# Chemical118/TREW

Hardware: NVIDIA B200
Metric: Gbases/s for trew short 5 32 at 1/2/4/8 B200; % of HBM roofline (higher is better)
Workload: dtype u64

## Files before the change

trew_b200/csrc/device_ctx.cu:

```cuda
#include <algorithm>
#include <chrono>
#include <cstdarg>
#include <cstdio>
#include <cstdlib>
#include <cstring>
#include <string>
#include <thread>
#include <vector>

#include <cuda_runtime.h>

#include "host_internal.h"
#include "scan_kernels.cuh"

using namespace trew;

namespace {

struct SlotRes {
    void* h_buf = nullptr;
    void* d_buf = nullptr;
    unsigned char* h_inv = nullptr;
    unsigned char* d_inv = nullptr;
    size_t inv_cap = 0;
    unsigned int* h_keys = nullptr;
    unsigned int* d_survivors = nullptr;
    unsigned int* d_counters = nullptr;
    unsigned char* d_scratch = nullptr;
    size_t scratch_bytes = 0;
    size_t survivors_cap = 0;
    cudaStream_t stream = nullptr;
    cudaEvent_t ev_start = nullptr, ev_done = nullptr;
    bool in_flight = false;
};

struct RangeInfo { uint32_t r0, r1; uint64_t bases; uint32_t max_len; };

}

struct trew_resident {
    void* d_buf = nullptr;
    DevBatch batch{};
    uint32_t n_reads = 0, n_units = 0, max_read_len = 0;
    uint64_t bases = 0;
    unsigned int* d_survivors = nullptr;
    unsigned int* d_counters = nullptr;
    unsigned char* d_scratch = nullptr;
    size_t scratch_bytes = 0;
    cudaEvent_t ev[4] = {nullptr, nullptr, nullptr, nullptr};
    bool ev_pending = false;
};

struct trew_ctx {
    trew_config cfg{};
    int sm_count = 0;
    LaunchPlan plan{};
    cudaStream_t aux_stream = nullptr;
    cudaEvent_t ev_join = nullptr;
    int resident_streams = 1;
    uint64_t resident_seq = 0;
    DevCfg dcfg{};
    size_t n_slots = 0;
    unsigned int* d_error = nullptr;
    unsigned short* d_thr = nullptr;
    unsigned long long* d_total_surv = nullptr;
    std::vector<SlotRes> slots;
    size_t next_slot = 0;
    size_t staging_bytes = 0;
    cudaStream_t main_stream = nullptr;
    cudaEvent_t ev_a = nullptr, ev_b = nullptr;
    trew_entry* d_entries = nullptr; size_t d_entries_cap = 0;
    trew_entry* d_sorted = nullptr; size_t d_sorted_cap = 0;
    trew_entry* d_concat = nullptr; size_t d_concat_cap = 0;
    bool sorted_valid = false;
    void* d_sort_tmp = nullptr; size_t sort_tmp_bytes = 0;
    unsigned int* d_n = nullptr;
    uint64_t n_export = 0;
    bool export_valid = false;
    trew_stats stats{};
    Pool* pool = nullptr;
    bool own_pool = true;
    std::string err;
    std::vector<RangeInfo> ranges_tmp;
    unsigned int keys_seen = 0;
    bool sparse_val = true;
    unsigned int exact_flags = 0;
    std::vector<InvList> inv_tmp;
    IngestScratch ingest;
    cudaEvent_t ev_t0 = nullptr, ev_t1 = nullptr;
    double screen_ms = 0, decide_ms = 0, exact_ms = 0; uint64_t n_prof_scans = 0;
    std::vector<trew_resident*> pending_prof;
    void* h_export = nullptr; size_t h_export_bytes = 0;
    unsigned int report_min = 0;
    trew_entry* d_filtered = nullptr; size_t d_filtered_cap = 0;
};

namespace {

int fail(trew_ctx* c, int status, const char* fmt, ...) {
    char buf[512];
    va_list ap; va_start(ap, fmt); vsnprintf(buf, sizeof(buf), fmt, ap); va_end(ap);
    if (c) c->err = buf;
    return status;
}

#define CK(call)                                                                                         \
    do {                                                                                                 \
        cudaError_t e_ = (call);                                                                         \
        if (e_ != cudaSuccess) return fail(ctx, TREW_ERR_CUDA, "%s: %s", #call, cudaGetErrorString(e_)); \
    } while (0)

void build_thr(double B, std::vector<unsigned short>& thr) {
    thr.assign(kThrTableSize, 0xFFFF);
    for (int T = 1; T < kThrTableSize; T++) {
        int lo = 0, hi = T;
        while (lo < hi) {
            int mid = (lo + hi) / 2;
            if ((double)mid / (double)T >= B) hi = mid; else lo = mid + 1;
        }
        thr[T] = (unsigned short)lo;
    }
}

int run_cap_for(const trew_config& cfg, uint32_t max_read_len) {
    uint32_t w = max_read_len;
    if (cfg.mode == TREW_MODE_LONG) w = std::min<uint32_t>(max_read_len, 2u * (uint32_t)cfg.slice_length);
    w = std::min<uint32_t>(w, (uint32_t)kMaxWindow);
    return (int)std::max<uint32_t>((w + 2 + 7) & ~7u, 32u);
}

constexpr unsigned int kLongThreadCap = 32768;

size_t scratch_need(const trew_ctx* ctx, uint32_t max_read_len, uint32_t n_units, unsigned int* stride, size_t* long_off,
                    unsigned int* s_cap, unsigned int* max_slices) {
    unsigned int st = 16;
    if (ctx->cfg.mode == TREW_MODE_LONG) st = 2u * (max_read_len / (uint32_t)ctx->cfg.slice_length + 2u);
    st = (st + 15u) & ~15u;
    *stride = st;
    size_t bytes = ((size_t)st * (size_t)exact_warps_total(ctx->sm_count) + 255) & ~(size_t)255;
    *long_off = bytes;
    *s_cap = 0; *max_slices = 0;
    if (long_thread_path_applies(ctx->dcfg) && (ctx->exact_flags & 16u)) {
        *s_cap = std::min<unsigned int>(std::max<unsigned int>(n_units, 1u), kLongThreadCap);
        *max_slices = max_read_len / (uint32_t)ctx->cfg.slice_length + 1u;
        bytes += long_thread_scratch_bytes(*s_cap, *max_slices);
    }
    return bytes;
}

constexpr int kScanCounters = 8;

static int env_blocks_thread() {
    static const int v = [] { const char* e = getenv("TREW_GRID_THREAD"); int x = e && *e ? atoi(e) : 0; return x > 0 ? x : 0; }();
    return v;
}

int launch_scan(trew_ctx* ctx, const DevBatch& b, uint32_t n_units, uint32_t max_read_len, unsigned int* d_survivors,
                unsigned int* d_counters, unsigned char** d_scratch, size_t* scratch_bytes, cudaStream_t st,
                cudaEvent_t* ev = nullptr) {
    unsigned int stride, s_cap, max_slices;
    size_t long_off;
    size_t need = scratch_need(ctx, max_read_len, n_units, &stride, &long_off, &s_cap, &max_slices);
    if (need > *scratch_bytes) {
        if (*d_scratch) { CK(cudaStreamSynchronize(st)); CK(cudaFree(*d_scratch)); *d_scratch = nullptr; }
        CK(cudaMalloc((void**)d_scratch, need));
        *scratch_bytes = need;
    }
    ctx->export_valid = false;
    CK(cudaMemsetAsync(d_counters, 0, kScanCounters * sizeof(unsigned int), st));
    if (ev) CK(cudaEventRecord(ev[0], st));
    const bool thread_path = thread_path_applies(ctx->dcfg, max_read_len) && !(ctx->exact_flags & 4u) && n_units < (1u << 28);
    launch_filter(ctx->dcfg, b, n_units, max_read_len, d_survivors + n_units, d_counters + 2, d_survivors, d_counters, ctx->plan, st,
                  ev ? ev[1] : nullptr, thread_path ? d_survivors + n_units - 1 : nullptr, thread_path ? d_counters + 4 : nullptr,
                  d_counters + 7);
    if (ev) CK(cudaEventRecord(ev[2], st));
    ExactArgs a{};
    a.survivors = d_survivors; a.n_survivors = d_counters; a.work_counter = d_counters + 1;
    a.slice_scratch = *d_scratch; a.slice_scratch_stride = stride; a.run_cap = run_cap_for(ctx->cfg, max_read_len);
    a.total_survivors = ctx->d_total_surv;
    a.packed_probes = n_units < (1u << 28) ? 1 : 0;
    a.exp_flags = ctx->exact_flags;
    if (thread_path) {
        unsigned int* hard = d_survivors + n_units;
        launch_exact_thread(ctx->dcfg, b, d_survivors, d_counters, a.packed_probes, hard, d_counters + 3, ctx->d_total_surv,
                            ctx->sm_count, env_blocks_thread(), d_counters + 6, st);
        ExactArgs ab = a;
        ab.survivors = d_survivors + n_units - 1; ab.reverse = 1; ab.n_survivors = d_counters + 4;
        launch_exact(ctx->dcfg, b, ab, ctx->plan, st);
        a.survivors = hard; a.n_survivors = d_counters + 3; a.work_counter = d_counters + 5; a.total_survivors = nullptr;
        ctx->stats.kernel_launches += 2;
    } else if (s_cap > 0 && n_units < (1u << 28)) {
        unsigned int* hard = d_survivors + n_units;
        launch_long_thread(ctx->dcfg, b, d_survivors, d_counters, a.packed_probes, s_cap, max_slices, *d_scratch + long_off, hard,
                           d_counters + 3, ctx->d_total_surv, ctx->sm_count, st);
        a.survivors = hard; a.n_survivors = d_counters + 3; a.total_survivors = nullptr;
        ctx->stats.kernel_launches += 3;
    }
    launch_exact(ctx->dcfg, b, a, ctx->plan, st);
    if (ev) CK(cudaEventRecord(ev[3], st));
    CK(cudaGetLastError());
    ctx->stats.kernel_launches += 3;
    return TREW_OK;
}

int retire_slot(trew_ctx* ctx, SlotRes& s) {
    if (!s.in_flight) return TREW_OK;
    CK(cudaEventSynchronize(s.ev_done));
    float ms = 0.f;
    CK(cudaEventElapsedTime(&ms, s.ev_start, s.ev_done));
    ctx->stats.device_ms += ms;
    s.in_flight = false;
    ctx->keys_seen = std::max(ctx->keys_seen, *s.h_keys);
    return TREW_OK;
}

int export_sorted(trew_ctx* ctx, uint64_t* n_out);
int check_device_error(trew_ctx* ctx);

int grow_table_to(trew_ctx* ctx, size_t min_slots) {
    size_t new_slots = ctx->n_slots;
    while (new_slots < ((size_t)1 << 28) && new_slots < min_slots) new_slots <<= 1;
    if (new_slots == ctx->n_slots) return TREW_OK;
    uint64_t n = 0;
    int rc = export_sorted(ctx, &n);
    if (rc) return rc;
    Slot* d_new = nullptr;
    CK(cudaMalloc((void**)&d_new, new_slots * sizeof(Slot)));
    CK(cudaMemsetAsync(d_new, 0, new_slots * sizeof(Slot), ctx->main_stream));
    CK(cudaMemsetAsync(ctx->d_error + 1, 0, sizeof(unsigned int), ctx->main_stream));
    Slot* d_old = ctx->dcfg.slots;
    ctx->dcfg.slots = d_new; ctx->dcfg.slot_mask = (unsigned int)(new_slots - 1); ctx->n_slots = new_slots;
    launch_merge_entries(ctx->dcfg, ctx->d_entries, (unsigned int)n, ctx->main_stream);
    CK(cudaGetLastError());
    CK(cudaStreamSynchronize(ctx->main_stream));
    CK(cudaFree(d_old));
    ctx->stats.kernel_launches += 1;
    ctx->keys_seen = (unsigned int)n;
    for (auto& sl : ctx->slots) *sl.h_keys = (unsigned int)n;
    return check_device_error(ctx);
}

int maybe_grow_table(trew_ctx* ctx) {
    if ((size_t)ctx->keys_seen * 16 <= ctx->n_slots) return TREW_OK;
    unsigned int keys = 0;
    CK(cudaMemcpy(&keys, ctx->d_error + 1, sizeof(keys), cudaMemcpyDeviceToHost));
    ctx->keys_seen = std::max(ctx->keys_seen, keys);
    if ((size_t)keys * 4 <= ctx->n_slots) return TREW_OK;
    return grow_table_to(ctx, (size_t)keys * 8);
}

int submit_ranges(trew_ctx* ctx, const ChunkView& cv, const RangeInfo* rg, int n_ranges) {
    uint64_t total_bases = 0; uint32_t max_len = 0;
    for (int i = 0; i < n_ranges; i++) { total_bases += rg[i].bases; max_len = std::max(max_len, rg[i].max_len); }
    const uint32_t n = n_ranges ? rg[n_ranges - 1].r1 - rg[0].r0 : 0u;
    if (n == 0) return TREW_OK;
    SlotRes& s = ctx->slots[ctx->next_slot];
    ctx->next_slot = (ctx->next_slot + 1) % ctx->slots.size();
    static const bool trace = getenv("TREW_SUBMIT_TRACE") != nullptr;
    auto now = [] { return std::chrono::duration<double, std::milli>(std::chrono::steady_clock::now().time_since_epoch()).count(); };
    const double t0 = trace ? now() : 0;
    int rc = retire_slot(ctx, s);
    if (rc) return rc;
    const double t1 = trace ? now() : 0;
    if ((rc = maybe_grow_table(ctx)) != TREW_OK) return rc;
    const double t2 = now();
    BatchView v;
    batch_layout(s.h_buf, n, total_bases, &v);
    std::vector<uint64_t> bit0((size_t)n_ranges);
    uint64_t acc = 0;
    for (int i = 0; i < n_ranges; i++) { bit0[i] = acc; acc += rg[i].bases; }
    v.bit_off[n] = (uint32_t)total_bases;
    const uint32_t first = rg[0].r0;
    std::vector<uint64_t> side_flat((size_t)3 * n_ranges);
    uint64_t (*side)[3] = (uint64_t (*)[3])side_flat.data();
    if (ctx->inv_tmp.size() < (size_t)n_ranges) ctx->inv_tmp.resize((size_t)n_ranges);
    auto pack = [&](bool list) {
        pack_prepare(bit0.data(), n_ranges, total_bases, v);
        ctx->pool->run(n_ranges, [&](int i) {
            pack_chunk_range(cv, rg[i].r0, rg[i].r1, rg[i].r0 - first, bit0[i], v, side[i], list ? &ctx->inv_tmp[(size_t)i] : nullptr, list,
                             rg[i].bases);
        });
        pack_fixup(bit0.data(), side, n_ranges, v);
    };
    size_t n_inv = 0;
    bool sparse = ctx->sparse_val;
    pack(sparse);
    const bool tail_pad = (total_bases & 31) != 0;
    if (sparse) {
        n_inv = tail_pad ? 1 : 0;
        for (int i = 0; i < n_ranges; i++) n_inv += ctx->inv_tmp[(size_t)i].size();
        if (n_inv > s.inv_cap) { sparse = false; pack(false); }
    }

    const double t3 = now();
    ctx->stats.host_pack_bytes += total_bases; ctx->stats.host_pack_ms += t3 - t2;
    CK(cudaEventRecord(s.ev_start, s.stream));
    const size_t head_bytes = (size_t)((char*)v.val - (char*)s.h_buf);
    unsigned int* d_val = (unsigned int*)((char*)s.d_buf + head_bytes);
    size_t sent = v.bytes;
    if (sparse) {
        std::vector<size_t> at((size_t)n_ranges + 1, 0);
        for (int i = 0; i < n_ranges; i++) at[(size_t)i + 1] = at[(size_t)i] + ctx->inv_tmp[(size_t)i].bytes();
        ctx->pool->run(n_ranges, [&](int i) {
            const InvList& l = ctx->inv_tmp[(size_t)i];
            if (l.bytes()) memcpy(s.h_inv + at[(size_t)i], l.buf.get(), l.bytes());
        });
        if (tail_pad) inv_record(s.h_inv + at[(size_t)n_ranges], (uint32_t)total_bases, (1ULL << (32 - (total_bases & 31))) - 1ULL);
        const size_t ones_words = (size_t)((total_bases + 31) / 32);
        CK(cudaMemsetAsync(d_val, 0xFF, ones_words * 4, s.stream));
        CK(cudaMemsetAsync(d_val + ones_words, 0, (v.plane_words - ones_words) * 4, s.stream));
        CK(cudaMemcpyAsync(s.d_buf, s.h_buf, head_bytes, cudaMemcpyHostToDevice, s.stream));
        if (n_inv) {
            CK(cudaMemcpyAsync(s.d_inv, s.h_inv, n_inv * kInvRecBytes, cudaMemcpyHostToDevice, s.stream));
            launch_clear_invalid(d_val, (const unsigned int*)s.d_inv, (unsigned int)n_inv, s.stream);
            ctx->stats.kernel_launches += 1;
        }
        sent = head_bytes + n_inv * kInvRecBytes;
    } else {
        CK(cudaMemcpyAsync(s.d_buf, s.h_buf, v.bytes, cudaMemcpyHostToDevice, s.stream));
    }
    DevBatch b{};
    b.n_reads = n;
    b.bit_off = (const unsigned int*)s.d_buf;
    b.hi = (const unsigned int*)((char*)s.d_buf + ((char*)v.hi - (char*)s.h_buf));
    b.lo = b.hi + v.plane_words; b.val = d_val;
    uint32_t n_units = ctx->cfg.mode == TREW_MODE_PAIR ? n / 2 : n;
    rc = launch_scan(ctx, b, n_units, max_len, s.d_survivors, s.d_counters, &s.d_scratch, &s.scratch_bytes, s.stream);
    if (rc) return rc;
    CK(cudaMemcpyAsync(s.h_keys, ctx->d_error + 1, sizeof(unsigned int), cudaMemcpyDeviceToHost, s.stream));
    CK(cudaEventRecord(s.ev_done, s.stream));
    s.in_flight = true;
    ctx->stats.reads += n; ctx->stats.bases += total_bases; ctx->stats.units += n_units; ctx->stats.h2d_bytes += sent;
    if (trace)
        fprintf(stderr, "[submit] %u reads: wait slot %.3f ms, table check %.3f ms, pack %.3f ms, enqueue %.3f ms\n", n, t1 - t0, t2 - t1,
                t3 - t2, now() - t3);
    return TREW_OK;
}

int submit_chunk_view(trew_ctx* ctx, const ChunkView& cv, uint32_t n) {
    if (n == 0) return TREW_OK;
    const uint32_t unit = cv.unit;
    const uint32_t n_units = n / unit;
    uint64_t span = 0;
    for (int sd = 0; sd < (int)unit; sd++) {
        const int32_t* l = cv.locs[sd];
        span += (uint64_t)std::max<int64_t>(0, (int64_t)l[2 * (size_t)(n_units - 1) + 1] - l[0] + 1);
    }
    uint64_t by_size = span / std::max<uint64_t>(1, ctx->staging_bytes / 16) + 1;
    uint32_t n_ranges = (uint32_t)std::min<uint64_t>(n_units, std::max<uint64_t>(by_size, (uint64_t)ctx->pool->size() * 4));
    auto& rg = ctx->ranges_tmp;
    rg.resize(n_ranges);
    for (uint32_t i = 0; i < n_ranges; i++) {
        rg[i].r0 = (uint32_t)((uint64_t)n_units * i / n_ranges) * unit;
        rg[i].r1 = (uint32_t)((uint64_t)n_units * (i + 1) / n_ranges) * unit;
    }
    ctx->pool->run((int)n_ranges, [&](int i) { chunk_stats(cv, rg[i].r0, rg[i].r1, &rg[i].bases, &rg[i].max_len); });
    uint32_t mx = 0;
    for (auto& r : rg) mx = std::max(mx, r.max_len);
    if (ctx->cfg.mode == TREW_MODE_SHORT && mx > 1000)
        return fail(ctx, TREW_ERR_TOO_LONG, "%s", trew_status_string(TREW_ERR_TOO_LONG));
    if (ctx->cfg.mode == TREW_MODE_PAIR && mx > (uint32_t)kMaxWindow) return fail(ctx, TREW_ERR_TOO_LONG, "paired read longer than %d", kMaxWindow);
    const size_t cap = ctx->slots[0].survivors_cap;
    uint32_t g = 0;
    while (g < n_ranges) {
        uint32_t h = g; uint64_t bases = 0; uint64_t reads = 0;
        while (h < n_ranges) {
            uint64_t nb = bases + rg[h].bases, nr = reads + (rg[h].r1 - rg[h].r0);
            if (batch_bytes((uint32_t)nr, nb) > ctx->staging_bytes || nr > cap || nb >= 0xfffff000ULL) break;
            bases = nb; reads = nr; h++;
        }
        if (h == g) {
            if (rg[g].r1 - rg[g].r0 <= unit)
                return fail(ctx, TREW_ERR_ARG, "a single read/pair (%llu bases) does not fit a staging buffer of %zu bytes",
                            (unsigned long long)rg[g].bases, ctx->staging_bytes);
            std::vector<RangeInfo> fine;
            for (uint32_t r = rg[g].r0; r < rg[g].r1; r += unit) {
                RangeInfo f{r, r + unit, 0, 0};
                chunk_stats(cv, f.r0, f.r1, &f.bases, &f.max_len);
                fine.push_back(f);
            }
            size_t a = 0;
            while (a < fine.size()) {
                size_t e = a; uint64_t fb = 0, fr = 0;
                while (e < fine.size()) {
                    uint64_t nb = fb + fine[e].bases, nr = fr + unit;
                    if (batch_bytes((uint32_t)nr, nb) > ctx->staging_bytes || nr > cap || nb >= 0xfffff000ULL) break;
                    fb = nb; fr = nr; e++;
                }
                if (e == a)
                    return fail(ctx, TREW_ERR_ARG, "a single read/pair (%llu bases) does not fit a staging buffer of %zu bytes",
                                (unsigned long long)fine[a].bases, ctx->staging_bytes);
                std::vector<RangeInfo> merged;
                size_t per = std::max<size_t>(1, (e - a) / (size_t)ctx->pool->size());
                for (size_t i = a; i < e; i += per) {
                    RangeInfo m{fine[i].r0, 0, 0, 0};
                    for (size_t j = i; j < std::min(e, i + per); j++) { m.r1 = fine[j].r1; m.bases += fine[j].bases; m.max_len = std::max(m.max_len, fine[j].max_len); }
                    merged.push_back(m);
                }
                int rc = submit_ranges(ctx, cv, merged.data(), (int)merged.size());
                if (rc) return rc;
                a = e;
            }
            g++;
            continue;
        }
        int rc = submit_ranges(ctx, cv, rg.data() + g, (int)(h - g));
        if (rc) return rc;
        g = h;
    }
    return TREW_OK;
}

int collect_prof(trew_ctx* ctx) {
    for (trew_resident* r : ctx->pending_prof) {
        if (!r->ev_pending) continue;
        CK(cudaEventSynchronize(r->ev[3]));
        float a = 0, b = 0, c = 0;
        CK(cudaEventElapsedTime(&a, r->ev[0], r->ev[1]));
        CK(cudaEventElapsedTime(&b, r->ev[1], r->ev[2]));
        CK(cudaEventElapsedTime(&c, r->ev[2], r->ev[3]));
        ctx->screen_ms += a; ctx->decide_ms += b; ctx->exact_ms += c; ctx->n_prof_scans++;
        ctx->stats.device_ms += a + b + c;
        r->ev_pending = false;
    }
    ctx->pending_prof.clear();
    return TREW_OK;
}

int join_aux(trew_ctx* ctx) {
    if (ctx->resident_streams != 2) return TREW_OK;
    CK(cudaEventRecord(ctx->ev_join, ctx->aux_stream));
    CK(cudaStreamWaitEvent(ctx->main_stream, ctx->ev_join, 0));
    return TREW_OK;
}

int fork_aux(trew_ctx* ctx) {
    if (ctx->resident_streams != 2) return TREW_OK;
    CK(cudaEventRecord(ctx->ev_join, ctx->main_stream));
    CK(cudaStreamWaitEvent(ctx->aux_stream, ctx->ev_join, 0));
    return TREW_OK;
}

int check_device_error(trew_ctx* ctx) {
    unsigned int e = 0;
    CK(cudaMemcpy(&e, ctx->d_error, sizeof(e), cudaMemcpyDeviceToHost));
    if (e == 3u) return fail(ctx, TREW_ERR_TABLE_FULL, "device count table full (%zu slots): raise table_log2_slots", ctx->n_slots);
    if (e) return fail(ctx, TREW_ERR_CUDA, "device error flag %u", e);
    return TREW_OK;
}

}

extern "C" {

int trew_abi_version(void) { return TREW_ABI_VERSION; }

const char* trew_status_string(int status) {
    switch (status) {
        case TREW_OK: return "ok";
        case TREW_ERR_ARG: return "bad argument";
        case TREW_ERR_CUDA: return "CUDA failure";
        case TREW_ERR_TABLE_FULL: return "device count table full";
        case TREW_ERR_TOO_LONG: return "This mode is designed for short-read sequencing. Please use 'trew long'.";
        case TREW_ERR_IO: return "file I/O error";
        case TREW_ERR_PAIRING: return "paired-end record mismatch";
        case TREW_ERR_NOMEM: return "memory allocation failure";
        default: return "unknown status";
    }
}

static thread_local std::string g_create_error;

static int default_host_threads(int asked) {
    return asked > 0 ? asked : (int)std::min(64u, std::max(1u, std::thread::hardware_concurrency()));
}

const char* trew_dev_last_error(const trew_ctx* ctx) { return ctx ? ctx->err.c_str() : g_create_error.c_str(); }

static int create_ctx(const trew_config* cfg, trew_ctx** out, std::string& g_create_error, Pool* shared_pool) {
    if (!cfg || !out) return TREW_ERR_ARG;
    *out = nullptr;
    g_create_error.clear();
    auto bad_arg = [&](const char* msg) { g_create_error = msg; return TREW_ERR_ARG; };
    if (cfg->mode < 0 || cfg->mode > 2) return bad_arg("mode must be TREW_MODE_SHORT, _PAIR or _LONG");
    if (cfg->min_mer < 3 || cfg->max_mer > 64 || cfg->min_mer > cfg->max_mer) return bad_arg("need 3 <= MIN_MER <= MAX_MER <= 64");
    if (!(0 < cfg->low_baseline && cfg->low_baseline <= 1) || !(0 < cfg->high_baseline && cfg->high_baseline <= 1) ||
        cfg->low_baseline > cfg->high_baseline) return bad_arg("need 0 < LOW_BASELINE <= HIGH_BASELINE <= 1");
    if (cfg->mode == TREW_MODE_LONG && cfg->slice_length > 0 && cfg->slice_length < 2 * cfg->max_mer)
        return bad_arg("SLICE_LENGTH must be greater than or equal to twice of MAX_MER.");
    if (cfg->mode == TREW_MODE_LONG && cfg->slice_length > 512)
        return bad_arg("SLICE_LENGTH above 512 is not supported by the GPU path (a slice of up to 2*SLICE_LENGTH-1 bases must fit "
                       "a 1023-base window); use -s 512 or less.");
    trew_ctx* ctx = new trew_ctx();
    ctx->cfg = *cfg;
    if (ctx->cfg.slice_length <= 0) ctx->cfg.slice_length = 150;
    auto bail = [&](int rc) { g_create_error = ctx->err; trew_dev_destroy(ctx); return rc; };
#define CKC(call)                                                                                   \
    do {                                                                                            \
        cudaError_t e_ = (call);                                                                    \
        if (e_ != cudaSuccess) { fail(ctx, TREW_ERR_CUDA, "%s: %s", #call, cudaGetErrorString(e_)); return bail(TREW_ERR_CUDA); } \
    } while (0)
    const bool timing = getenv("TREW_CLI_TIMING") != nullptr;
    auto now = [] { return std::chrono::duration<double, std::milli>(std::chrono::steady_clock::now().time_since_epoch()).count(); };
    double t_prev = now();
    auto lap = [&](const char* what) {
        if (!timing) return;
        const double t = now();
        fprintf(stderr, "[trew] create, device %d: %s %.1f ms\n", cfg->device, what, t - t_prev);
        t_prev = t;
    };
    int ndev = 0;
    CKC(cudaGetDeviceCount(&ndev));
    lap("driver init");
    if (cfg->device < 0 || cfg->device >= ndev) { fail(ctx, TREW_ERR_CUDA, "no CUDA device %d (found %d)", cfg->device, ndev); return bail(TREW_ERR_CUDA); }
    CKC(cudaSetDevice(cfg->device));
    cudaDeviceProp prop;
    CKC(cudaGetDeviceProperties(&prop, cfg->device));
    ctx->sm_count = prop.multiProcessorCount;
    ctx->plan = default_launch_plan(ctx->sm_count);
    {
        auto env_int = [](const char* name, int dflt) { const char* e = getenv(name); return e && *e ? atoi(e) : dflt; };
        int v;
        if ((v = env_int("TREW_GRID_SCREEN", 0)) > 0) ctx->plan.screen_blocks = ctx->sm_count * v;
        if ((v = env_int("TREW_GRID_DECIDE", 0)) > 0) ctx->plan.decide_blocks = ctx->sm_count * v;
        if ((v = env_int("TREW_GRID_EXACT", 0)) > 0) ctx->plan.exact_blocks = std::min(ctx->plan.exact_blocks, ctx->sm_count * v);
        ctx->resident_streams = env_int("TREW_RESIDENT_STREAMS", 1) >= 2 ? 2 : 1;
        ctx->sparse_val = env_int("TREW_DENSE_VAL", 0) == 0;
        ctx->exact_flags = (unsigned int)env_int("TREW_EXACT_FLAGS", 0);
    }
    int lg = cfg->table_log2_slots > 0 ? cfg->table_log2_slots : 22;
    if (lg < 10 || lg > 28) { fail(ctx, TREW_ERR_ARG, "table_log2_slots out of range"); return bail(TREW_ERR_ARG); }
    ctx->n_slots = (size_t)1 << lg;
    Slot* d_slots = nullptr;
    CKC(cudaMalloc((void**)&d_slots, ctx->n_slots * sizeof(Slot)));
    CKC(cudaMemset(d_slots, 0, ctx->n_slots * sizeof(Slot)));
    lap("primary context + count table");
    CKC(cudaMalloc((void**)&ctx->d_error, 2 * sizeof(unsigned int)));
    CKC(cudaMemset(ctx->d_error, 0, 2 * sizeof(unsigned int)));
    CKC(cudaMalloc((void**)&ctx->d_total_surv, sizeof(unsigned long long)));
    CKC(cudaMemset(ctx->d_total_surv, 0, sizeof(unsigned long long)));
    std::vector<unsigned short> thr;
    build_thr(cfg->low_baseline, thr);
    std::vector<unsigned short> thr_hi;
    build_thr(cfg->high_baseline, thr_hi);
    CKC(cudaMalloc((void**)&ctx->d_thr, 2 * thr.size() * sizeof(unsigned short)));
    CKC(cudaMemcpy(ctx->d_thr, thr.data(), thr.size() * sizeof(unsigned short), cudaMemcpyHostToDevice));
    CKC(cudaMemcpy(ctx->d_thr + thr.size(), thr_hi.data(), thr_hi.size() * sizeof(unsigned short), cudaMemcpyHostToDevice));
    ctx->dcfg.mode = cfg->mode; ctx->dcfg.min_mer = cfg->min_mer; ctx->dcfg.max_mer = cfg->max_mer;
    ctx->dcfg.slice_len = ctx->cfg.slice_length; ctx->dcfg.low = cfg->low_baseline; ctx->dcfg.high = cfg->high_baseline;
    ctx->dcfg.slots = d_slots; ctx->dcfg.slot_mask = (unsigned int)(ctx->n_slots - 1);
    ctx->dcfg.error_flag = ctx->d_error; ctx->dcfg.thr_low = ctx->d_thr; ctx->dcfg.thr_high = ctx->d_thr + kThrTableSize;
    CKC(prepare_exact(kMaxWindow + 9));
    lap("kernel attributes (module load)");
    CKC(cudaStreamCreateWithFlags(&ctx->main_stream, cudaStreamNonBlocking));
    CKC(cudaStreamCreateWithFlags(&ctx->aux_stream, cudaStreamNonBlocking));
    CKC(cudaEventCreateWithFlags(&ctx->ev_join, cudaEventDisableTiming));
    CKC(cudaEventCreate(&ctx->ev_a));
    CKC(cudaEventCreate(&ctx->ev_b));
    CKC(cudaEventCreate(&ctx->ev_t0));
    CKC(cudaEventCreate(&ctx->ev_t1));
    ctx->staging_bytes = cfg->staging_bytes ? (size_t)cfg->staging_bytes : ((size_t)64 << 20);
    int ns = cfg->n_staging > 0 ? cfg->n_staging : 3;
    ctx->slots.resize((size_t)ns);
    for (auto& s : ctx->slots) {
        CKC(cudaHostAlloc(&s.h_buf, ctx->staging_bytes, cudaHostAllocDefault));
        CKC(cudaMalloc(&s.d_buf, ctx->staging_bytes));
        s.inv_cap = ctx->staging_bytes / 8 / kInvRecBytes;
        CKC(cudaHostAlloc((void**)&s.h_inv, (s.inv_cap + 1) * kInvRecBytes, cudaHostAllocDefault));
        CKC(cudaMalloc((void**)&s.d_inv, (s.inv_cap + 1) * kInvRecBytes));
        CKC(cudaHostAlloc((void**)&s.h_keys, sizeof(unsigned int), cudaHostAllocDefault));
        *s.h_keys = 0;
        s.survivors_cap = ctx->staging_bytes / 8;
        CKC(cudaMalloc((void**)&s.d_survivors, 2 * s.survivors_cap * sizeof(unsigned int)));
        CKC(cudaMalloc((void**)&s.d_counters, kScanCounters * sizeof(unsigned int)));
        CKC(cudaStreamCreateWithFlags(&s.stream, cudaStreamNonBlocking));
        CKC(cudaEventCreate(&s.ev_start));
        CKC(cudaEventCreate(&s.ev_done));
    }
    CKC(cudaMalloc((void**)&ctx->d_n, sizeof(unsigned int)));
    lap("staging ring (pinned + device buffers)");
    if (shared_pool) { ctx->pool = shared_pool; ctx->own_pool = false; }
    else ctx->pool = new Pool(default_host_threads(cfg->host_threads));
#undef CKC
    *out = ctx;
    return TREW_OK;
}

int trew_dev_create(const trew_config* cfg, trew_ctx** out) { return create_ctx(cfg, out, g_create_error, nullptr); }

void trew_dev_destroy(trew_ctx* ctx) {
    if (!ctx) return;
    cudaSetDevice(ctx->cfg.device);
    cudaDeviceSynchronize();
    for (auto& s : ctx->slots) {
        if (s.h_buf) cudaFreeHost(s.h_buf);
        if (s.d_buf) cudaFree(s.d_buf);
        if (s.h_inv) cudaFreeHost(s.h_inv);
        if (s.d_inv) cudaFree(s.d_inv);
        if (s.h_keys) cudaFreeHost(s.h_keys);
        if (s.d_survivors) cudaFree(s.d_survivors);
        if (s.d_counters) cudaFree(s.d_counters);
        if (s.d_scratch) cudaFree(s.d_scratch);
        if (s.stream) cudaStreamDestroy(s.stream);
        if (s.ev_start) cudaEventDestroy(s.ev_start);
        if (s.ev_done) cudaEventDestroy(s.ev_done);
    }
    if (ctx->dcfg.slots) cudaFree(ctx->dcfg.slots);
    if (ctx->d_error) cudaFree(ctx->d_error);
    if (ctx->d_thr) cudaFree(ctx->d_thr);
    if (ctx->d_total_surv) cudaFree(ctx->d_total_surv);
    if (ctx->d_entries) cudaFree(ctx->d_entries);
    if (ctx->d_sorted) cudaFree(ctx->d_sorted);
    if (ctx->d_concat) cudaFree(ctx->d_concat);
    if (ctx->d_filtered) cudaFree(ctx->d_filtered);
    if (ctx->d_sort_tmp) cudaFree(ctx->d_sort_tmp);
    if (ctx->d_n) cudaFree(ctx->d_n);
    if (ctx->h_export) cudaFreeHost(ctx->h_export);
    if (ctx->main_stream) cudaStreamDestroy(ctx->main_stream);
    if (ctx->aux_stream) cudaStreamDestroy(ctx->aux_stream);
    if (ctx->ev_join) cudaEventDestroy(ctx->ev_join);
    if (ctx->ev_a) cudaEventDestroy(ctx->ev_a);
    if (ctx->ev_b) cudaEventDestroy(ctx->ev_b);
    if (ctx->ev_t0) cudaEventDestroy(ctx->ev_t0);
    if (ctx->ev_t1) cudaEventDestroy(ctx->ev_t1);
    if (ctx->own_pool) delete ctx->pool;
    delete ctx;
}

int trew_dev_submit_chunk(trew_ctx* ctx, const char* buffer1, const int32_t* locs1, uint32_t n1,
                          const char* buffer2, const int32_t* locs2, uint32_t n2) {
    if (!ctx) return TREW_ERR_ARG;
    CK(cudaSetDevice(ctx->cfg.device));
    const bool pair = ctx->cfg.mode == TREW_MODE_PAIR;
    if (pair ? (!buffer2 && n2) : (buffer2 != nullptr || n2 != 0)) return fail(ctx, TREW_ERR_ARG, "second chunk only in pair mode");
    if ((n1 && (!buffer1 || !locs1)) || (n2 && !locs2)) return fail(ctx, TREW_ERR_ARG, "null chunk");
    ChunkView cv{{buffer1, buffer2}, {locs1, locs2}, {nullptr, nullptr}, pair ? 2u : 1u};
    const uint32_t n = pair ? 2u * std::min(n1, n2) : n1;
    if (n == 0) return TREW_OK;
    for (int sd = 0; sd < (pair ? 2 : 1); sd++) {
        const int32_t* l = cv.locs[sd];
        uint32_t cnt = pair ? n / 2 : n;
        int32_t last = l[2 * (size_t)(cnt - 1) + 1];
        if (last >= l[2 * (size_t)(cnt - 1)]) cv.end[sd] = cv.buf[sd] + last + 1;
    }
    return submit_chunk_view(ctx, cv, n);
}

int trew_dev_submit_packed(trew_ctx* ctx, const trew_batch* batch) {
    if (!ctx || !batch) return TREW_ERR_ARG;
    CK(cudaSetDevice(ctx->cfg.device));
    uint32_t n = batch->n_reads;
    if (n == 0) return TREW_OK;
    uint64_t bases = batch->bit_off[n];
    size_t bytes = batch_bytes(n, bases);
    if (bytes > ctx->staging_bytes || n > ctx->slots[0].survivors_cap)
        return fail(ctx, TREW_ERR_ARG, "packed batch (%zu bytes) larger than a staging buffer (%zu)", bytes, ctx->staging_bytes);
    if (batch->bit_off[0] != 0) return fail(ctx, TREW_ERR_ARG, "bit_off[0] must be 0");
    SlotRes& s = ctx->slots[ctx->next_slot];
    ctx->next_slot = (ctx->next_slot + 1) % ctx->slots.size();
    int rc = retire_slot(ctx, s);
    if (rc) return rc;
    BatchView v;
    batch_layout(s.h_buf, n, bases, &v);
    size_t words = (size_t)((bases + 31) / 32);
    memcpy(v.bit_off, batch->bit_off, (size_t)(n + 1) * 4);
    const uint32_t* src[3] = {batch->hi, batch->lo, batch->val};
    uint32_t* dst[3] = {v.hi, v.lo, v.val};
    ctx->pool->run(3, [&](int i) {
        memcpy(dst[i], src[i], words * 4);
        memset(dst[i] + words, 0, (v.plane_words - words) * 4);
    });
    CK(cudaEventRecord(s.ev_start, s.stream));
    CK(cudaMemcpyAsync(s.d_buf, s.h_buf, v.bytes, cudaMemcpyHostToDevice, s.stream));
    DevBatch b{};
    b.n_reads = n;
    b.bit_off = (const unsigned int*)s.d_buf;
    b.hi = (const unsigned int*)((char*)s.d_buf + ((char*)v.hi - (char*)s.h_buf));
    b.lo = b.hi + v.plane_words; b.val = b.lo + v.plane_words;
    uint32_t n_units = ctx->cfg.mode == TREW_MODE_PAIR ? n / 2 : n;
    rc = launch_scan(ctx, b, n_units, batch->max_read_len, s.d_survivors, s.d_counters, &s.d_scratch, &s.scratch_bytes, s.stream);
    if (rc) return rc;
    CK(cudaMemcpyAsync(s.h_keys, ctx->d_error + 1, sizeof(unsigned int), cudaMemcpyDeviceToHost, s.stream));
    CK(cudaEventRecord(s.ev_done, s.stream));
    s.in_flight = true;
    ctx->stats.reads += n; ctx->stats.bases += bases; ctx->stats.units += n_units; ctx->stats.h2d_bytes += v.bytes;
    return TREW_OK;
}

int trew_dev_upload(trew_ctx* ctx, const trew_batch* batch, trew_resident** out) {
    if (!ctx || !batch || !out) return TREW_ERR_ARG;
    CK(cudaSetDevice(ctx->cfg.device));
    uint32_t n = batch->n_reads;
    uint64_t bases = n ? batch->bit_off[n] : 0;
    trew_resident* r = new trew_resident();
    size_t bytes = batch_bytes(n, bases);
    std::vector<char> tmp(bytes, 0);
    BatchView v;
    batch_layout(tmp.data(), n, bases, &v);
    size_t words = (size_t)((bases + 31) / 32);
    if (n) {
        memcpy(v.bit_off, batch->bit_off, (size_t)(n + 1) * 4);
        memcpy(v.hi, batch->hi, words * 4); memcpy(v.lo, batch->lo, words * 4); memcpy(v.val, batch->val, words * 4);
    }
    CK(cudaMalloc(&r->d_buf, bytes));
    CK(cudaMemcpy(r->d_buf, tmp.data(), bytes, cudaMemcpyHostToDevice));
    r->batch.n_reads = n;
    r->batch.bit_off = (const unsigned int*)r->d_buf;
    r->batch.hi = (const unsigned int*)((char*)r->d_buf + ((char*)v.hi - tmp.data()));
    r->batch.lo = r->batch.hi + v.plane_words; r->batch.val = r->batch.lo + v.plane_words;
    r->n_reads = n; r->n_units = ctx->cfg.mode == TREW_MODE_PAIR ? n / 2 : n; r->max_read_len = batch->max_read_len; r->bases = bases;
    CK(cudaMalloc((void**)&r->d_survivors, 2 * (size_t)std::max<uint32_t>(r->n_units, 1) * sizeof(unsigned int)));
    CK(cudaMalloc((void**)&r->d_counters, kScanCounters * sizeof(unsigned int)));
    *out = r;
    return TREW_OK;
}

int trew_dev_scan_resident(trew_ctx* ctx, const trew_resident* rb) {
    if (!ctx || !rb) return TREW_ERR_ARG;
    CK(cudaSetDevice(ctx->cfg.device));
    trew_resident* r = const_cast<trew_resident*>(rb);
    ctx->keys_seen = std::max<unsigned int>(ctx->keys_seen, (unsigned int)(ctx->n_slots / 16 + 1));
    if (r->ev_pending) { int rc0 = collect_prof(ctx); if (rc0) return rc0; }
    if (!r->ev[0]) for (int i = 0; i < 4; i++) CK(cudaEventCreate(&r->ev[i]));
    cudaStream_t st = (ctx->resident_streams == 2 && (ctx->resident_seq++ & 1)) ? ctx->aux_stream : ctx->main_stream;
    CK(cudaEventRecord(ctx->ev_a, st));
    int rc = launch_scan(ctx, r->batch, r->n_units, r->max_read_len, r->d_survivors, r->d_counters, &r->d_scratch,
                         &r->scratch_bytes, st, r->ev);
    r->ev_pending = true; ctx->pending_prof.push_back(r);
    if (rc) return rc;
    CK(cudaEventRecord(ctx->ev_b, st));
    ctx->stats.reads += r->n_reads; ctx->stats.bases += r->bases; ctx->stats.units += r->n_units;
    return TREW_OK;
}

void trew_dev_free_resident(trew_ctx* ctx, trew_resident* r) {
    if (!r) return;
    if (ctx) { cudaSetDevice(ctx->cfg.device); cudaStreamSynchronize(ctx->main_stream); cudaStreamSynchronize(ctx->aux_stream); collect_prof(ctx); }
    for (int i = 0; i < 4; i++) if (r->ev[i]) cudaEventDestroy(r->ev[i]);
    if (r->d_buf) cudaFree(r->d_buf);
    if (r->d_survivors) cudaFree(r->d_survivors);
    if (r->d_counters) cudaFree(r->d_counters);
    if (r->d_scratch) cudaFree(r->d_scratch);
    delete r;
}

int trew_dev_sync(trew_ctx* ctx) {
    if (!ctx) return TREW_ERR_ARG;
    CK(cudaSetDevice(ctx->cfg.device));
    for (auto& s : ctx->slots) { int rc = retire_slot(ctx, s); if (rc) return rc; }
    { int rc = join_aux(ctx); if (rc) return rc; }
    CK(cudaStreamSynchronize(ctx->main_stream));
    { int rc = collect_prof(ctx); if (rc) return rc; }
    return check_device_error(ctx);
}

}

namespace {

int export_entries(trew_ctx* ctx, bool need_sorted, const trew_entry** out, uint64_t* n_out) {
    int rc = trew_dev_sync(ctx);
    if (rc) return rc;
    if (!ctx->export_valid) {
        unsigned int n = 0;
        for (int pass = 0; pass < 2; pass++) {
            CK(cudaMemsetAsync(ctx->d_n, 0, sizeof(unsigned int), ctx->main_stream));
            if (pass == 0 && ctx->d_entries_cap == 0) {
                ctx->d_entries_cap = (size_t)1 << 20;
                CK(cudaMalloc((void**)&ctx->d_entries, ctx->d_entries_cap * sizeof(trew_entry)));
            }
            launch_compact(ctx->dcfg.slots, (unsigned int)ctx->n_slots, ctx->d_entries, ctx->d_n, ctx->main_stream,
                           (unsigned int)ctx->d_entries_cap);
            CK(cudaGetLastError());
            ctx->stats.kernel_launches += 1;
            CK(cudaMemcpyAsync(&n, ctx->d_n, sizeof(n), cudaMemcpyDeviceToHost, ctx->main_stream));
            CK(cudaStreamSynchronize(ctx->main_stream));
            if (n <= ctx->d_entries_cap) break;
            CK(cudaFree(ctx->d_entries));
            ctx->d_entries = nullptr;
            ctx->d_entries_cap = (size_t)n + n / 4 + 1024;
            CK(cudaMalloc((void**)&ctx->d_entries, ctx->d_entries_cap * sizeof(trew_entry)));
        }
        ctx->n_export = n;
        ctx->export_valid = true;
        ctx->sorted_valid = false;
    }
    const unsigned int n = (unsigned int)ctx->n_export;
    if (need_sorted && !ctx->sorted_valid) {
        if (n > ctx->d_sorted_cap) {
            if (ctx->d_sorted) CK(cudaFree(ctx->d_sorted));
            ctx->d_sorted = nullptr;
            ctx->d_sorted_cap = std::max<size_t>((size_t)n + n / 4 + 1024, (size_t)1 << 20);
            CK(cudaMalloc((void**)&ctx->d_sorted, ctx->d_sorted_cap * sizeof(trew_entry)));
        }
        if (n == 1) CK(cudaMemcpyAsync(ctx->d_sorted, ctx->d_entries, sizeof(trew_entry), cudaMemcpyDeviceToDevice, ctx->main_stream));
        if (n > 1) {
            const bool wide = ctx->cfg.max_mer > 32;
            size_t need = 0;
            CK(sort_entries_radix(ctx->d_entries, ctx->d_sorted, n, wide, nullptr, &need, ctx->main_stream));
            if (need > ctx->sort_tmp_bytes) {
                if (ctx->d_sort_tmp) CK(cudaFree(ctx->d_sort_tmp));
                ctx->d_sort_tmp = nullptr;
                ctx->sort_tmp_bytes = need + need / 4;
                CK(cudaMalloc(&ctx->d_sort_tmp, ctx->sort_tmp_bytes));
            }
            size_t bytes = ctx->sort_tmp_bytes;
            CK(sort_entries_radix(ctx->d_entries, ctx->d_sorted, n, wide, ctx->d_sort_tmp, &bytes, ctx->main_stream));
            ctx->stats.kernel_launches += wide ? 11 : 8;
        }
        CK(cudaStreamSynchronize(ctx->main_stream));
        ctx->sorted_valid = true;
    }
    if (out) *out = need_sorted ? ctx->d_sorted : ctx->d_entries;
    if (n_out) *n_out = n;
    return TREW_OK;
}

int export_sorted(trew_ctx* ctx, uint64_t* n_out) { return export_entries(ctx, false, nullptr, n_out); }

int rows_to_host(trew_ctx* ctx, const trew_entry* d_rows, uint64_t n, const trew_entry** entries, uint64_t* n_entries) {
    size_t need_host = (size_t)n * sizeof(trew_entry) + 64;
    if (need_host > ctx->h_export_bytes) {
        if (ctx->h_export) CK(cudaFreeHost(ctx->h_export));
        ctx->h_export = nullptr;
        size_t cap = std::max(need_host * 2, (size_t)1 << 20);
        CK(cudaHostAlloc(&ctx->h_export, cap, cudaHostAllocDefault));
        ctx->h_export_bytes = cap;
    }
    if (n) {
        CK(cudaMemcpyAsync(ctx->h_export, d_rows, n * sizeof(trew_entry), cudaMemcpyDeviceToHost, ctx->main_stream));
        CK(cudaStreamSynchronize(ctx->main_stream));
    }
    ctx->stats.d2h_bytes += n * sizeof(trew_entry) + 4;
    if (entries) *entries = (const trew_entry*)ctx->h_export;
    if (n_entries) *n_entries = n;
    return TREW_OK;
}

int finish_rows(trew_ctx* ctx, const trew_entry* d_in, uint64_t n_in, bool combine, const trew_entry** entries, uint64_t* n_entries) {
    auto ensure = [&](trew_entry** buf, size_t* cap, size_t want) -> int {
        if (want <= *cap) return TREW_OK;
        if (*buf) CK(cudaFree(*buf));
        *buf = nullptr;
        *cap = std::max<size_t>(want + want / 4 + 1024, (size_t)1 << 20);
        CK(cudaMalloc((void**)buf, *cap * sizeof(trew_entry)));
        return TREW_OK;
    };
    auto ensure_tmp = [&](size_t need) -> int {
        if (need <= ctx->sort_tmp_bytes) return TREW_OK;
        CK(cudaStreamSynchronize(ctx->main_stream));
        if (ctx->d_sort_tmp) CK(cudaFree(ctx->d_sort_tmp));
        ctx->d_sort_tmp = nullptr;
        ctx->sort_tmp_bytes = need + need / 4;
        CK(cudaMalloc(&ctx->d_sort_tmp, ctx->sort_tmp_bytes));
        return TREW_OK;
    };
    int rc;
    if ((rc = ensure(&ctx->d_sorted, &ctx->d_sorted_cap, (size_t)n_in)) != TREW_OK) return rc;
    if ((rc = ensure(&ctx->d_filtered, &ctx->d_filtered_cap, (size_t)n_in)) != TREW_OK) return rc;
    ctx->sorted_valid = false;
    const bool wide = ctx->cfg.max_mer > 32;
    const trew_entry* src = d_in;
    unsigned int n = (unsigned int)n_in;
    if (ctx->report_min > 0 && n > 0) {
        size_t need = 0;
        CK(filter_report_rows(src, n, ctx->report_min, ctx->d_filtered, ctx->d_n, nullptr, &need, ctx->main_stream));
        if ((rc = ensure_tmp(need)) != TREW_OK) return rc;
        size_t bytes = ctx->sort_tmp_bytes;
        CK(filter_report_rows(src, n, ctx->report_min, ctx->d_filtered, ctx->d_n, ctx->d_sort_tmp, &bytes, ctx->main_stream));
        CK(cudaMemcpyAsync(&n, ctx->d_n, sizeof(n), cudaMemcpyDeviceToHost, ctx->main_stream));
        CK(cudaStreamSynchronize(ctx->main_stream));
        ctx->stats.kernel_launches += 5;
        src = ctx->d_filtered;
    }
    if (n == 1) CK(cudaMemcpyAsync(ctx->d_sorted, src, sizeof(trew_entry), cudaMemcpyDeviceToDevice, ctx->main_stream));
    if (n > 1) {
        size_t need = 0;
        CK(sort_entries_radix(src, ctx->d_sorted, n, wide, nullptr, &need, ctx->main_stream));
        if ((rc = ensure_tmp(need)) != TREW_OK) return rc;
        size_t bytes = ctx->sort_tmp_bytes;
        CK(sort_entries_radix(src, ctx->d_sorted, n, wide, ctx->d_sort_tmp, &bytes, ctx->main_stream));
        ctx->stats.kernel_launches += wide ? 11 : 8;
    }
    const trew_entry* rows = ctx->d_sorted;
    if (combine && n > 0) {
        size_t need = 0;
        CK(combine_sorted_rows(ctx->d_sorted, n, ctx->d_filtered, ctx->d_n, nullptr, &need, ctx->main_stream));
        if ((rc = ensure_tmp(need)) != TREW_OK) return rc;
        size_t bytes = ctx->sort_tmp_bytes;
        CK(combine_sorted_rows(ctx->d_sorted, n, ctx->d_filtered, ctx->d_n, ctx->d_sort_tmp, &bytes, ctx->main_stream));
        CK(cudaMemcpyAsync(&n, ctx->d_n, sizeof(n), cudaMemcpyDeviceToHost, ctx->main_stream));
        CK(cudaStreamSynchronize(ctx->main_stream));
        ctx->stats.kernel_launches += 3;
        rows = ctx->d_filtered;
    }
    return rows_to_host(ctx, rows, n, entries, n_entries);
}

}

extern "C" {

int trew_dev_export_device(trew_ctx* ctx, const trew_entry** d_entries, uint64_t* n_entries) {
    if (!ctx) return TREW_ERR_ARG;
    return export_entries(ctx, true, d_entries, n_entries);
}

int trew_dev_finish(trew_ctx* ctx, const trew_entry** entries, uint64_t* n_entries) {
    if (!ctx) return TREW_ERR_ARG;
    uint64_t n = 0;
    const trew_entry* d_rows = nullptr;
    if (ctx->report_min > 0) {
        int rc = export_entries(ctx, false, &d_rows, &n);
        if (rc) return rc;
        return finish_rows(ctx, d_rows, n, false, entries, n_entries);
    }
    int rc = export_entries(ctx, true, &d_rows, &n);
    if (rc) return rc;
    return rows_to_host(ctx, d_rows, n, entries, n_entries);
}

int trew_dev_finish_merged(trew_ctx* ctx, const trew_entry* const* d_lists, const uint64_t* n_rows, uint32_t n_lists,
                           const trew_entry** entries, uint64_t* n_entries) {
    if (!ctx || (n_lists && (!d_lists || !n_rows))) return TREW_ERR_ARG;
    uint64_t n0 = 0;
    const trew_entry* d_own = nullptr;
    int rc = export_entries(ctx, false, &d_own, &n0);
    if (rc) return rc;
    uint64_t total = n0;
    for (uint32_t i = 0; i < n_lists; i++) total += n_rows[i];
    if (total > 0xfffffff0ULL) return fail(ctx, TREW_ERR_ARG, "too many rows to merge (%llu)", (unsigned long long)total);
    auto ensure = [&](trew_entry** buf, size_t* cap) -> int {
        if (total <= *cap) return TREW_OK;
        if (*buf) CK(cudaFree(*buf));
        *buf = nullptr;
        *cap = std::max<size_t>((size_t)total + total / 4 + 1024, (size_t)1 << 20);
        CK(cudaMalloc((void**)buf, *cap * sizeof(trew_entry)));
        return TREW_OK;
    };
    if ((rc = ensure(&ctx->d_concat, &ctx->d_concat_cap)) != TREW_OK) return rc;
    uint64_t at = 0;
    if (n0) CK(cudaMemcpyAsync(ctx->d_concat, d_own, n0 * sizeof(trew_entry), cudaMemcpyDeviceToDevice, ctx->main_stream));
    at += n0;
    for (uint32_t i = 0; i < n_lists; i++) {
        if (n_rows[i]) CK(cudaMemcpyAsync(ctx->d_concat + at, d_lists[i], n_rows[i] * sizeof(trew_entry), cudaMemcpyDeviceToDevice, ctx->main_stream));
        at += n_rows[i];
    }
    return finish_rows(ctx, ctx->d_concat, total, true, entries, n_entries);
}

int trew_dev_export_rows(trew_ctx* ctx, trew_entry* d_rows, uint64_t capacity_rows, uint64_t* n_rows) {
    if (!ctx || !n_rows) return TREW_ERR_ARG;
    uint64_t n = 0;
    const trew_entry* d_src = nullptr;
    int rc = export_entries(ctx, false, &d_src, &n);
    if (rc) return rc;
    *n_rows = n;
    if (!d_rows) return TREW_OK;
    if (n > capacity_rows) return fail(ctx, TREW_ERR_ARG, "row buffer too small: %llu rows, capacity %llu", (unsigned long long)n,
                                       (unsigned long long)capacity_rows);
    if (n) CK(cudaMemcpyAsync(d_rows, d_src, n * sizeof(trew_entry), cudaMemcpyDeviceToDevice, ctx->main_stream));
    CK(cudaStreamSynchronize(ctx->main_stream));
    return TREW_OK;
}

int trew_dev_merge_rows(trew_ctx* ctx, const trew_entry* d_rows, uint64_t n_rows) {
    if (!ctx || (n_rows && !d_rows) || n_rows > 0xffffffffULL) return TREW_ERR_ARG;
    CK(cudaSetDevice(ctx->cfg.device));
    ctx->export_valid = false;
    ctx->keys_seen = std::max<unsigned int>(ctx->keys_seen, (unsigned int)(ctx->n_slots / 16 + 1));
    launch_merge_entries(ctx->dcfg, d_rows, (unsigned int)n_rows, ctx->main_stream);
    CK(cudaGetLastError());
    ctx->stats.kernel_launches += n_rows ? 1 : 0;
    return TREW_OK;
}

int trew_dev_set_report_filter(trew_ctx* ctx, uint32_t min_total) {
    if (!ctx) return TREW_ERR_ARG;
    ctx->report_min = min_total;
    return TREW_OK;
}

int trew_dev_reserve(trew_ctx* ctx, uint64_t expected_new_keys) {
    if (!ctx) return TREW_ERR_ARG;
    int rc = trew_dev_sync(ctx);
    if (rc) return rc;
    unsigned int keys = 0;
    CK(cudaMemcpy(&keys, ctx->d_error + 1, sizeof(keys), cudaMemcpyDeviceToHost));
    const uint64_t want = ((uint64_t)keys + expected_new_keys) * 4;
    if (want <= ctx->n_slots) return TREW_OK;
    return grow_table_to(ctx, (size_t)std::min<uint64_t>(want, (uint64_t)1 << 28));
}

int trew_dev_reset(trew_ctx* ctx) {
    if (!ctx) return TREW_ERR_ARG;
    int rc = trew_dev_sync(ctx);
    if (rc && rc != TREW_ERR_TABLE_FULL) return rc;
    ctx->export_valid = false;
    CK(cudaMemsetAsync(ctx->dcfg.slots, 0, ctx->n_slots * sizeof(Slot), ctx->main_stream));
    CK(cudaMemsetAsync(ctx->d_error, 0, 2 * sizeof(unsigned int), ctx->main_stream));
    CK(cudaStreamSynchronize(ctx->main_stream));
    ctx->keys_seen = 0;
    for (auto& sl : ctx->slots) *sl.h_keys = 0;
    return TREW_OK;
}

int trew_dev_get_stats(trew_ctx* ctx, trew_stats* out) {
    if (!ctx || !out) return TREW_ERR_ARG;
    CK(cudaSetDevice(ctx->cfg.device));
    unsigned long long s = 0;
    CK(cudaMemcpy(&s, ctx->d_total_surv, sizeof(s), cudaMemcpyDeviceToHost));
    ctx->stats.survivors = s;
    *out = ctx->stats;
    return TREW_OK;
}

int trew_dev_last_resident_ms(trew_ctx* ctx, float* ms) {
    if (!ctx || !ms) return TREW_ERR_ARG;
    CK(cudaEventSynchronize(ctx->ev_b));
    CK(cudaEventElapsedTime(ms, ctx->ev_a, ctx->ev_b));
    return TREW_OK;
}

int trew_dev_timer_start(trew_ctx* ctx) {
    if (!ctx) return TREW_ERR_ARG;
    CK(cudaSetDevice(ctx->cfg.device));
    CK(cudaEventRecord(ctx->ev_t0, ctx->main_stream));
    return fork_aux(ctx);
}

int trew_dev_timer_stop(trew_ctx* ctx, float* ms) {
    if (!ctx || !ms) return TREW_ERR_ARG;
    CK(cudaSetDevice(ctx->cfg.device));
    { int rc = join_aux(ctx); if (rc) return rc; }
    CK(cudaEventRecord(ctx->ev_t1, ctx->main_stream));
    CK(cudaEventSynchronize(ctx->ev_t1));
    CK(cudaEventElapsedTime(ms, ctx->ev_t0, ctx->ev_t1));
    return TREW_OK;
}

int trew_dev_kernel_times(trew_ctx* ctx, double* screen_ms, double* decide_ms, double* exact_ms, uint64_t* n_scans) {
    if (!ctx) return TREW_ERR_ARG;
    CK(cudaSetDevice(ctx->cfg.device));
    { int rc0 = join_aux(ctx); if (rc0) return rc0; }
    CK(cudaStreamSynchronize(ctx->main_stream));
    int rc = collect_prof(ctx);
    if (rc) return rc;
    if (screen_ms) *screen_ms = ctx->screen_ms;
    if (decide_ms) *decide_ms = ctx->decide_ms;
    if (exact_ms) *exact_ms = ctx->exact_ms;
    if (n_scans) *n_scans = ctx->n_prof_scans;
    ctx->screen_ms = ctx->decide_ms = ctx->exact_ms = 0; ctx->n_prof_scans = 0;
    return TREW_OK;
}

int trew_synth_resident(trew_ctx* ctx, uint64_t seed, uint32_t n_reads, uint32_t read_len, uint32_t tel_ppm,
                        uint32_t half_ppm, uint32_t n_ppm, uint32_t sub_ppm, trew_resident** out) {
    return trew_synth_resident_ex(ctx, seed, n_reads, read_len, tel_ppm, half_ppm, n_ppm, sub_ppm, 0, out);
}

int trew_synth_resident_ex(trew_ctx* ctx, uint64_t seed, uint32_t n_reads, uint32_t read_len, uint32_t tel_ppm,
                           uint32_t half_ppm, uint32_t n_ppm, uint32_t sub_ppm, uint32_t flavor, trew_resident** out) {
    if (!ctx || !out || read_len == 0 || flavor > 2 || (uint64_t)n_reads * read_len >= 0xfffff000ULL) return TREW_ERR_ARG;
    CK(cudaSetDevice(ctx->cfg.device));
    auto thr = [](uint32_t ppm) { return (unsigned int)(((unsigned long long)ppm << 32) / 1000000ULL); };
    uint64_t bases = (uint64_t)n_reads * read_len;
    size_t bytes = batch_bytes(n_reads, bases);
    trew_resident* r = new trew_resident();
    CK(cudaMalloc(&r->d_buf, bytes));
    BatchView v;
    batch_layout(r->d_buf, n_reads, bases, &v);
    launch_synth(seed, n_reads, read_len, thr(tel_ppm), thr(half_ppm), thr(n_ppm), thr(sub_ppm), flavor, v.bit_off, v.hi, v.lo, v.val,
                 v.plane_words, ctx->main_stream);
    CK(cudaGetLastError());
    CK(cudaStreamSynchronize(ctx->main_stream));
    r->batch.n_reads = n_reads; r->batch.bit_off = v.bit_off; r->batch.hi = v.hi; r->batch.lo = v.lo; r->batch.val = v.val;
    r->n_reads = n_reads; r->n_units = ctx->cfg.mode == TREW_MODE_PAIR ? n_reads / 2 : n_reads;
    r->max_read_len = read_len; r->bases = bases;
    CK(cudaMalloc((void**)&r->d_survivors, 2 * (size_t)std::max<uint32_t>(r->n_units, 1) * sizeof(unsigned int)));
    CK(cudaMalloc((void**)&r->d_counters, kScanCounters * sizeof(unsigned int)));
    *out = r;
    return TREW_OK;
}

int trew_dev_process_file(trew_ctx* ctx, const char* file1, int is_gz1, const char* file2, int is_gz2) {
    if (!ctx || !file1) return TREW_ERR_ARG;
    if ((ctx->cfg.mode == TREW_MODE_PAIR) != (file2 != nullptr)) return fail(ctx, TREW_ERR_ARG, "second file only in pair mode");
    const size_t chunk = 0;
    IngestResult r = ingest_file(ctx->cfg.mode, ctx->cfg.slice_length, file1, is_gz1 != 0, file2, is_gz2 != 0, chunk,
                                 [&](const char* b1, const std::vector<int32_t>& l1, const char* b2, const std::vector<int32_t>& l2) {
                                     return trew_dev_submit_chunk(ctx, b1, l1.data(), (uint32_t)(l1.size() / 2), b2,
                                                                  b2 ? l2.data() : nullptr, b2 ? (uint32_t)(l2.size() / 2) : 0u);
                                 },
                                 ctx->pool, &ctx->ingest);
    if (r.status != TREW_OK && r.status != TREW_ERR_CUDA && !r.message.empty()) ctx->err = r.message;
    return r.status;
}

}


struct trew_multi {
    std::vector<trew_ctx*> ctx;
    Pool* pool = nullptr;
    size_t next = 0;
    std::string err;
    std::vector<trew_entry*> d_peer; std::vector<size_t> d_peer_cap;
};

namespace {
int mfail(trew_multi* m, int status, const std::string& msg) { if (m) m->err = msg; return status; }
}

extern "C" {

int trew_multi_create(const trew_config* cfg, const int32_t* devices, int32_t n_devices, trew_multi** out) {
    if (!cfg || !out || n_devices < 0 || (n_devices > 0 && !devices)) return TREW_ERR_ARG;
    *out = nullptr;
    std::vector<int32_t> dev;
    if (n_devices == 0) {
        int nd = 0;
        if (cudaGetDeviceCount(&nd) != cudaSuccess || nd <= 0) { g_create_error = "no CUDA device"; return TREW_ERR_CUDA; }
        for (int i = 0; i < nd; i++) dev.push_back(i);
    } else {
        dev.assign(devices, devices + n_devices);
    }
    trew_multi* m = new trew_multi();
    m->pool = new Pool(default_host_threads(cfg->host_threads));
    int rc = TREW_OK;
    {
        std::vector<trew_ctx*> made(dev.size(), nullptr);
        std::vector<int> rcs(dev.size(), TREW_OK);
        std::vector<std::string> errs(dev.size());
        std::vector<std::thread> th;
        auto make = [&](size_t i) {
            trew_config c = *cfg;
            c.device = dev[i];
            rcs[i] = create_ctx(&c, &made[i], errs[i], m->pool);
        };
        for (size_t i = 1; i < dev.size(); i++) th.emplace_back(make, i);
        make(0);
        for (auto& t : th) t.join();
        for (size_t i = 0; i < dev.size(); i++) {
            if (rcs[i] != TREW_OK && rc == TREW_OK) { rc = rcs[i]; g_create_error = errs[i]; }
            if (made[i]) m->ctx.push_back(made[i]);
        }
    }
    if (rc != TREW_OK) { trew_multi_destroy(m); return rc; }
    for (size_t i = 1; i < m->ctx.size(); i++) {
        int can = 0;
        if (dev[i] != dev[0] && cudaDeviceCanAccessPeer(&can, dev[0], dev[i]) == cudaSuccess && can) {
            cudaSetDevice(dev[0]);
            cudaError_t e = cudaDeviceEnablePeerAccess(dev[i], 0);
            if (e != cudaSuccess) cudaGetLastError();
        }
    }
    m->d_peer.assign(m->ctx.size(), nullptr);
    m->d_peer_cap.assign(m->ctx.size(), 0);
    *out = m;
    return TREW_OK;
}

void trew_multi_destroy(trew_multi* m) {
    if (!m) return;
    if (!m->ctx.empty()) {
        cudaSetDevice(m->ctx[0]->cfg.device);
        for (trew_entry* p : m->d_peer) if (p) cudaFree(p);
    }
    for (trew_ctx* x : m->ctx) trew_dev_destroy(x);
    delete m->pool;
    delete m;
}

int trew_multi_device_count(const trew_multi* m) { return m ? (int)m->ctx.size() : 0; }

const char* trew_multi_last_error(const trew_multi* m) { return m ? m->err.c_str() : g_create_error.c_str(); }

trew_ctx* trew_multi_ctx(trew_multi* m, int32_t i) { return m && i >= 0 && (size_t)i < m->ctx.size() ? m->ctx[(size_t)i] : nullptr; }

int trew_multi_submit_chunk(trew_multi* m, const char* buffer1, const int32_t* locs1, uint32_t n1, const char* buffer2,
                            const int32_t* locs2, uint32_t n2) {
    if (!m) return TREW_ERR_ARG;
    trew_ctx* x = m->ctx[m->next];
    m->next = (m->next + 1) % m->ctx.size();
    int rc = trew_dev_submit_chunk(x, buffer1, locs1, n1, buffer2, locs2, n2);
    if (rc != TREW_OK) return mfail(m, rc, x->err);
    return TREW_OK;
}

int trew_multi_process_file(trew_multi* m, const char* file1, int is_gz1, const char* file2, int is_gz2) {
    if (!m || !file1) return TREW_ERR_ARG;
    trew_ctx* x0 = m->ctx[0];
    if ((x0->cfg.mode == TREW_MODE_PAIR) != (file2 != nullptr)) return mfail(m, TREW_ERR_ARG, "second file only in pair mode");
    IngestResult r = ingest_file(x0->cfg.mode, x0->cfg.slice_length, file1, is_gz1 != 0, file2, is_gz2 != 0, 0,
                                 [&](const char* b1, const std::vector<int32_t>& l1, const char* b2, const std::vector<int32_t>& l2) {
                                     return trew_multi_submit_chunk(m, b1, l1.data(), (uint32_t)(l1.size() / 2), b2, b2 ? l2.data() : nullptr,
                                                                    b2 ? (uint32_t)(l2.size() / 2) : 0u);
                                 },
                                 m->pool, &x0->ingest);
    if (r.status != TREW_OK && !r.message.empty()) m->err = r.message;
    return r.status;
}

int trew_multi_reset(trew_multi* m) {
    if (!m) return TREW_ERR_ARG;
    for (trew_ctx* x : m->ctx) { int rc = trew_dev_reset(x); if (rc != TREW_OK) return mfail(m, rc, x->err); }
    m->next = 0;
    return TREW_OK;
}

int trew_multi_finish(trew_multi* m, const trew_entry** entries, uint64_t* n_entries) {
    if (!m) return TREW_ERR_ARG;
    trew_ctx* x0 = m->ctx[0];
    const size_t nd = m->ctx.size();
    if (nd == 1) {
        int rc = trew_dev_finish(x0, entries, n_entries);
        return rc == TREW_OK ? rc : mfail(m, rc, x0->err);
    }
    std::vector<const trew_entry*> d_src(nd, nullptr);
    std::vector<uint64_t> n_rows(nd, 0);
    for (size_t i = 1; i < nd; i++) {
        int rc = export_entries(m->ctx[i], false, &d_src[i], &n_rows[i]);
        if (rc != TREW_OK) return mfail(m, rc, m->ctx[i]->err);
    }
    trew_ctx* ctx = x0;
    CK(cudaSetDevice(x0->cfg.device));
    std::vector<const trew_entry*> lists;
    std::vector<uint64_t> sizes;
    for (size_t i = 1; i < nd; i++) {
        if (n_rows[i] == 0) continue;
        if (n_rows[i] > m->d_peer_cap[i]) {
            if (m->d_peer[i]) CK(cudaFree(m->d_peer[i]));
            m->d_peer[i] = nullptr;
            m->d_peer_cap[i] = (size_t)n_rows[i] + n_rows[i] / 4 + 1024;
            CK(cudaMalloc((void**)&m->d_peer[i], m->d_peer_cap[i] * sizeof(trew_entry)));
        }
        CK(cudaMemcpyPeerAsync(m->d_peer[i], x0->cfg.device, d_src[i], m->ctx[i]->cfg.device, n_rows[i] * sizeof(trew_entry), x0->main_stream));
        lists.push_back(m->d_peer[i]);
        sizes.push_back(n_rows[i]);
    }
    int rc = trew_dev_finish_merged(x0, lists.data(), sizes.data(), (uint32_t)lists.size(), entries, n_entries);
    return rc == TREW_OK ? rc : mfail(m, rc, x0->err);
}

int trew_multi_set_report_filter(trew_multi* m, uint32_t min_total) {
    if (!m) return TREW_ERR_ARG;
    return trew_dev_set_report_filter(m->ctx[0], min_total);
}

int trew_multi_get_stats(trew_multi* m, trew_stats* out) {
    if (!m || !out) return TREW_ERR_ARG;
    trew_stats t;
    memset(&t, 0, sizeof(t));
    for (trew_ctx* x : m->ctx) {
        trew_stats s;
        int rc = trew_dev_get_stats(x, &s);
        if (rc != TREW_OK) return mfail(m, rc, x->err);
        t.reads += s.reads; t.bases += s.bases; t.units += s.units; t.survivors += s.survivors;
        t.kernel_launches += s.kernel_launches; t.h2d_bytes += s.h2d_bytes; t.d2h_bytes += s.d2h_bytes;
        t.host_pack_bytes += s.host_pack_bytes; t.host_pack_ms += s.host_pack_ms;
        t.device_ms = std::max(t.device_ms, s.device_ms);
    }
    *out = t;
    return TREW_OK;
}

}
```

trew_b200/csrc/scan_kernels.cu:

```cuda
#include "scan_kernels.cuh"
#include "exact_thread.cuh"

#include <cstdio>

namespace trew {

typedef unsigned int u32;
typedef unsigned long long u64;
typedef unsigned __int128 u128;


__device__ __forceinline__ u32 lane_id() { return threadIdx.x & 31; }

__device__ __forceinline__ u32 low_mask(int bits) {
    return bits >= 32 ? 0xffffffffu : ((1u << bits) - 1u);
}

__device__ __forceinline__ u32 prefix_xor32(u32 x) {
    x ^= x << 1; x ^= x << 2; x ^= x << 4; x ^= x << 8; x ^= x << 16;
    return x;
}

__device__ __forceinline__ u64 mix64(u64 x) {
    x ^= x >> 33; x *= 0xff51afd7ed558ccdULL; x ^= x >> 33; x *= 0xc4ceb9fe1a85ec53ULL; x ^= x >> 33;
    return x;
}


__device__ __noinline__ void table_add_impl(Slot* slots, u32 slot_mask, u32* error_flag, u32 meta, u64 lo, u64 hi, u64 cnt) {
#ifdef TREW_EXP_NOADD
    return;
#endif
    u64 h = mix64(lo ^ mix64(hi + 0x9e3779b97f4a7c15ULL * (u64)(meta + 1)));
    u32 i = (u32)h & slot_mask;
    for (u32 probe = 0; probe <= slot_mask; probe++, i = (i + 1) & slot_mask) {
        Slot* s = slots + i;
        const uint4 a = __ldcg(reinterpret_cast<const uint4*>(s)), c = __ldcg(reinterpret_cast<const uint4*>(s) + 1);
        u32 st = c.w;
        if (st == 2u) {
            if (c.z == meta && a.x == (u32)lo && a.y == (u32)(lo >> 32) && a.z == (u32)hi && a.w == (u32)(hi >> 32)) {
                atomicAdd(&s->count, cnt);
                return;
            }
            __threadfence();
            if (__ldcg(&s->meta) == meta && __ldcg(&s->seq_lo) == lo && __ldcg(&s->seq_hi) == hi) {
                atomicAdd(&s->count, cnt);
                return;
            }
            continue;
        }
        int outcome = 0;
        do {
            st = atomicCAS(&s->state, 0u, 1u);
            if (st == 0u) {
                s->seq_lo = lo; s->seq_hi = hi; s->meta = meta;
                __threadfence();
                atomicExch(&s->state, 2u);
                atomicAdd(&s->count, cnt);
                atomicAdd(error_flag + 1, 1u);
                outcome = 1;
            } else if (st == 2u) {
                __threadfence();
                if (__ldcg(&s->meta) == meta && __ldcg(&s->seq_lo) == lo && __ldcg(&s->seq_hi) == hi) {
                    atomicAdd(&s->count, cnt);
                    outcome = 1;
                } else outcome = 2;
            }
        } while (outcome == 0);
        if (outcome == 1) return;
    }
    atomicExch(error_flag, 3u);
}

__global__ void merge_entries_kernel(Slot* slots, u32 slot_mask, u32* error_flag, const trew_entry* __restrict__ e, u32 n) {
    for (u32 i = blockIdx.x * blockDim.x + threadIdx.x; i < n; i += gridDim.x * blockDim.x)
        table_add_impl(slots, slot_mask, error_flag, ((u32)e[i].table << 8) | (u32)e[i].k, e[i].seq_lo, e[i].seq_hi, e[i].count);
}

void launch_merge_entries(const DevCfg& cfg, const trew_entry* entries, unsigned int n, cudaStream_t stream) {
    if (n) merge_entries_kernel<<<(n + 255) / 256, 256, 0, stream>>>(cfg.slots, cfg.slot_mask, cfg.error_flag, entries, n);
}


__host__ __device__ inline u32 synth_hash(u64 seed, u64 a, u64 b) {
    u64 x = seed + 0x9e3779b97f4a7c15ULL * (a + 1) + 0xbf58476d1ce4e5b9ULL * (b + 1);
    x ^= x >> 30; x *= 0xbf58476d1ce4e5b9ULL; x ^= x >> 27; x *= 0x94d049bb133111ebULL; x ^= x >> 31;
    return (u32)(x >> 32);
}

__global__ void synth_kernel(u64 seed, u32 n_reads, u32 L, u32 tel_thr, u32 half_thr, u32 n_thr, u32 sub_thr, u32 flavor,
                             u32* __restrict__ bit_off, u32* __restrict__ hi, u32* __restrict__ lo, u32* __restrict__ val,
                             size_t plane_words) {
    const u64 total = (u64)n_reads * L;
    const size_t stride = (size_t)gridDim.x * blockDim.x;
    for (size_t i = (size_t)blockIdx.x * blockDim.x + threadIdx.x; i <= n_reads; i += stride) bit_off[i] = (u32)(i * L);
    const int unit_f[6] = {0, 0, 3, 1, 1, 1};
    const int unit_r[6] = {2, 2, 2, 0, 3, 3};
    for (size_t w = (size_t)blockIdx.x * blockDim.x + threadIdx.x; w < plane_words; w += stride) {
        u32 h = 0, l = 0, v = 0;
        for (int b = 0; b < 32; b++) {
            u64 pos = (u64)w * 32 + b;
            if (pos >= total) break;
            u64 r = pos / L; u32 j = (u32)(pos % L);
            const u64 frag = flavor == 1 ? r >> 1 : r;
            u32 kind = synth_hash(seed, frag, 0xffffffffULL);
            u32 aux = synth_hash(seed, frag, 0xfffffffeULL);
            u32 code = synth_hash(seed, r, j) & 3u;
            bool tel = kind < tel_thr;
            bool halfk = !tel && kind < tel_thr + half_thr;
            if (halfk) tel = ((aux >> 8) & 1u) ? (j < L / 2) : (j >= L / 2);
            if (flavor == 2 && tel) {
                u32 tl = 500u + synth_hash(seed, frag, 0xfffffffdULL) % 4501u;
                if (tl > L) tl = L;
                tel = ((aux >> 9) & 1u) ? (j < tl) : (j >= L - tl);
            }
            if (tel) {
                u32 phase = aux % 6u;
                bool rc = (((aux >> 4) & 1u) ^ (flavor == 1 ? (u32)(r & 1u) : 0u)) != 0u;
                u32 idx = (j + phase) % 6u;
                u32 c = rc ? unit_r[idx] : unit_f[idx];
                u32 sh = synth_hash(seed ^ 0x5555555555555555ULL, r, j);
                code = sh < sub_thr ? (sh >> 3) & 3u : c;
            }
            bool inval = synth_hash(seed ^ 0xaaaaaaaaaaaaaaaaULL, r, j) < n_thr;
            if (!inval) { v |= 1u << b; h |= (code >> 1) << b; l |= (code & 1u) << b; }
        }
        hi[w] = h; lo[w] = l; val[w] = v;
    }
}

void launch_synth(unsigned long long seed, unsigned int n_reads, unsigned int read_len, unsigned int tel_thr,
                  unsigned int half_thr, unsigned int n_thr, unsigned int sub_thr, unsigned int flavor, unsigned int* bit_off,
                  unsigned int* hi, unsigned int* lo, unsigned int* val, size_t plane_words, cudaStream_t stream) {
    synth_kernel<<<1184, 256, 0, stream>>>(seed, n_reads, read_len, tel_thr, half_thr, n_thr, sub_thr, flavor, bit_off, hi, lo, val,
                                            plane_words);
}


struct Probe { u32 pos; int wl, k0, k1; };

__device__ __forceinline__ int unit_probes(const DevCfg& c, const DevBatch& b, u32 u, Probe* p) {
    const int MINM = c.min_mer, MAXM = c.max_mer;
    int np = 0;
    if (c.mode == 0) {
        u32 b0 = __ldg(b.bit_off + u);
        int n = (int)(__ldg(b.bit_off + u + 1) - b0);
        if (n < 2 * MINM) return 0;
        if (n >= 4 * MINM) {
            int kmax = min(n / 4, MAXM);
            p[np++] = Probe{b0, n / 2, MINM, kmax};
            p[np++] = Probe{b0 + (u32)(n - (n + 1) / 2), (n + 1) / 2, MINM, kmax};
        }
        if (4 * MAXM > n) p[np++] = Probe{b0, n, max(n / 4 + 1, MINM), min(n / 2, MAXM)};
    } else if (c.mode == 1) {
        u32 a0 = __ldg(b.bit_off + 2 * u), a1 = __ldg(b.bit_off + 2 * u + 1), a2 = __ldg(b.bit_off + 2 * u + 2);
        int n1 = (int)(a1 - a0), n2 = (int)(a2 - a1);
        int n = min(n1, n2);
        if (n < 2 * MINM) return 0;
        if (n >= 4 * MINM) {
            int kmax = min(n / 4, MAXM);
            p[np++] = Probe{a0, n1 / 2, MINM, kmax};
            p[np++] = Probe{a1, n2 / 2, MINM, kmax};
        }
        if (4 * MAXM > n) {
            int lo = max(n / 4 + 1, MINM), hi = min(n / 2, MAXM);
            p[np++] = Probe{a0, n1, lo, hi};
            p[np++] = Probe{a1, n2, lo, hi};
        }
    } else {
        u32 b0 = __ldg(b.bit_off + u);
        int n = (int)(__ldg(b.bit_off + u + 1) - b0);
        const int SL = c.slice_len;
        if (n < SL) return 0;
        int snum = n / SL, mid = (snum + 1) / 2, bonus = n % SL;
        int l1 = SL + (1 == mid ? bonus : 0);
        p[np++] = Probe{b0, l1, MINM, MAXM};
        if (snum > 1) {
            int l2 = SL + (snum == mid ? bonus : 0);
            p[np++] = Probe{b0 + (u32)(n - l2), l2, MINM, MAXM};
        }
    }
    return np;
}


template <int NW>
__device__ __forceinline__ void load_bits(const u32* __restrict__ plane, u32 pos, u32 (&out)[NW]) {
    const u32* p = plane + (pos >> 5);
    u32 sh = pos & 31;
    u32 prev = __ldg(p);
#pragma unroll
    for (int j = 0; j < NW; j++) {
        u32 nxt = __ldg(p + j + 1);
        out[j] = __funnelshift_r(prev, nxt, sh);
        prev = nxt;
    }
}

template <int NW>
__device__ __forceinline__ void mask_bits(u32 (&x)[NW], int wl) {
#pragma unroll
    for (int j = 0; j < NW; j++) {
        int v = wl - 32 * j;
        x[j] &= v <= 0 ? 0u : low_mask(v);
    }
}

template <int NW>
__device__ __forceinline__ void prefix_xor_excl(const u32 (&in)[NW], u32 (&out)[NW]) {
    u32 carry = 0, prev_top = 0;
#pragma unroll
    for (int j = 0; j < NW; j++) {
        u32 inc = prefix_xor32(in[j]) ^ carry;
        out[j] = (inc << 1) | prev_top;
        prev_top = inc >> 31;
        carry = 0u - prev_top;
    }
}

template <int NW>
__device__ __forceinline__ void shr1(u32 (&x)[NW]) {
#pragma unroll
    for (int j = 0; j < NW; j++) x[j] = __funnelshift_r(x[j], j + 1 < NW ? x[j + 1] : 0u, 1);
}

template <int NW>
__device__ __forceinline__ void shr_var(const u32 (&in)[NW], int k, u32 (&out)[NW]) {
#pragma unroll
    for (int j = 0; j < NW; j++) out[j] = in[j];
    for (int s = k >> 5; s > 0; s--) {
#pragma unroll
        for (int j = 0; j < NW; j++) out[j] = j + 1 < NW ? out[j + 1] : 0u;
    }
    u32 r = k & 31;
#pragma unroll
    for (int j = 0; j < NW; j++) out[j] = __funnelshift_r(out[j], j + 1 < NW ? out[j + 1] : 0u, r);
}

template <int NW>
__device__ __forceinline__ void sliding_and(u32 (&a)[NW], int k) {
    u32 t[NW];
    int w = 1;
    while (2 * w <= k) {
        shr_var<NW>(a, w, t);
#pragma unroll
        for (int j = 0; j < NW; j++) a[j] &= t[j];
        w *= 2;
    }
    if (k > w) {
        shr_var<NW>(a, k - w, t);
#pragma unroll
        for (int j = 0; j < NW; j++) a[j] &= t[j];
    }
}

__device__ __forceinline__ void csa(u32 a, u32 b, u32 c, u32& s, u32& cy) {
    s = a ^ b ^ c;
    cy = (a & b) | (c & (a ^ b));
}

template <int NW>
__device__ __forceinline__ int popc_multi(const u32 (&x)[NW]) {
    if constexpr (NW == 1) return __popc(x[0]);
    else if constexpr (NW == 2) return __popc(x[0]) + __popc(x[1]);
    else if constexpr (NW == 3) {
        u32 s, c; csa(x[0], x[1], x[2], s, c);
        return __popc(s) + 2 * __popc(c);
    } else if constexpr (NW == 5) {
        u32 s1, c1, s2, c2; csa(x[0], x[1], x[2], s1, c1); csa(s1, x[3], x[4], s2, c2);
        return __popc(s2) + 2 * (__popc(c1) + __popc(c2));
    } else if constexpr (NW == 8) {
        u32 s1, c1, s2, c2, s3, c3, s4, c4;
        csa(x[0], x[1], x[2], s1, c1); csa(x[3], x[4], x[5], s2, c2); csa(s1, s2, x[6], s3, c3);
        csa(c1, c2, c3, s4, c4);
        return __popc(s3) + __popc(x[7]) + 2 * __popc(s4) + 4 * __popc(c4);
    } else {
        int t = 0;
#pragma unroll
        for (int j = 0; j < NW; j++) t += __popc(x[j]);
        return t;
    }
}

template <int NW>
__device__ __noinline__ bool probe_filter(const DevBatch& b, u32 pos, int wl, int k0, int k1,
                                          const unsigned short* __restrict__ thr) {
    u32 PH[NW], PL[NW], QH[NW], QL[NW], WV[NW];
    {
        u32 t[NW];
        load_bits<NW>(b.hi, pos, t); prefix_xor_excl<NW>(t, PH);
        load_bits<NW>(b.lo, pos, t); prefix_xor_excl<NW>(t, PL);
        load_bits<NW>(b.val, pos, WV); mask_bits<NW>(WV, wl);
    }
    shr_var<NW>(PH, k0, QH);
    shr_var<NW>(PL, k0, QL);
    sliding_and<NW>(WV, k0);
    u32 PA[NW];
    bool have_pa = false;
    for (int k = k0; k <= k1; k++) {
        u32 a[NW], bb[NW], c[NW];
#pragma unroll
        for (int j = 0; j < NW; j++) {
            u32 dh = QH[j] ^ PH[j], dl = QL[j] ^ PL[j];
            a[j] = dh & WV[j]; bb[j] = dl & WV[j]; c[j] = a[j] & dl;
        }
        int T = popc_multi<NW>(WV);
        if (T == 0) break;
        int cH = popc_multi<NW>(a), cL = popc_multi<NW>(bb), c11 = popc_multi<NW>(c);
        int c10 = cH - c11, c01 = cL - c11, c00 = T - cH - cL + c11;
        int U = max(max(c00, c01), max(c10, c11));
        int need = thr[T];
        if (U >= need) {
            u32 QA[NW];
            if (!have_pa) {
                u32 A[NW], t[NW];
                load_bits<NW>(b.hi, pos, A); load_bits<NW>(b.lo, pos, t);
#pragma unroll
                for (int j = 0; j < NW; j++) A[j] &= t[j];
                prefix_xor_excl<NW>(A, PA);
                have_pa = true;
            }
            shr_var<NW>(PA, k, QA);
            u32 x11[NW], x10[NW], x01[NW], x00[NW];
#pragma unroll
            for (int j = 0; j < NW; j++) {
                u32 da = QA[j] ^ PA[j];
                u32 dh = QH[j] ^ PH[j], dl = QL[j] ^ PL[j];
                x11[j] = c[j] & da; x10[j] = a[j] & ~dl & da; x01[j] = bb[j] & ~dh & da; x00[j] = WV[j] & ~dh & ~dl & da;
            }
            int n11 = popc_multi<NW>(x11), n10 = popc_multi<NW>(x10), n01 = popc_multi<NW>(x01), n00 = popc_multi<NW>(x00);
            int U2 = max(max(max(n11, c11 - n11), max(n10, c10 - n10)), max(max(n01, c01 - n01), max(n00, c00 - n00)));
            if (U2 >= need) return true;
        }
        shr1<NW>(QH); shr1<NW>(QL);
        u32 t[NW];
#pragma unroll
        for (int j = 0; j < NW; j++) t[j] = WV[j];
        shr1<NW>(t);
#pragma unroll
        for (int j = 0; j < NW; j++) WV[j] &= t[j];
    }
    return false;
}

template <int MAXNW>
__device__ __forceinline__ bool probe_dispatch(const DevBatch& b, const Probe& p, const unsigned short* thr) {
    if (p.k1 < p.k0) return false;
    int need_bits = p.wl + 1;
    if (need_bits <= 96) return probe_filter<3>(b, p.pos, p.wl, p.k0, p.k1, thr);
    if constexpr (MAXNW >= 5) { if (need_bits <= 160) return probe_filter<5>(b, p.pos, p.wl, p.k0, p.k1, thr); }
    if constexpr (MAXNW >= 8) { if (need_bits <= 256) return probe_filter<8>(b, p.pos, p.wl, p.k0, p.k1, thr); }
    return true;
}


constexpr u32 kPackC11 = 1u - (1u << 8) - (1u << 16) + (1u << 24);
constexpr u32 kPackH = (1u << 8) - (1u << 24);
constexpr u32 kPackL = (1u << 16) - (1u << 24);
#ifndef TREW_SCREEN_UNROLL
#define TREW_SCREEN_UNROLL 2
#endif
constexpr int kScreenUnroll = TREW_SCREEN_UNROLL;
constexpr int kFastMaxWl = 95;
constexpr int kFastTabSize = kFastMaxWl + 2;
constexpr int kProbeShift = 28;
constexpr int kMod4BelowWindows = 48;
constexpr int kThreadMinWindows = 36;

__device__ __forceinline__ uint4 fast_entry(int T, int need) {
    uint4 e = make_uint4(0u, 0u, 0u, 0u);
    if (T <= 0) return e;
    int T01 = min(T, 64);
    e.y = T >= 32 ? 0xffffffffu : ((1u << T) - 1u);
    e.z = T <= 32 ? 0u : (T >= 64 ? 0xffffffffu : ((1u << (T - 32)) - 1u));
    int np = need - (T - T01);
    if (np <= 0) e.x = 0x80808080u;
    else if (np > 64) e.x = (u32)T01 << 24;
    else e.x = ((u32)T01 << 24) + (u32)(128 - np) * 0x01010101u;
    return e;
}

template <int S>
__device__ __forceinline__ bool fast_span(const u32 (&ph)[5], const u32 (&pl)[5], int wl, int ka, int kb,
                                          const uint4* __restrict__ tab) {
    const uint4* tp = tab + (wl - ka + 1);
#pragma unroll (kScreenUnroll)
    for (int k = ka; k <= kb; k++, tp--) {
        const uint4 e = *tp;
        u32 qh0 = __funnelshift_r(ph[S], ph[S + 1], k), qh1 = __funnelshift_r(ph[S + 1], ph[S + 2], k);
        u32 ql0 = __funnelshift_r(pl[S], pl[S + 1], k), ql1 = __funnelshift_r(pl[S + 1], pl[S + 2], k);
        u32 a0 = (qh0 ^ ph[0]) & e.y, a1 = (qh1 ^ ph[1]) & e.z;
        u32 b0 = (ql0 ^ pl[0]) & e.y, b1 = (ql1 ^ pl[1]) & e.z;
        u32 x = e.x + (u32)(__popc(a0) + __popc(a1)) * kPackH + (u32)(__popc(b0) + __popc(b1)) * kPackL +
                (u32)(__popc(a0 & b0) + __popc(a1 & b1)) * kPackC11;
        if (x & 0x80808080u) return true;
    }
    return false;
}

__device__ __forceinline__ bool probe_is_fast(const Probe& p) { return p.wl <= kFastMaxWl && p.k1 <= 63 && p.k1 <= p.wl; }

__device__ __forceinline__ bool screen_probe(const DevBatch& b, const Probe& p, const uint4* __restrict__ tab) {
    if (p.k1 < p.k0) return false;
    if (!probe_is_fast(p)) return true;
    u32 t[3], full[3] = {0xffffffffu, 0xffffffffu, 0xffffffffu};
    mask_bits<3>(full, p.wl);
    load_bits<3>(b.val, p.pos, t);
    if ((((t[0] & full[0]) ^ full[0]) | ((t[1] & full[1]) ^ full[1]) | ((t[2] & full[2]) ^ full[2])) != 0u) return true;
    u32 ph[5], pl[5], q[3];
    load_bits<3>(b.hi, p.pos, t); mask_bits<3>(t, p.wl); prefix_xor_excl<3>(t, q);
    ph[0] = q[0]; ph[1] = q[1]; ph[2] = q[2]; ph[3] = 0u; ph[4] = 0u;
    load_bits<3>(b.lo, p.pos, t); mask_bits<3>(t, p.wl); prefix_xor_excl<3>(t, q);
    pl[0] = q[0]; pl[1] = q[1]; pl[2] = q[2]; pl[3] = 0u; pl[4] = 0u;
    int k0 = p.k0;
    if (k0 < 32) {
        if (fast_span<0>(ph, pl, p.wl, k0, min(p.k1, 31), tab)) return true;
        k0 = 32;
    }
    return p.k1 >= 32 && fast_span<1>(ph, pl, p.wl, k0, p.k1, tab);
}

constexpr int kFastMaxWlLong = 159;
constexpr int kFastTabSizeLong = kFastMaxWlLong + 2;
struct __align__(16) FastEntryLong { u32 base, m0, m1, m2, m3, pad0, pad1, pad2; };

__device__ __forceinline__ FastEntryLong fast_entry_long(int T, int need) {
    FastEntryLong e = {0u, 0u, 0u, 0u, 0u, 0u, 0u, 0u};
    if (T <= 0) return e;
    const int T01 = min(T, 128);
    u32 m[4];
#pragma unroll
    for (int j = 0; j < 4; j++) { int vb = T - 32 * j; m[j] = vb <= 0 ? 0u : low_mask(min(32, vb)); }
    e.m0 = m[0]; e.m1 = m[1]; e.m2 = m[2]; e.m3 = m[3];
    const int np = need - (T - T01);
    if (np <= 0) e.base = 0x80808080u;
    else if (np > 128) e.base = 0u;
    else e.base = ((u32)T01 << 24) + (u32)(128 - np) * 0x01010101u;
    return e;
}

template <int S>
__device__ __forceinline__ bool fast_span_long(const u32 (&ph)[8], const u32 (&pl)[8], int wl, int ka, int kb,
                                               const FastEntryLong* __restrict__ tab) {
    const FastEntryLong* tp = tab + (wl - ka + 1);
    for (int k = ka; k <= kb; k++, tp--) {
        const uint4 e0 = *reinterpret_cast<const uint4*>(tp);
        const u32 m3 = tp->m3;
        if (e0.x == 0u) continue;
        const u32 mk[4] = {e0.y, e0.z, e0.w, m3};
        int cH = 0, cL = 0, c11 = 0;
#pragma unroll
        for (int j = 0; j < 4; j++) {
            u32 a = (__funnelshift_r(ph[S + j], ph[S + j + 1], k) ^ ph[j]) & mk[j];
            u32 bb = (__funnelshift_r(pl[S + j], pl[S + j + 1], k) ^ pl[j]) & mk[j];
            cH += __popc(a); cL += __popc(bb); c11 += __popc(a & bb);
        }
        u32 x = e0.x + (u32)cH * kPackH + (u32)cL * kPackL + (u32)c11 * kPackC11;
        if (x & 0x80808080u) return true;
    }
    return false;
}

__device__ __forceinline__ bool probe_is_fast_long(const Probe& p) { return p.wl <= kFastMaxWlLong && p.k1 <= 64 && p.k1 <= p.wl; }

__device__ __noinline__ bool screen_probe_long(const DevBatch& b, const Probe& p, const FastEntryLong* __restrict__ tab) {
    u32 t[5], full[5] = {0xffffffffu, 0xffffffffu, 0xffffffffu, 0xffffffffu, 0xffffffffu};
    mask_bits<5>(full, p.wl);
    load_bits<5>(b.val, p.pos, t);
    u32 bad = 0;
#pragma unroll
    for (int j = 0; j < 5; j++) bad |= (t[j] & full[j]) ^ full[j];
    if (bad) return true;
    u32 ph[8], pl[8], q[5];
    load_bits<5>(b.hi, p.pos, t); mask_bits<5>(t, p.wl); prefix_xor_excl<5>(t, q);
#pragma unroll
    for (int j = 0; j < 8; j++) ph[j] = j < 5 ? q[j] : 0u;
    load_bits<5>(b.lo, p.pos, t); mask_bits<5>(t, p.wl); prefix_xor_excl<5>(t, q);
#pragma unroll
    for (int j = 0; j < 8; j++) pl[j] = j < 5 ? q[j] : 0u;
    int k0 = p.k0;
    if (k0 < 32) {
        if (fast_span_long<0>(ph, pl, p.wl, k0, min(p.k1, 31), tab)) return true;
        k0 = 32;
    }
    if (k0 < 64 && p.k1 >= 32) {
        if (fast_span_long<1>(ph, pl, p.wl, k0, min(p.k1, 63), tab)) return true;
        k0 = 64;
    }
    return p.k1 >= 64 && fast_span_long<2>(ph, pl, p.wl, k0, p.k1, tab);
}

__device__ __forceinline__ void list_append(bool flag, u32 value, u32* __restrict__ list, u32* __restrict__ count) {
    u32 m = __ballot_sync(0xffffffffu, flag);
    if (m) {
        u32 base = 0;
        if (lane_id() == 0) base = atomicAdd(count, (u32)__popc(m));
        base = __shfl_sync(0xffffffffu, base, 0);
        if (flag) list[base + __popc(m & ((1u << lane_id()) - 1u))] = value;
    }
}

__device__ __forceinline__ void list_append_rev(bool flag, u32 value, u32* __restrict__ top, u32* __restrict__ count) {
    u32 m = __ballot_sync(0xffffffffu, flag);
    if (m) {
        u32 base = 0;
        if (lane_id() == 0) base = atomicAdd(count, (u32)__popc(m));
        base = __shfl_sync(0xffffffffu, base, 0);
        if (flag) *(top - (base + __popc(m & ((1u << lane_id()) - 1u)))) = value;
    }
}

#ifndef TREW_SCREEN_BPS
#define TREW_SCREEN_BPS 8
#endif
template <bool LONG>
__global__ void __launch_bounds__(256, LONG ? 4 : TREW_SCREEN_BPS) trew_screen_kernel(DevCfg cfg, DevBatch b, u32 n_units,
                                                                                     u32* __restrict__ deferred, u32* __restrict__ n_deferred) {
    __shared__ uint4 tab[kFastTabSize];
    __shared__ FastEntryLong tab_long[LONG ? kFastTabSizeLong : 1];
    for (int T = threadIdx.x; T < kFastTabSize; T += blockDim.x) tab[T] = fast_entry(T, (int)cfg.thr_low[T]);
    if (LONG) for (int T = threadIdx.x; T < kFastTabSizeLong; T += blockDim.x) tab_long[T] = fast_entry_long(T, (int)cfg.thr_low[T]);
    __syncthreads();
    u32 stride = gridDim.x * blockDim.x;
    u32 n_round = (n_units + 31u) & ~31u;
    for (u32 u = blockIdx.x * blockDim.x + threadIdx.x; u < n_round; u += stride) {
        u32 pm = 0;
        if (u < n_units) {
            Probe p[4];
            int np = unit_probes(cfg, b, u, p);
            for (int i = 0; i < np; i++) {
                bool d;
                if (LONG && p[i].k1 >= p[i].k0 && !probe_is_fast(p[i]) && probe_is_fast_long(p[i])) d = screen_probe_long(b, p[i], tab_long);
                else d = screen_probe(b, p[i], tab);
                pm |= d ? 1u << i : 0u;
            }
        }
        list_append(pm != 0, u | (pm << kProbeShift), deferred, n_deferred);
    }
}

__device__ __forceinline__ int max4(int a, int b, int c, int d) { return max(max(a, b), max(c, d)); }

__device__ __forceinline__ u32 shr3(const u32 (&p)[3], int j, int k) {
    const int s = k >> 5;
    const u32 lo = j + s < 3 ? (s ? (j == 0 ? p[1] : p[2]) : p[j]) : 0u;
    const u32 hi = j + s + 1 < 3 ? (s ? p[2] : (j == 0 ? p[1] : p[2])) : 0u;
    return __funnelshift_r(lo, hi, k);
}
constexpr int kDecideThreads = 256;
__device__ __noinline__ bool mod4_level(const DevBatch& b, u32 pos, int wl, int k, int need, u32 pass8, u32 wv0, u32 wv1, u32 wv2, u32* cache,
                                        bool& cached) {
    const u32 wv[3] = {wv0, wv1, wv2};
    u32 p0[3][3], p1[3][3];
    if (!cached) {
        u32 x[3][3];
        load_bits<3>(b.hi, pos, x[0]); mask_bits<3>(x[0], wl);
        load_bits<3>(b.lo, pos, x[1]); mask_bits<3>(x[1], wl);
#pragma unroll
        for (int j = 0; j < 3; j++) x[2][j] = x[0][j] & x[1][j];
#pragma unroll
        for (int p = 0; p < 3; p++) {
            prefix_xor_excl<3>(x[p], p0[p]);
            u32 c[3];
#pragma unroll
            for (int j = 0; j < 3; j++) c[j] = x[p][j] & p0[p][j];
            prefix_xor_excl<3>(c, p1[p]);
#pragma unroll
            for (int j = 0; j < 3; j++) { cache[(6 * p + j) * kDecideThreads] = p0[p][j]; cache[(6 * p + 3 + j) * kDecideThreads] = p1[p][j]; }
        }
        cached = true;
    } else {
#pragma unroll
        for (int p = 0; p < 3; p++)
#pragma unroll
            for (int j = 0; j < 3; j++) { p0[p][j] = cache[(6 * p + j) * kDecideThreads]; p1[p][j] = cache[(6 * p + 3 + j) * kDecideThreads]; }
    }
    u32 d0[3][3], d1[3][3];
#pragma unroll
    for (int p = 0; p < 3; p++) {
#pragma unroll
        for (int j = 0; j < 3; j++) {
            const u32 q0 = shr3(p0[p], j, k);
            d0[p][j] = q0 ^ p0[p][j];
            d1[p][j] = shr3(p1[p], j, k) ^ p1[p][j] ^ (~q0 & p0[p][j]);
        }
    }
#pragma unroll 1
    for (int c2 = 0; c2 < 8; c2++) {
        if (!((pass8 >> c2) & 1u)) continue;
        u32 mw[3];
        int cnt = 0;
#pragma unroll
        for (int j = 0; j < 3; j++) {
            mw[j] = wv[j] & (d0[0][j] ^ ((c2 & 1) ? 0u : ~0u)) & (d0[1][j] ^ ((c2 & 2) ? 0u : ~0u)) & (d0[2][j] ^ ((c2 & 4) ? 0u : ~0u));
            cnt += __popc(mw[j]);
        }
        if (cnt < need) continue;
        bool may = true;
#pragma unroll
        for (int p = 0; p < 3 && may; p++) {
            const int one = __popc(mw[0] & d1[p][0]) + __popc(mw[1] & d1[p][1]) + __popc(mw[2] & d1[p][2]);
            const int zero = cnt - one;
            if (min(one, zero) >= need) return true;
            const u32 flip = one >= zero ? 0u : ~0u;
#pragma unroll
            for (int j = 0; j < 3; j++) mw[j] &= d1[p][j] ^ flip;
            cnt = max(one, zero);
            may = cnt >= need;
        }
        if (may) return true;
    }
    return false;
}

template <int S>
__device__ __forceinline__ bool decide_span(const u32 (&ph)[5], const u32 (&pl)[5], const u32 (&pa)[5], u32 (&wv)[3], int ka, int kb,
                                            const unsigned short* __restrict__ thr, bool& done, int& t_hit, const DevBatch& bt, u32 pos, int wl,
                                            u32* cache, bool& cached, int m4_below) {
    for (int k = ka; k <= kb; k++) {
        const int T01 = __popc(wv[0]) + __popc(wv[1]), E = __popc(wv[2]), T = T01 + E;
        if (T == 0) { done = true; return false; }
        const int need = thr[T];
        u32 a0 = (__funnelshift_r(ph[S], ph[S + 1], k) ^ ph[0]) & wv[0], a1 = (__funnelshift_r(ph[S + 1], ph[S + 2], k) ^ ph[1]) & wv[1];
        u32 b0 = (__funnelshift_r(pl[S], pl[S + 1], k) ^ pl[0]) & wv[0], b1 = (__funnelshift_r(pl[S + 1], pl[S + 2], k) ^ pl[1]) & wv[1];
        int cH = __popc(a0) + __popc(a1), cL = __popc(b0) + __popc(b1), c11 = __popc(a0 & b0) + __popc(a1 & b1);
        if (max4(c11, cH - c11, cL - c11, T01 - cH - cL + c11) + E >= need) {
            u32 a2 = (__funnelshift_r(ph[S + 2], ph[S + 3], k) ^ ph[2]) & wv[2], b2 = (__funnelshift_r(pl[S + 2], pl[S + 3], k) ^ pl[2]) & wv[2];
            cH += __popc(a2); cL += __popc(b2); c11 += __popc(a2 & b2);
            const int c10 = cH - c11, c01 = cL - c11, c00 = T - cH - cL + c11;
            if (max4(c11, c10, c01, c00) >= need) {
                u32 x0 = __funnelshift_r(pa[S], pa[S + 1], k) ^ pa[0], x1 = __funnelshift_r(pa[S + 1], pa[S + 2], k) ^ pa[1];
                u32 x2 = __funnelshift_r(pa[S + 2], pa[S + 3], k) ^ pa[2];
                int n11 = __popc(a0 & b0 & x0) + __popc(a1 & b1 & x1) + __popc(a2 & b2 & x2);
                int n10 = __popc(a0 & ~b0 & x0) + __popc(a1 & ~b1 & x1) + __popc(a2 & ~b2 & x2);
                int n01 = __popc(b0 & ~a0 & x0) + __popc(b1 & ~a1 & x1) + __popc(b2 & ~a2 & x2);
                int n00 = __popc(wv[0] & ~a0 & ~b0 & x0) + __popc(wv[1] & ~a1 & ~b1 & x1) + __popc(wv[2] & ~a2 & ~b2 & x2);
                int U2 = max(max4(n11, c11 - n11, n10, c10 - n10), max4(n01, c01 - n01, n00, c00 - n00));
                if (U2 >= need) {
                    const u32 pass8 = (u32)(c00 - n00 >= need) | (u32)(c10 - n10 >= need) << 1 | (u32)(c01 - n01 >= need) << 2 |
                                      (u32)(c11 - n11 >= need) << 3 | (u32)(n00 >= need) << 4 | (u32)(n10 >= need) << 5 |
                                      (u32)(n01 >= need) << 6 | (u32)(n11 >= need) << 7;
                    if (T >= m4_below || mod4_level(bt, pos, wl, k, need, pass8, wv[0], wv[1], wv[2], cache, cached)) { t_hit = T; return true; }
                }
            }
        }
        u32 t0 = __funnelshift_r(wv[0], wv[1], 1), t1 = __funnelshift_r(wv[1], wv[2], 1), t2 = wv[2] >> 1;
        wv[0] &= t0; wv[1] &= t1; wv[2] &= t2;
    }
    return false;
}

__device__ __noinline__ bool decide_short(const DevBatch& b, u32 pos, int wl, int k0, int k1, const unsigned short* __restrict__ thr, int& t_hit,
                                          u32* cache, int m4_below) {
    bool cached = false;
    u32 wv[3], ph[5], pl[5], pa[5];
    load_bits<3>(b.val, pos, wv); mask_bits<3>(wv, wl);
    {
        u32 h[3], l[3], q[3];
        load_bits<3>(b.hi, pos, h); mask_bits<3>(h, wl); prefix_xor_excl<3>(h, q);
        ph[0] = q[0]; ph[1] = q[1]; ph[2] = q[2]; ph[3] = 0u; ph[4] = 0u;
        load_bits<3>(b.lo, pos, l); mask_bits<3>(l, wl); prefix_xor_excl<3>(l, q);
        pl[0] = q[0]; pl[1] = q[1]; pl[2] = q[2]; pl[3] = 0u; pl[4] = 0u;
#pragma unroll
        for (int j = 0; j < 3; j++) h[j] &= l[j];
        prefix_xor_excl<3>(h, q);
        pa[0] = q[0]; pa[1] = q[1]; pa[2] = q[2]; pa[3] = 0u; pa[4] = 0u;
    }
    sliding_and<3>(wv, k0);
    bool done = false;
    if (k0 < 32) {
        if (decide_span<0>(ph, pl, pa, wv, k0, min(k1, 31), thr, done, t_hit, b, pos, wl, cache, cached, m4_below)) return true;
        if (done) return false;
        k0 = 32;
    }
    return k1 >= 32 && decide_span<1>(ph, pl, pa, wv, k0, k1, thr, done, t_hit, b, pos, wl, cache, cached, m4_below);
}

template <int MAXNW>
__global__ void __launch_bounds__(kDecideThreads, (MAXNW <= 5 ? 4 : 2)) trew_filter_kernel(DevCfg cfg, DevBatch b, const u32* __restrict__ units,
                                                          const u32* __restrict__ n_units_ptr, u32 n_units_all,
                                                          u32* __restrict__ survivors, u32* __restrict__ n_survivors,
                                                          u32* __restrict__ surv_b_top, u32* __restrict__ n_surv_b, int thread_min_windows, int third_level,
                                                          u32* __restrict__ work_counter) {
    __shared__ unsigned short thr[kThrTableSize];
    __shared__ u32 s_m4[18 * kDecideThreads];
    for (int i = threadIdx.x; i < kThrTableSize; i += blockDim.x) thr[i] = cfg.thr_low[i];
    __syncthreads();
    const u32 n_units = units ? *n_units_ptr : n_units_all;
    const bool pack_probes = n_units_all < (1u << kProbeShift);
    const u32 lane = lane_id();
    bool have = false, maybe = false, exhausted = false;
    u32 u = 0, live = 0, todo = 0;
    int t_hit = 1 << 20;
    Probe p[4];
    for (;;) {
        const u32 idle = __ballot_sync(0xffffffffu, !have);
        if (idle != 0u && !exhausted) {
            u32 base = 0;
            if (lane == 0) base = atomicAdd(work_counter, (u32)__popc(idle));
            base = __shfl_sync(0xffffffffu, base, 0);
            exhausted = base + (u32)__popc(idle) >= n_units;
            const u32 i = base + (u32)__popc(idle & ((1u << lane) - 1u));
            if (!have && i < n_units) {
                u32 pm = 0xfu;
                u = i;
                if (units) { const u32 e = units[i]; u = e & ((1u << kProbeShift) - 1u); pm = e >> kProbeShift; }
                const int np = unit_probes(cfg, b, u, p);
                live = todo = pm & ((1u << np) - 1u);
                maybe = false; t_hit = 1 << 20; have = true;
            }
        }
        if (__ballot_sync(0xffffffffu, have) == 0u) break;
        if (have && todo != 0u) {
            const int j = __ffs(todo) - 1;
            todo &= todo - 1u;
            if (p[j].k1 >= p[j].k0)
                maybe = probe_is_fast(p[j]) ? decide_short(b, p[j].pos, p[j].wl, p[j].k0, p[j].k1, thr, t_hit, s_m4 + threadIdx.x, third_level)
                                            : probe_dispatch<MAXNW>(b, p[j], thr);
            if (!maybe) live &= ~(1u << j);
        }
        const bool fin = have && (todo == 0u || maybe);
        const bool keep = fin && maybe;
        const u32 entry = pack_probes ? u | (live << kProbeShift) : u;
        if (surv_b_top == nullptr) {
            list_append(keep, entry, survivors, n_survivors);
        } else {
            bool to_b = false;
            if (keep) {
                int len;
                if (cfg.mode == 1) {
                    const u32 a0 = __ldg(b.bit_off + 2 * u), a1 = __ldg(b.bit_off + 2 * u + 1), a2 = __ldg(b.bit_off + 2 * u + 2);
                    len = (int)max(a1 - a0, a2 - a1);
                } else {
                    len = (int)(__ldg(b.bit_off + u + 1) - __ldg(b.bit_off + u));
                }
                to_b = len > et::kMaxRead || t_hit < thread_min_windows;
            }
            list_append(keep && !to_b, entry, survivors, n_survivors);
            list_append_rev(keep && to_b, entry, surv_b_top, n_surv_b);
        }
        if (fin) have = false;
    }
}

void launch_filter(const DevCfg& cfg, const DevBatch& b, unsigned int n_units, unsigned int max_read_len,
                   unsigned int* deferred, unsigned int* n_deferred, unsigned int* survivors, unsigned int* n_survivors,
                   const LaunchPlan& plan, cudaStream_t stream, cudaEvent_t after_screen, unsigned int* surv_b_top,
                   unsigned int* n_surv_b, unsigned int* work_counter) {
    if (n_units == 0) return;
    unsigned int longest;
    if (cfg.mode == 2) longest = 2u * (unsigned)cfg.slice_len;
    else longest = (max_read_len < 4u * (unsigned)cfg.max_mer) ? max_read_len : (max_read_len + 1) / 2;
    unsigned int need = (n_units + 255) / 256;
    const bool screen = deferred != nullptr && !(cfg.mode == 2 && cfg.slice_len > kFastMaxWlLong) && n_units < (1u << kProbeShift);
    if (screen) {
        int blocks = plan.screen_blocks;
        if ((unsigned)blocks > need) blocks = (int)need;
        if (longest <= (unsigned)kFastMaxWl) trew_screen_kernel<false><<<blocks, 256, 0, stream>>>(cfg, b, n_units, deferred, n_deferred);
        else trew_screen_kernel<true><<<blocks, 256, 0, stream>>>(cfg, b, n_units, deferred, n_deferred);
    }
    if (after_screen) cudaEventRecord(after_screen, stream);
    static const int tmw = [] { const char* e = getenv("TREW_THREAD_MIN_WINDOWS"); return e && *e ? atoi(e) : kThreadMinWindows; }();
    static const int m4_on = [] { const char* e = getenv("TREW_MOD4_BELOW"); return e && *e ? atoi(e) : kMod4BelowWindows; }();
    const unsigned int* list = screen ? deferred : nullptr;
    int blocks = plan.decide_blocks;
    if ((unsigned)blocks > need) blocks = (int)need;
    if (longest + 1 <= 96) trew_filter_kernel<3><<<blocks, 256, 0, stream>>>(cfg, b, list, n_deferred, n_units, survivors, n_survivors, surv_b_top, n_surv_b, tmw, m4_on, work_counter);
    else if (longest + 1 <= 160) trew_filter_kernel<5><<<blocks, 256, 0, stream>>>(cfg, b, list, n_deferred, n_units, survivors, n_survivors, surv_b_top, n_surv_b, tmw, m4_on, work_counter);
    else trew_filter_kernel<8><<<blocks, 256, 0, stream>>>(cfg, b, list, n_deferred, n_units, survivors, n_survivors, surv_b_top, n_surv_b, tmw, m4_on, work_counter);
}


extern __shared__ __align__(16) unsigned char g_smem[];

constexpr int kPlaneWords = 36;
#ifndef TREW_EXACT_BPS
#define TREW_EXACT_BPS 8
#endif
#ifndef TREW_EXACT_WARPS
#define TREW_EXACT_WARPS 4
#endif
constexpr int kExactWarps = TREW_EXACT_WARPS;
constexpr u32 kEmptySlot = 0xffffffffu;
constexpr int kSerialMaxRuns = 12;

enum { HD_CUR_POS = 0, HD_CUR_LEN, HD_ALLVALID, HD_EV_POS, HD_EV_LEN, HD_EV_K, HD_EV_PACK, HD_S = 8 ,
       HD_BLK_L = 12 , HD_BLK_H = 14 , HD_NEED_L = 16, HD_NEED_H = 17, HD_BLK64 = 18, HD_RES = 19,
       HD_SH = 20 , HD_SL = 24  };
constexpr int kHeaderBytes = 128;

__host__ __device__ inline int exact_hash_slots(int cap) {
    int hs = 64;
    while (hs < cap + cap / 4) hs <<= 1;
    return hs;
}

__host__ __device__ inline size_t exact_warp_bytes(int cap) {
    size_t b = kHeaderBytes + 5 * kPlaneWords * sizeof(u32) + kPlaneWords * sizeof(u64);
    b += (size_t)2 * cap * sizeof(u64) + (size_t)exact_hash_slots(cap) * sizeof(u32) + (size_t)2 * cap * sizeof(u32);
    b += (size_t)(3 * cap + 4) * sizeof(unsigned short);
    return (b + 15) & ~(size_t)15;
}

size_t exact_smem_bytes(int run_cap, bool) { return exact_warp_bytes(run_cap) * kExactWarps; }

struct WS {
    u32 off; int cap; int hs; u32 lane; u32 flags;
    __device__ __forceinline__ u32* hdr() const { return (u32*)(g_smem + off); }
    __device__ __forceinline__ u32* H() const { return (u32*)(g_smem + off + kHeaderBytes); }
    __device__ __forceinline__ u32* L() const { return H() + kPlaneWords; }
    __device__ __forceinline__ u32* V() const { return H() + 2 * kPlaneWords; }
    __device__ __forceinline__ u32* PH() const { return H() + 3 * kPlaneWords; }
    __device__ __forceinline__ u32* PL() const { return H() + 4 * kPlaneWords; }
    __device__ __forceinline__ u64* rev2() const { return (u64*)(H() + 5 * kPlaneWords); }
    __device__ __forceinline__ u64* run_lo() const { return rev2() + kPlaneWords; }
    __device__ __forceinline__ u64* run_hi() const { return run_lo() + cap; }
    __device__ __forceinline__ u32* htab() const { return (u32*)(run_hi() + cap); }
    __device__ __forceinline__ u32* grp_tot() const { return htab() + hs; }
    __device__ __forceinline__ u32* grp_last() const { return grp_tot() + cap; }
    __device__ __forceinline__ unsigned short* run_start() const { return (unsigned short*)(grp_last() + cap); }
    __device__ __forceinline__ unsigned short* run_cw() const { return run_start() + cap; }
    __device__ __forceinline__ unsigned short* run_total() const { return run_cw() + cap + 4; }
};

struct TableRef { Slot* slots; u32 mask; u32* err; };

struct ScanRes { int th, tl; u64 sh_lo, sh_hi, sl_lo, sl_hi; };

__device__ __forceinline__ int pk_T(u32 p) { return (int)(p & 1023u); }
__device__ __forceinline__ int pk_M(u32 p) { return (int)((p >> 10) & 1023u); }
__device__ __forceinline__ int pk_runs(u32 p) { return (int)((p >> 20) & 1023u); }
__device__ __forceinline__ bool pk_homo(u32 p) { return ((p >> 30) & 1u) != 0; }


__device__ __noinline__ u64 canon64(u64 w, int k) {
    int sh = 2 * (k - 1);
    if (k <= 16) {
        u32 b32 = (u32)w, c32 = (u32)w;
        for (int r = 1; r < k; r++) {
            c32 = ((c32 & 3u) << sh) | (c32 >> 2);
            b32 = min(b32, c32);
        }
        return b32;
    }
    u64 best = w, cur = w;
    for (int r = 1; r < k; r++) {
        cur = ((cur & 3ULL) << sh) | (cur >> 2);
        best = cur < best ? cur : best;
    }
    return best;
}

__device__ __noinline__ u128 canon128(u128 w, int k) {
    u128 best = w, cur = w;
    int sh = 2 * (k - 1);
    for (int r = 1; r < k; r++) {
        cur = ((cur & 3) << sh) | (cur >> 2);
        best = cur < best ? cur : best;
    }
    return best;
}

__device__ __forceinline__ u64 rev_pairs64(u64 x) {
    x = __brevll(x);
    return ((x >> 1) & 0x5555555555555555ULL) | ((x & 0x5555555555555555ULL) << 1);
}

__device__ __forceinline__ void canon_pair(u64& lo, u64& hi, int k) {
    if (k <= 32) { lo = canon64(lo, k); hi = 0; }
    else { u128 c = canon128(((u128)hi << 64) | lo, k); lo = (u64)c; hi = (u64)(c >> 64); }
}

__device__ __forceinline__ void crc_pair(u64& lo, u64& hi, int k) {
    if (k <= 32) {
        u64 r = ~rev_pairs64(lo) >> (64 - 2 * k);
        lo = canon64(r, k); hi = 0;
    } else {
        u128 r = ((u128)(~rev_pairs64(lo)) << 64) | (u128)(~rev_pairs64(hi));
        r >>= (128 - 2 * k);
        u128 c = canon128(r, k); lo = (u64)c; hi = (u64)(c >> 64);
    }
}

__device__ __forceinline__ bool homo_pair(u64 lo, u64 hi, int k) {
    if (k <= 1) return true;
    if (k <= 32) return ((lo ^ (lo >> 2)) & ((1ULL << (2 * (k - 1))) - 1ULL)) == 0;
    u128 w = ((u128)hi << 64) | lo;
    u128 m = (((u128)1 << (2 * (k - 1))) - 1);
    return ((w ^ (w >> 2)) & m) == 0;
}

__device__ __forceinline__ bool less_pair(u64 alo, u64 ahi, u64 blo, u64 bhi) {
    return ahi < bhi || (ahi == bhi && alo < blo);
}

__device__ __forceinline__ u32 shfl_next_bit0(u32 x, u32 lane) {
    u32 nx = __shfl_down_sync(0xffffffffu, x, 1);
    return lane == 31 ? 0u : (nx & 1u);
}


__device__ __noinline__ void load_window(WS ws, const u32* __restrict__ bhi, const u32* __restrict__ blo,
                                         const u32* __restrict__ bval, u32 pos, int len) {
    u32* hd = ws.hdr();
    if ((int)hd[HD_CUR_LEN] == len && hd[HD_CUR_POS] == pos) return;
    __syncwarp();
    const u32 lane = ws.lane;
    int vbits = len - 32 * (int)lane;
    u32 msk = vbits <= 0 ? 0u : low_mask(vbits);
    u32 h = 0, l = 0, v = 0;
    if (vbits > 0) {
        u32 wi = (pos >> 5) + lane, sh = pos & 31;
        h = __funnelshift_r(__ldg(bhi + wi), __ldg(bhi + wi + 1), sh) & msk;
        l = __funnelshift_r(__ldg(blo + wi), __ldg(blo + wi + 1), sh) & msk;
        v = __funnelshift_r(__ldg(bval + wi), __ldg(bval + wi + 1), sh) & msk;
    }
    const bool all_valid = __all_sync(0xffffffffu, v == msk);
    u32 ih = prefix_xor32(h), il = prefix_xor32(l);
    u32 bh = __ballot_sync(0xffffffffu, ih >> 31), bl = __ballot_sync(0xffffffffu, il >> 31);
    u32 lt = (1u << lane) - 1u;
    if (__popc(bh & lt) & 1) ih = ~ih;
    if (__popc(bl & lt) & 1) il = ~il;
    u32 ph_prev = __shfl_up_sync(0xffffffffu, ih, 1), pl_prev = __shfl_up_sync(0xffffffffu, il, 1);
    u32 ph = (ih << 1) | (lane ? ph_prev >> 31 : 0u);
    u32 pl = (il << 1) | (lane ? pl_prev >> 31 : 0u);
    u32 *H = ws.H(), *L = ws.L(), *V = ws.V(), *PH = ws.PH(), *PL = ws.PL();
    u64* rev2 = ws.rev2();
    H[lane] = h; L[lane] = l; V[lane] = v; PH[lane] = ph; PL[lane] = pl;
    if (lane < kPlaneWords - 32) {
        H[32 + lane] = 0; L[32 + lane] = 0; V[32 + lane] = 0; PH[32 + lane] = 0; PL[32 + lane] = 0;
        rev2[32 + lane] = 0;
    }
    __syncwarp();
    {
        int cs = len - 32 * (int)lane - 32;
        u32 hb = 0, lb = 0;
        if (cs > -32) {
            if (cs >= 0) {
                int wi = cs >> 5, sh = cs & 31;
                hb = __funnelshift_r(H[wi], H[wi + 1], sh);
                lb = __funnelshift_r(L[wi], L[wi + 1], sh);
            } else {
                hb = H[0] << (-cs);
                lb = L[0] << (-cs);
            }
        }
        hb = __brev(hb); lb = __brev(lb);
        u64 x = hb, y = lb;
        x = (x | (x << 16)) & 0x0000FFFF0000FFFFULL; y = (y | (y << 16)) & 0x0000FFFF0000FFFFULL;
        x = (x | (x << 8)) & 0x00FF00FF00FF00FFULL;  y = (y | (y << 8)) & 0x00FF00FF00FF00FFULL;
        x = (x | (x << 4)) & 0x0F0F0F0F0F0F0F0FULL;  y = (y | (y << 4)) & 0x0F0F0F0F0F0F0F0FULL;
        x = (x | (x << 2)) & 0x3333333333333333ULL;  y = (y | (y << 2)) & 0x3333333333333333ULL;
        x = (x | (x << 1)) & 0x5555555555555555ULL;  y = (y | (y << 1)) & 0x5555555555555555ULL;
        rev2[lane] = (x << 1) | y;
    }
    if (lane == 0) { hd[HD_CUR_POS] = pos; hd[HD_CUR_LEN] = (u32)len; hd[HD_ALLVALID] = all_valid ? 1u : 0u; }
    __syncwarp();
}

__device__ __forceinline__ void kmer_at(const u64* __restrict__ rev2, int len, int i, int k, u64& lo, u64& hi) {
    int o = 2 * (len - i - k);
    int wi = o >> 6, sh = o & 63;
    u64 a = rev2[wi], b = rev2[wi + 1];
    lo = sh ? (a >> sh) | (b << (64 - sh)) : a;
    if (k <= 32) {
        if (k < 32) lo &= (1ULL << (2 * k)) - 1ULL;
        hi = 0;
    } else {
        u64 c = rev2[wi + 2];
        hi = sh ? (b >> sh) | (c << (64 - sh)) : b;
        if (k < 64) hi &= (1ULL << (2 * k - 64)) - 1ULL;
    }
}

__device__ __forceinline__ u32 wv_for_k(WS ws, int len, int k) {
    const u32 lane = ws.lane;
    if (ws.hdr()[HD_ALLVALID]) {
        int vb = len - k + 1 - 32 * (int)lane;
        return vb <= 0 ? 0u : low_mask(min(32, vb));
    }
    u32 wv = ws.V()[lane];
    for (int t = 1; t < k; t++) {
        u32 nb = shfl_next_bit0(wv, lane);
        wv &= (wv >> 1) | (nb << 31);
    }
    return wv;
}

__device__ __forceinline__ u32 wv_step(u32 wv, u32 lane) {
    u32 nb = shfl_next_bit0(wv, lane);
    return wv & ((wv >> 1) | (nb << 31));
}

__device__ __forceinline__ int bound_k(WS ws, int k, u32 wv, int T) {
    const u32 lane = ws.lane;
    const u32 *PH = ws.PH(), *PL = ws.PL();
    int s = k >> 5, r = k & 31;
    u32 qh = __funnelshift_r(PH[lane + s], PH[lane + s + 1], r);
    u32 ql = __funnelshift_r(PL[lane + s], PL[lane + s + 1], r);
    u32 dh = (qh ^ PH[lane]) & wv, dl = (ql ^ PL[lane]) & wv;
    u32 packed = (u32)__popc(dh) | ((u32)__popc(dl) << 10) | ((u32)__popc(dh & dl) << 20);
    packed = __reduce_add_sync(0xffffffffu, packed);
    int cH = packed & 1023, cL = (packed >> 10) & 1023, c11 = packed >> 20;
    int c10 = cH - c11, c01 = cL - c11, c00 = T - cH - cL + c11;
    return max(max(c00, c01), max(c10, c11));
}

__device__ __noinline__ int comp_bound(WS ws, int k, u32 wv, int T) {
    const u32 lane = ws.lane;
    const u32 cnt = (u32)__popc(wv);
    u32 inc = cnt;
#pragma unroll
    for (int d = 1; d < 32; d <<= 1) {
        u32 t = __shfl_up_sync(0xffffffffu, inc, d);
        if ((int)lane >= d) inc += t;
    }
    unsigned short* pos = ws.run_start();
    {
        u32 rb = inc - cnt, x = wv;
        while (x) {
            int bit = __ffs(x) - 1;
            x &= x - 1;
            pos[rb++] = (unsigned short)(32 * lane + bit);
        }
    }
    __syncwarp();
    const bool act = (int)lane < T;
    u32 key = 0;
    if (act) {
        const u32 *H = ws.H(), *L = ws.L();
        const int p = pos[lane], w0 = p >> 5, o = p & 31;
        const u32 m0 = low_mask(min(k, 32)), m1 = k <= 32 ? 0u : low_mask(k - 32);
        const u32 h0 = __funnelshift_r(H[w0], H[w0 + 1], o) & m0, h1 = __funnelshift_r(H[w0 + 1], H[w0 + 2], o) & m1;
        const u32 l0 = __funnelshift_r(L[w0], L[w0 + 1], o) & m0, l1 = __funnelshift_r(L[w0 + 1], L[w0 + 2], o) & m1;
        key = (u32)(__popc(h0) + __popc(h1)) | ((u32)(__popc(l0) + __popc(l1)) << 8) | ((u32)(__popc(h0 & l0) + __popc(h1 & l1)) << 16);
    }
    const u32 actm = __ballot_sync(0xffffffffu, act);
    const u32 same = __match_any_sync(0xffffffffu, key) & actm;
    const u32 best = __reduce_max_sync(0xffffffffu, act ? (u32)__popc(same) : 0u);
    __syncwarp();
    return (int)best;
}

__device__ __noinline__ u32 eval_k(WS ws, int len, int k, u32 wv) {
    const u32 lane = ws.lane;
    u32* hd = ws.hdr();
    const u32 *H = ws.H(), *L = ws.L();
    int s = k >> 5, r = k & 31;
    u32 hs = __funnelshift_r(H[lane + s], H[lane + s + 1], r);
    u32 ls = __funnelshift_r(L[lane + s], L[lane + s + 1], r);
    u32 eq = ~((hs ^ H[lane]) | (ls ^ L[lane]));
    u32 nb = shfl_next_bit0(wv, lane);
    u32 link = eq & wv & ((wv >> 1) | (nb << 31));
    u32 link_prev = __shfl_up_sync(0xffffffffu, link, 1);
    u32 rs = wv & ~((link << 1) | (lane ? link_prev >> 31 : 0u));
    u32 pk = (u32)__popc(wv) | ((u32)__popc(rs) << 16);
    const u32 tot_pk = __reduce_add_sync(0xffffffffu, pk);
    const int T = (int)(tot_pk & 0xffffu), R = (int)(tot_pk >> 16);
    if (T == 0) return 0u;
    unsigned short *run_start = ws.run_start(), *run_cw = ws.run_cw(), *run_total = ws.run_total();
    u64 *run_lo = ws.run_lo(), *run_hi = ws.run_hi();
    u32 *htab = ws.htab(), *grp_tot = ws.grp_tot(), *grp_last = ws.grp_last();
    const u64* rev2 = ws.rev2();
    const bool wide = k > 32;
    if (!wide && R <= kSerialMaxRuns && (ws.flags & 1u)) {
        u32* scr = htab;
        scr[lane] = wv; scr[32 + lane] = link; scr[64 + lane] = rs;
        __syncwarp();
        unsigned short* cls_last = run_cw;
        int ncls = 0, ord = 0;
        const int nw = (len + 31) >> 5;
        for (int j = 0; j < nw; j++) {
// ... 259 lines not shown
                    u32 a0 = __shfl_sync(0xffffffffu, wvv[0], bit), a1 = __shfl_sync(0xffffffffu, wvv[1], bit);
                    u32 a2 = __shfl_sync(0xffffffffu, wvv[2], bit), a3 = __shfl_sync(0xffffffffu, wvv[3], bit);
                    wv = lane == 0 ? a0 : lane == 1 ? a1 : lane == 2 ? a2 : lane == 3 ? a3 : 0u;
                }
                if (try_k(ws, thr_low, low, high, pos, len, kb + bit, Uk, Tk, wv) && cm) {
                    bool still = false;
                    if (T > 0 && k <= 64)
                        still = (!blocked_k(hd, HD_BLK_L, k) && need_pre(low, hd[HD_NEED_L], U, T)) ||
                                (!blocked_k(hd, HD_BLK_H, k) && need_pre(high, hd[HD_NEED_H], U, T));
                    cm &= __ballot_sync(0xffffffffu, still);
                }
            }
        }
        return hd[HD_RES];
    }

    u32 wv = wv_for_k(ws, len, kmin);
    for (int k = kmin; k <= kmax; k++, wv = wv_step(wv, lane)) {
        int T = (int)__reduce_add_sync(0xffffffffu, (u32)__popc(wv));
        if (T == 0) break;
        int U = bound_k(ws, k, wv, T);
        try_k(ws, thr_low, low, high, pos, len, k, U, T, wv);
    }
    return hd[HD_RES];
}

__device__ __forceinline__ ScanRes scan_stats(WS ws, const DevBatch& b, u32 pos, int len, int kmin, int kmax, const DevCfg& cfg) {
    const u32 r = scan_core(ws, b, pos, len, kmin, kmax, cfg.thr_low, cfg.low, cfg.high);
    const u32* hd = ws.hdr();
    ScanRes res;
    res.th = (int)(r & 0xffu); res.tl = (int)(r >> 8);
    res.sh_lo = (u64)hd[HD_SH] | ((u64)hd[HD_SH + 1] << 32); res.sh_hi = (u64)hd[HD_SH + 2] | ((u64)hd[HD_SH + 3] << 32);
    res.sl_lo = (u64)hd[HD_SL] | ((u64)hd[HD_SL + 1] << 32); res.sl_hi = (u64)hd[HD_SL + 2] | ((u64)hd[HD_SL + 3] << 32);
    return res;
}

__device__ __noinline__ u32 eval_cached(WS ws, DevBatch b, u32 pos, int len, int k) {
    u32* hd = ws.hdr();
    if ((int)hd[HD_EV_K] == k && hd[HD_EV_POS] == pos && (int)hd[HD_EV_LEN] == len) return hd[HD_EV_PACK];
    load_window(ws, b.hi, b.lo, b.val, pos, len);
    u32 wv = wv_for_k(ws, len, k);
    u32 ev = eval_k(ws, len, k, wv);
    if (ws.lane == 0) { hd[HD_EV_POS] = pos; hd[HD_EV_LEN] = (u32)len; hd[HD_EV_K] = (u32)k; hd[HD_EV_PACK] = ev; }
    __syncwarp();
    return ev;
}

__device__ void emit_window(TableRef tr, WS ws, const DevBatch& b, u32 pos, int len, int k, int table, bool folded) {
    u32 ev = eval_cached(ws, b, pos, len, k);
    emit_classes(tr, ws, k, pk_runs(ev), table, folded);
}

__device__ void target_window(TableRef tr, WS ws, const DevBatch& b, u32 pos, int len, int k, const unsigned short* thr_low, bool high, int table) {
    u32 ev = eval_cached(ws, b, pos, len, k);
    if (pk_T(ev) > 0 && !pk_homo(ev) && pk_M(ev) >= thr_at(ws, thr_low, high, pk_T(ev))) emit_classes(tr, ws, k, pk_runs(ev), table, true);
}


enum { T_F = 0, T_B = 2, T_O = 4 };

__device__ void route_short(const DevCfg& cfg, TableRef tr, WS ws, const DevBatch& b, u32 u, u32 pm) {
    const int MINM = cfg.min_mer, MAXM = cfg.max_mer;
    u32 b0 = __ldg(b.bit_off + u);
    int n = (int)(__ldg(b.bit_off + u + 1) - b0);
    if (n < 2 * MINM || n > kMaxWindow) return;
    int L[2] = {0, 0}, R[2] = {0, 0};
    if (n >= 4 * MINM) {
        int kmax = min(n / 4, MAXM);
        u32 lpos = b0, rpos = b0 + (u32)(n - (n + 1) / 2);
        int llen = n / 2, rlen = (n + 1) / 2;
        if (pm & 1u) { ScanRes l = scan_stats(ws, b, lpos, llen, MINM, kmax, cfg); L[0] = l.th; L[1] = l.tl; }
        if (pm & 2u) { ScanRes r = scan_stats(ws, b, rpos, rlen, MINM, kmax, cfg); R[0] = r.th; R[1] = r.tl; }
        pm >>= 2;
#pragma unroll
        for (int c = 0; c < 2; c++) {
            if (L[c] > 0 && L[c] == R[c]) target_window(tr, ws, b, b0, n, L[c], cfg.thr_low, c == 0, T_O + c);
            else if (L[c] > 0) emit_window(tr, ws, b, lpos, llen, L[c], T_F + c, false);
            else if (R[c] > 0) emit_window(tr, ws, b, rpos, rlen, R[c], T_B + c, false);
        }
    }
    bool hc[2] = {L[0] == 0 && R[0] == 0, L[1] == 0 && R[1] == 0};
    if (4 * MAXM > n && (hc[0] || hc[1]) && (pm & 1u)) {
        ScanRes s = scan_stats(ws, b, b0, n, max(n / 4 + 1, MINM), min(n / 2, MAXM), cfg);
        if (hc[0] && s.th) emit_window(tr, ws, b, b0, n, s.th, T_O + 0, false);
        if (hc[1] && s.tl) emit_window(tr, ws, b, b0, n, s.tl, T_O + 1, false);
    }
}

__device__ void route_pair(const DevCfg& cfg, TableRef tr, WS ws, const DevBatch& b, u32 u) {
    const int MINM = cfg.min_mer, MAXM = cfg.max_mer;
    u32 a0 = __ldg(b.bit_off + 2 * u), a1 = __ldg(b.bit_off + 2 * u + 1), a2 = __ldg(b.bit_off + 2 * u + 2);
    int n1 = (int)(a1 - a0), n2 = (int)(a2 - a1);
    int n = min(n1, n2);
    if (n < 2 * MINM || n1 > kMaxWindow || n2 > kMaxWindow) return;
    int lef[2] = {0, 0}, km[2] = {0, 0};
    if (n >= 4 * MINM) {
        u32 spos[5] = {0, a0, a0 + (u32)(n1 - (n1 + 1) / 2), a1 + (u32)(n2 - (n2 + 1) / 2), a1};
        int slen[5] = {0, n1 / 2, (n1 + 1) / 2, (n2 + 1) / 2, n2 / 2};
        int kmax = min(n / 4, MAXM);
        ScanRes sr[5]; bool have[5] = {false, false, false, false, false};
        int pseg[2][8], ptmp[2][8], np[2] = {0, 0};
        int si[2] = {1, 1}; bool ended[2] = {false, false};
        u64 ks_lo[2] = {0, 0}, ks_hi[2] = {0, 0};
        for (int ti = 1; ti <= 4 && !(ended[0] && ended[1]); ti++) {
            if (!have[ti]) { sr[ti] = scan_stats(ws, b, spos[ti], slen[ti], MINM, kmax, cfg); have[ti] = true; }
            int k[2] = {sr[ti].th, sr[ti].tl};
            u64 slo[2] = {sr[ti].sh_lo, sr[ti].sl_lo}, shi[2] = {sr[ti].sh_hi, sr[ti].sl_hi};
#pragma unroll
            for (int c = 0; c < 2; c++) {
                if (!ended[c] && k[c]) { pseg[c][np[c]] = ti; ptmp[c][np[c]] = ti <= 2 ? 0 : 1; np[c]++; }
                bool ok = !ended[c] && k[c] > 0;
                if (ok && ti != 1) {
                    u64 dlo = slo[c], dhi = shi[c];
                    if (ti > 2) crc_pair(dlo, dhi, k[c]);
                    ok = km[c] == k[c] && ks_lo[c] == dlo && ks_hi[c] == dhi;
                }
                if (ok) { si[c]++; km[c] = k[c]; if (ti == 1) { ks_lo[c] = slo[c]; ks_hi[c] = shi[c]; } }
                else ended[c] = true;
            }
        }
        lef[0] = km[0]; lef[1] = km[1];
#pragma unroll
        for (int c = 0; c < 2; c++) {
            if (si[c] == 5) {
                for (int e = 0; e < np[c]; e++) {
                    int sg = pseg[c][e];
                    emit_window(tr, ws, b, spos[sg], slen[sg], c == 0 ? sr[sg].th : sr[sg].tl, T_O + c, true);
                }
            }
        }
        if (si[0] <= 4 || si[1] <= 4) {
            int sj[2] = {4, 4}; km[0] = km[1] = 0; ended[0] = ended[1] = false;
            for (int tj = 4; tj >= 1 && !(ended[0] && ended[1]); tj--) {
                if (!have[tj]) { sr[tj] = scan_stats(ws, b, spos[tj], slen[tj], MINM, kmax, cfg); have[tj] = true; }
                int k[2] = {sr[tj].th, sr[tj].tl};
                u64 slo[2] = {sr[tj].sh_lo, sr[tj].sl_lo}, shi[2] = {sr[tj].sh_hi, sr[tj].sl_hi};
#pragma unroll
                for (int c = 0; c < 2; c++) {
                    if (!ended[c] && k[c]) { pseg[c][np[c]] = tj; ptmp[c][np[c]] = tj <= 2 ? 1 : 0; np[c]++; }
                    bool ok = sj[c] >= si[c] && !ended[c] && k[c] > 0;
                    if (ok && tj != 4) {
                        u64 dlo = slo[c], dhi = shi[c];
                        if (tj <= 2) crc_pair(dlo, dhi, k[c]);
                        ok = km[c] == k[c] && ks_lo[c] == dlo && ks_hi[c] == dhi;
                    }
                    if (ok) { sj[c]--; km[c] = k[c]; if (tj == 4) { ks_lo[c] = slo[c]; ks_hi[c] = shi[c]; } }
                    else ended[c] = true;
                }
            }
        }
#pragma unroll
        for (int c = 0; c < 2; c++) {
            if (si[c] <= 4) {
                for (int e = 0; e < np[c]; e++) {
                    int sg = pseg[c][e];
                    emit_window(tr, ws, b, spos[sg], slen[sg], c == 0 ? sr[sg].th : sr[sg].tl,
                                (ptmp[c][e] == 0 ? T_F : T_B) + c, false);
                }
            }
        }
    }
    if (4 * MAXM > n && (lef[0] == 0 || lef[1] == 0 || km[0] == 0 || km[1] == 0)) {
        int lo = max(n / 4 + 1, MINM), hi = min(n / 2, MAXM);
        ScanRes l, r; l.th = l.tl = r.th = r.tl = 0; l.sh_lo = l.sh_hi = l.sl_lo = l.sl_hi = 0; r = l;
        if (lef[0] == 0 || lef[1] == 0) l = scan_stats(ws, b, a0, n1, lo, hi, cfg);
        if (km[0] == 0 || km[1] == 0) r = scan_stats(ws, b, a1, n2, lo, hi, cfg);
        int ltk[2] = {l.th, l.tl}, rtk[2] = {r.th, r.tl};
        u64 llo[2] = {l.sh_lo, l.sl_lo}, lhi[2] = {l.sh_hi, l.sl_hi}, rlo[2] = {r.sh_lo, r.sl_lo}, rhi[2] = {r.sh_hi, r.sl_hi};
#pragma unroll
        for (int c = 0; c < 2; c++) {
            bool el = lef[c] == 0 && ltk[c] > 0, er = km[c] == 0 && rtk[c] > 0;
            bool both = lef[c] == 0 && km[c] == 0 && ltk[c] == rtk[c] && ltk[c] > 0;
            if (both) {
                u64 dlo = rlo[c], dhi = rhi[c];
                crc_pair(dlo, dhi, rtk[c]);
                both = llo[c] == dlo && lhi[c] == dhi;
            }
            if (both) {
                if (el) emit_window(tr, ws, b, a0, n1, ltk[c], T_O + c, true);
                if (er) emit_window(tr, ws, b, a1, n2, rtk[c], T_O + c, true);
            }
            if (el) emit_window(tr, ws, b, a0, n1, ltk[c], T_F + c, false);
            if (er) emit_window(tr, ws, b, a1, n2, rtk[c], T_F + c, false);
        }
    }
}

__device__ void route_long(const DevCfg& cfg, TableRef tr, WS ws, const DevBatch& b, u32 u, unsigned char* scratch) {
    const int MINM = cfg.min_mer, MAXM = cfg.max_mer, SL = cfg.slice_len;
    u32 b0 = __ldg(b.bit_off + u);
    int n = (int)(__ldg(b.bit_off + u + 1) - b0);
    if (n < SL) return;
    int snum = n / SL, mid = (snum + 1) / 2, bonus = n % SL;
    auto s_start = [&](int t) { return (u32)((t - 1) * SL + (t > mid ? bonus : 0)); };
    auto s_len = [&](int t) { return SL + (t == mid ? bonus : 0); };
    int si[2] = {1, 1}, km[2] = {0, 0}; bool ended[2] = {false, false};
    int nf = 0;
    for (int ti = 1; ti <= snum && !(ended[0] && ended[1]); ti++) {
        ScanRes sr = scan_stats(ws, b, b0 + s_start(ti), s_len(ti), MINM, MAXM, cfg);
        if (ws.lane == 0) { scratch[2 * (ti - 1)] = (unsigned char)sr.th; scratch[2 * (ti - 1) + 1] = (unsigned char)sr.tl; }
        int k[2] = {sr.th, sr.tl};
#pragma unroll
        for (int c = 0; c < 2; c++) {
            if (!ended[c] && k[c] > 0 && (ti == 1 || km[c] == k[c])) { si[c]++; km[c] = k[c]; }
            else ended[c] = true;
        }
        nf = ti;
    }
    __syncwarp();
    {
        bool en[2] = {false, false}; int kk[2] = {0, 0};
        bool full[2] = {si[0] == snum + 1, si[1] == snum + 1};
        for (int ti = 1; ti <= nf; ti++) {
            int k[2] = {scratch[2 * (ti - 1)], scratch[2 * (ti - 1) + 1]};
#pragma unroll
            for (int c = 0; c < 2; c++) {
                if (!en[c] && k[c]) emit_window(tr, ws, b, b0 + s_start(ti), s_len(ti), k[c], (full[c] ? T_O : T_F) + c, full[c]);
                if (!en[c] && k[c] > 0 && (ti == 1 || kk[c] == k[c])) kk[c] = k[c];
                else en[c] = true;
            }
        }
    }
    if (si[0] <= snum || si[1] <= snum) {
        int sj[2] = {snum, snum}; km[0] = km[1] = 0; ended[0] = ended[1] = false;
        for (int tj = snum; tj >= 1 && !(ended[0] && ended[1]); tj--) {
            ScanRes sr = scan_stats(ws, b, b0 + s_start(tj), s_len(tj), MINM, MAXM, cfg);
            int k[2] = {sr.th, sr.tl};
#pragma unroll
            for (int c = 0; c < 2; c++) {
                if (!ended[c] && k[c]) emit_window(tr, ws, b, b0 + s_start(tj), s_len(tj), k[c], T_B + c, false);
                if (sj[c] >= si[c] && !ended[c] && k[c] > 0 && (tj == snum || km[c] == k[c])) { sj[c]--; km[c] = k[c]; }
                else ended[c] = true;
            }
        }
    }
}


constexpr int kStageSlots = 256;
constexpr int kStageProbes = 6;
constexpr u32 kStageLock = 0xffffffffu;

struct StageEmit {
    u32* s_meta; u32* s_cnt; u64* s_key;
    Slot* slots; u32 mask; u32* err;
    __device__ __forceinline__ void operator()(int table, int k, et::u128 key, u64 count) const {
        const u64 hi = (u64)(key >> 64);
        if (hi) table_add_impl(slots, mask, err, ((u32)table << 8) | (u32)k, (u64)key, hi, count);
        else (*this)(table, k, (et::u64)key, count);
    }
    __device__ __forceinline__ void operator()(int table, int k, et::u64 key_, u64 count) const {
        const u64 key = (u64)key_;
        const u32 meta = ((u32)table << 8) | (u32)k, tag = meta | 0x80000000u;
        u32 i = (u32)(mix64(key ^ ((u64)meta << 53)) >> 40) & (kStageSlots - 1);
        bool done = false;
        for (int p = 0; p < kStageProbes && !done; p++, i = (i + 1) & (kStageSlots - 1)) {
            int outcome = 0;
            do {
                const u32 st = atomicCAS(&s_meta[i], 0u, kStageLock);
                if (st == 0u) {
                    s_key[i] = key;
                    __threadfence_block();
                    atomicExch(&s_meta[i], tag);
                    atomicAdd(&s_cnt[i], (u32)count);
                    outcome = 1;
                } else if (st != kStageLock) {
                    __threadfence_block();
                    if (st == tag && *(volatile u64*)&s_key[i] == key) { atomicAdd(&s_cnt[i], (u32)count); outcome = 1; }
                    else outcome = 2;
                }
            } while (outcome == 0);
            done = outcome == 1;
        }
        if (!done) table_add_impl(slots, mask, err, meta, key, 0ULL, count);
    }
};

#ifndef TREW_THREAD_BLOCK
#define TREW_THREAD_BLOCK 128
#endif
template <class K>
constexpr size_t thread_kernel_smem() { return (size_t)et::Lay<K>::WORDS * TREW_THREAD_BLOCK * sizeof(u32) + (size_t)kStageSlots * 16; }
constexpr size_t kThreadKernelSmem = thread_kernel_smem<et::u64>();
template <int MODE, class K>
constexpr int thread_kernel_bps() { return (sizeof(K) == 8 ? 6 : 5) - (MODE == 1 ? 1 : 0); }

struct PlaneLoad {
    et::Mem m; const u32 *hi, *lo, *val; u32 b0[2];
    __device__ __forceinline__ void operator()(int mate, int off, int len) const {
        const u32 pos = b0[mate] + (u32)off, w0 = pos >> 5, sh = pos & 31u;
        for (int j = 0; j < et::kReadWords + 2; j++) {
            const u32 msk = low_mask(min(32, max(0, len - 32 * j)));
            u32 h = 0u, l = 0u;
            if (msk) {
                h = __funnelshift_r(__ldg(hi + w0 + j), __ldg(hi + w0 + j + 1), sh) & msk;
                l = __funnelshift_r(__ldg(lo + w0 + j), __ldg(lo + w0 + j + 1), sh) & msk;
            }
            m[et::W_H + j] = h; m[et::W_L + j] = l;
            if (j < et::kReadWords) m[et::W_V + j] = msk ? __funnelshift_r(__ldg(val + w0 + j), __ldg(val + w0 + j + 1), sh) & msk : 0u;
        }
    }
};

template <int MODE, class K>
__global__ void __launch_bounds__(TREW_THREAD_BLOCK, (thread_kernel_bps<MODE, K>())) trew_exact_thread_kernel(DevCfg cfg, DevBatch b, const u32* __restrict__ survivors,
                                                                              const u32* __restrict__ n_survivors, int packed_probes,
                                                                              u32* __restrict__ hard, u32* __restrict__ n_hard,
                                                                              unsigned long long* total_survivors, u32* work_counter) {
    u32* work = reinterpret_cast<u32*>(g_smem);
    u64* s_key = reinterpret_cast<u64*>(work + et::Lay<K>::WORDS * TREW_THREAD_BLOCK);
    u32* s_meta = reinterpret_cast<u32*>(s_key + kStageSlots);
    u32* s_cnt = s_meta + kStageSlots;
    for (int i = threadIdx.x; i < kStageSlots; i += blockDim.x) { s_meta[i] = 0u; s_cnt[i] = 0u; }
    __syncthreads();
    const et::Mem m{work + threadIdx.x, TREW_THREAD_BLOCK};
    const u32 n = *n_survivors;
    if (blockIdx.x == 0 && threadIdx.x == 0 && total_survivors) atomicAdd(total_survivors, (unsigned long long)n);
    StageEmit emit{s_meta, s_cnt, s_key, cfg.slots, cfg.slot_mask, cfg.error_flag};
    for (;;) {
        u32 base = 0;
        if (lane_id() == 0) base = atomicAdd(work_counter, 32u);
        base = __shfl_sync(0xffffffffu, base, 0);
        if (base >= n) break;
        const u32 i = base + lane_id();
        bool bail = false;
        u32 entry = 0;
        if (i < n) {
            entry = survivors[i];
            u32 u = entry, pm = 3u;
            if (packed_probes) { pm = entry >> kProbeShift; u &= (1u << kProbeShift) - 1u; }
            if (MODE == 0) {
                const u32 b0 = __ldg(b.bit_off + u);
                const int len = (int)(__ldg(b.bit_off + u + 1) - b0);
                if (len > et::kMaxRead) {
                    bail = true;
                } else {
                    PlaneLoad load{m, b.hi, b.lo, b.val, {b0, 0u}};
                    bail = !et::route_short_thread<K>(m, len, pm & 7u, cfg.min_mer, cfg.max_mer, cfg.thr_low, cfg.thr_high, load, emit);
                }
            } else {
                const u32 a0 = __ldg(b.bit_off + 2 * u), a1 = __ldg(b.bit_off + 2 * u + 1), a2 = __ldg(b.bit_off + 2 * u + 2);
                const int n1 = (int)(a1 - a0), n2 = (int)(a2 - a1);
                PlaneLoad load{m, b.hi, b.lo, b.val, {a0, a1}};
                bail = !et::route_pair_thread<K>(m, n1, n2, cfg.min_mer, cfg.max_mer, cfg.thr_low, cfg.thr_high, load, emit);
            }
        }
        list_append(bail, entry, hard, n_hard);
    }
    __syncthreads();
    for (int i = threadIdx.x; i < kStageSlots; i += blockDim.x) {
        const u32 st = s_meta[i], c = s_cnt[i];
        if (st != 0u && st != kStageLock && c != 0u) table_add_impl(cfg.slots, cfg.slot_mask, cfg.error_flag, st & 0x7fffffffu, s_key[i], 0ULL, (u64)c);
    }
}


struct LongArgs {
    const u32* survivors; const u32* n_survivors; int packed_probes;
    u32 s_cap, max_slices;
    unsigned short* stats; u32* emis;
    u32* hard; u32* n_hard;
    unsigned long long* total_survivors;
};

__global__ void __launch_bounds__(TREW_THREAD_BLOCK, 4) trew_long_stats_kernel(DevCfg cfg, DevBatch b, LongArgs a) {
    u32* work = reinterpret_cast<u32*>(g_smem);
    const et::Mem m{work + threadIdx.x, TREW_THREAD_BLOCK};
    const u32 n = min(*a.n_survivors, a.s_cap);
    const u32 warps = gridDim.x * (blockDim.x >> 5), lane = lane_id();
    et::ClsSpill<et::u64> x;
    for (u32 idx = blockIdx.x * (blockDim.x >> 5) + (threadIdx.x >> 5); idx < n; idx += warps) {
        u32 u = a.survivors[idx];
        if (a.packed_probes) u &= (1u << kProbeShift) - 1u;
        const u32 b0 = __ldg(b.bit_off + u);
        const int len = (int)(__ldg(b.bit_off + u + 1) - b0);
        if (len < cfg.slice_len) continue;
        const et::LongGeom g(len, cfg.slice_len);
        PlaneLoad load{m, b.hi, b.lo, b.val, {b0, 0u}};
        unsigned short* row = a.stats + (size_t)idx * (a.max_slices + 1);
        for (int t = 1 + (int)lane; t <= g.snum; t += 32) {
            u32 r = 0;
            if (g.len(t) <= et::kMaxRead) r = et::long_slice_stats(m, g, t, cfg.min_mer, cfg.max_mer, cfg.thr_low, cfg.thr_high, load, x);
            row[t] = (unsigned short)r;
        }
    }
}

__global__ void __launch_bounds__(256) trew_long_walk_kernel(DevCfg cfg, DevBatch b, LongArgs a) {
    const u32 n_all = *a.n_survivors;
    if (blockIdx.x == 0 && threadIdx.x == 0 && a.total_survivors) atomicAdd(a.total_survivors, (unsigned long long)n_all);
    const u32 stride = gridDim.x * blockDim.x, n_round = (n_all + 31u) & ~31u;
    for (u32 idx = blockIdx.x * blockDim.x + threadIdx.x; idx < n_round; idx += stride) {
        bool bail = false;
        u32 entry = 0;
        if (idx < n_all) {
            entry = a.survivors[idx];
            u32 u = entry;
            if (a.packed_probes) u &= (1u << kProbeShift) - 1u;
            const int len = (int)(__ldg(b.bit_off + u + 1) - __ldg(b.bit_off + u));
            if (idx >= a.s_cap) bail = len >= cfg.slice_len;
            else if (len >= cfg.slice_len) {
                const et::LongGeom g(len, cfg.slice_len);
                const unsigned short* row = a.stats + (size_t)idx * (a.max_slices + 1);
                u32* em = a.emis + (size_t)idx * (a.max_slices + 1);
                for (int t = 1; t <= g.snum; t++) em[t] = 0u;
                auto stat = [&](int t) { return (u32)row[t]; };
                auto task = [&](const et::LongTask& tk) {
                    const int tb = tk.table_folded & 7, c = tb & 1;
                    const bool backward = (tb & 6) == et::T_B;
                    const u32 byte = (u32)tk.k | ((tk.table_folded & 8) ? 0x80u : 0u);
                    em[tk.slice] |= byte << (8 * ((backward ? 2 : 0) + c));
                };
                bail = !et::long_walk(g, stat, task);
                if (bail) for (int t = 1; t <= g.snum; t++) em[t] = 0u;
            }
        }
        list_append(bail, entry, a.hard, a.n_hard);
    }
}

__global__ void __launch_bounds__(TREW_THREAD_BLOCK, 4) trew_long_emit_kernel(DevCfg cfg, DevBatch b, LongArgs a) {
    u32* work = reinterpret_cast<u32*>(g_smem);
    u64* s_key = reinterpret_cast<u64*>(work + et::Lay<et::u64>::WORDS * TREW_THREAD_BLOCK);
    u32* s_meta = reinterpret_cast<u32*>(s_key + kStageSlots);
    u32* s_cnt = s_meta + kStageSlots;
    for (int i = threadIdx.x; i < kStageSlots; i += blockDim.x) { s_meta[i] = 0u; s_cnt[i] = 0u; }
    __syncthreads();
    const et::Mem m{work + threadIdx.x, TREW_THREAD_BLOCK};
    StageEmit emit{s_meta, s_cnt, s_key, cfg.slots, cfg.slot_mask, cfg.error_flag};
    const u32 n = min(*a.n_survivors, a.s_cap);
    const u32 warps = gridDim.x * (blockDim.x >> 5), lane = lane_id();
    et::ClsSpill<et::u64> x;
    for (u32 idx = blockIdx.x * (blockDim.x >> 5) + (threadIdx.x >> 5); idx < n; idx += warps) {
        u32 u = a.survivors[idx];
        if (a.packed_probes) u &= (1u << kProbeShift) - 1u;
        const u32 b0 = __ldg(b.bit_off + u);
        const int len = (int)(__ldg(b.bit_off + u + 1) - b0);
        if (len < cfg.slice_len) continue;
        const et::LongGeom g(len, cfg.slice_len);
        PlaneLoad load{m, b.hi, b.lo, b.val, {b0, 0u}};
        const u32* em = a.emis + (size_t)idx * (a.max_slices + 1);
        for (int t = 1 + (int)lane; t <= g.snum; t += 32) {
            const u32 e = em[t];
            if (e == 0u) continue;
            for (int f = 0; f < 4; f++) {
                const u32 byte = (e >> (8 * f)) & 0xffu;
                if (byte == 0u) continue;
                const int c = f & 1;
                const bool folded = (byte & 0x80u) != 0u;
                const int table = (f >= 2 ? et::T_B : (folded ? et::T_O : et::T_F)) + c;
                et::LongTask tk{(unsigned short)t, (unsigned char)(byte & 0x7fu), (unsigned char)(table | (folded ? 8 : 0))};
                et::long_emit(m, g, tk, load, x, emit);
            }
        }
    }
    __syncthreads();
    for (int i = threadIdx.x; i < kStageSlots; i += blockDim.x) {
        const u32 st = s_meta[i], c = s_cnt[i];
        if (st != 0u && st != kStageLock && c != 0u) table_add_impl(cfg.slots, cfg.slot_mask, cfg.error_flag, st & 0x7fffffffu, s_key[i], 0ULL, (u64)c);
    }
}

bool long_thread_path_applies(const DevCfg& cfg) { return cfg.mode == 2 && cfg.max_mer <= 32 && cfg.slice_len <= et::kMaxRead; }

size_t long_thread_scratch_bytes(unsigned int s_cap, unsigned int max_slices) {
    return (size_t)s_cap * (max_slices + 1) * (sizeof(unsigned short) + sizeof(u32)) + 64;
}

void launch_long_thread(const DevCfg& cfg, const DevBatch& b, const unsigned int* survivors, const unsigned int* n_survivors,
                        int packed_probes, unsigned int s_cap, unsigned int max_slices, unsigned char* scratch, unsigned int* hard,
                        unsigned int* n_hard, unsigned long long* total_survivors, int sm_count, cudaStream_t stream) {
    LongArgs a{};
    a.survivors = survivors; a.n_survivors = n_survivors; a.packed_probes = packed_probes;
    a.s_cap = s_cap; a.max_slices = max_slices;
    a.emis = reinterpret_cast<u32*>(scratch);
    a.stats = reinterpret_cast<unsigned short*>(scratch + (size_t)s_cap * (max_slices + 1) * sizeof(u32));
    a.hard = hard; a.n_hard = n_hard; a.total_survivors = total_survivors;
    const size_t smem_stats = (size_t)et::Lay<et::u64>::WORDS * TREW_THREAD_BLOCK * sizeof(u32);
    trew_long_stats_kernel<<<sm_count * 4, TREW_THREAD_BLOCK, smem_stats, stream>>>(cfg, b, a);
    trew_long_walk_kernel<<<sm_count * 2, 256, 0, stream>>>(cfg, b, a);
    trew_long_emit_kernel<<<sm_count * 4, TREW_THREAD_BLOCK, kThreadKernelSmem, stream>>>(cfg, b, a);
}

bool thread_path_applies(const DevCfg& cfg, unsigned int max_read_len) {
    if (cfg.max_mer > 64) return false;
    if (cfg.mode == 0) return true;
    return cfg.mode == 1 && max_read_len >= 4u * (unsigned)cfg.max_mer;
}

void launch_exact_thread(const DevCfg& cfg, const DevBatch& b, const unsigned int* survivors, const unsigned int* n_survivors,
                         int packed_probes, unsigned int* hard, unsigned int* n_hard, unsigned long long* total_survivors, int sm_count,
                         int blocks_per_sm, unsigned int* work_counter, cudaStream_t stream) {
    const bool wide = cfg.max_mer > 32;
#define TREW_LAUNCH_THREAD(MODE, K)                                                                                               \
    trew_exact_thread_kernel<MODE, K><<<sm_count * (blocks_per_sm > 0 ? blocks_per_sm : thread_kernel_bps<MODE, K>()),            \
                                        TREW_THREAD_BLOCK, thread_kernel_smem<K>(), stream>>>(                                    \
        cfg, b, survivors, n_survivors, packed_probes, hard, n_hard, total_survivors, work_counter)
    if (cfg.mode == 0) { if (wide) TREW_LAUNCH_THREAD(0, et::u128); else TREW_LAUNCH_THREAD(0, et::u64); }
    else               { if (wide) TREW_LAUNCH_THREAD(1, et::u128); else TREW_LAUNCH_THREAD(1, et::u64); }
#undef TREW_LAUNCH_THREAD
}

template <int MODE>
__global__ void __launch_bounds__(kExactWarps * 32, TREW_EXACT_BPS) trew_exact_kernel(DevCfg cfg, DevBatch b, ExactArgs a) {
    const int wid = threadIdx.x >> 5;
    const u32 lane = lane_id();
    WS ws;
    ws.cap = a.run_cap; ws.hs = exact_hash_slots(a.run_cap);
    ws.off = (u32)((size_t)wid * exact_warp_bytes(a.run_cap)); ws.lane = lane; ws.flags = a.exp_flags;
    TableRef tr{cfg.slots, cfg.slot_mask, cfg.error_flag};
    ws.hdr()[lane] = lane == HD_CUR_LEN || lane == HD_EV_LEN || lane == HD_EV_K ? 0xffffffffu : 0u;
    __syncwarp();
    const u32 n = *a.n_survivors;
    if (blockIdx.x == 0 && threadIdx.x == 0 && a.total_survivors) atomicAdd(a.total_survivors, (u64)n);
    unsigned char* scratch = a.slice_scratch + (size_t)(blockIdx.x * kExactWarps + wid) * a.slice_scratch_stride;
    for (;;) {
        u32 idx = 0;
        if (lane == 0) idx = atomicAdd(a.work_counter, 1u);
        idx = __shfl_sync(0xffffffffu, idx, 0);
        if (idx >= n) break;
        u32 u = a.reverse ? *(a.survivors - idx) : a.survivors[idx], pm = 0xfu;
        if (a.packed_probes) { pm = u >> kProbeShift; u &= (1u << kProbeShift) - 1u; }
        if constexpr (MODE == 0) route_short(cfg, tr, ws, b, u, pm);
        else if constexpr (MODE == 1) route_pair(cfg, tr, ws, b, u);
        else route_long(cfg, tr, ws, b, u, scratch);
    }
}

constexpr int kExactBlocksPerSM = TREW_EXACT_BPS;
int exact_warps_total(int sm_count) { return sm_count * kExactBlocksPerSM * kExactWarps; }

cudaError_t prepare_exact(int run_cap_max) {
    int bytes = (int)exact_smem_bytes(run_cap_max, true);
    cudaError_t e = cudaFuncSetAttribute(trew_exact_kernel<0>, cudaFuncAttributeMaxDynamicSharedMemorySize, bytes);
    if (e == cudaSuccess) e = cudaFuncSetAttribute(trew_exact_kernel<1>, cudaFuncAttributeMaxDynamicSharedMemorySize, bytes);
    if (e == cudaSuccess) e = cudaFuncSetAttribute(trew_exact_kernel<2>, cudaFuncAttributeMaxDynamicSharedMemorySize, bytes);
    if (e == cudaSuccess) e = cudaFuncSetAttribute(trew_exact_thread_kernel<0, et::u64>, cudaFuncAttributeMaxDynamicSharedMemorySize, (int)thread_kernel_smem<et::u64>());
    if (e == cudaSuccess) e = cudaFuncSetAttribute(trew_exact_thread_kernel<1, et::u64>, cudaFuncAttributeMaxDynamicSharedMemorySize, (int)thread_kernel_smem<et::u64>());
    if (e == cudaSuccess) e = cudaFuncSetAttribute(trew_exact_thread_kernel<0, et::u128>, cudaFuncAttributeMaxDynamicSharedMemorySize, (int)thread_kernel_smem<et::u128>());
    if (e == cudaSuccess) e = cudaFuncSetAttribute(trew_exact_thread_kernel<1, et::u128>, cudaFuncAttributeMaxDynamicSharedMemorySize, (int)thread_kernel_smem<et::u128>());
    if (e == cudaSuccess) e = cudaFuncSetAttribute(trew_long_stats_kernel, cudaFuncAttributeMaxDynamicSharedMemorySize, (int)kThreadKernelSmem);
    if (e == cudaSuccess) e = cudaFuncSetAttribute(trew_long_emit_kernel, cudaFuncAttributeMaxDynamicSharedMemorySize, (int)kThreadKernelSmem);
    return e;
}

LaunchPlan default_launch_plan(int sm_count) { return LaunchPlan{sm_count * 128, sm_count * 4, sm_count * kExactBlocksPerSM}; }

void launch_exact(const DevCfg& cfg, const DevBatch& b, const ExactArgs& a, const LaunchPlan& plan, cudaStream_t stream) {
    size_t smem = exact_smem_bytes(a.run_cap, true);
    dim3 grid(plan.exact_blocks), block(kExactWarps * 32);
    if (cfg.mode == 0) trew_exact_kernel<0><<<grid, block, smem, stream>>>(cfg, b, a);
    else if (cfg.mode == 1) trew_exact_kernel<1><<<grid, block, smem, stream>>>(cfg, b, a);
    else trew_exact_kernel<2><<<grid, block, smem, stream>>>(cfg, b, a);
}

}
```

trew_b200/csrc/scan_kernels.cuh:

```cuda
#pragma once
#include <cstdint>
#include <cuda_runtime.h>

#include "../../include/trew_b200.h"

namespace trew {

constexpr int kThrTableSize = 1025;
constexpr int kMaxWindow = 1023;

struct __align__(32) Slot {
    unsigned long long seq_lo;
    unsigned long long seq_hi;
    unsigned long long count;
    unsigned int meta;
    unsigned int state;
};

struct DevCfg {
    int mode, min_mer, max_mer, slice_len;
    double low, high;
    Slot* slots;
    unsigned int slot_mask;
    unsigned int* error_flag;
    const unsigned short* thr_low;
    const unsigned short* thr_high;
};

struct DevBatch {
    unsigned int n_reads;
    const unsigned int* bit_off;
    const unsigned int* hi;
    const unsigned int* lo;
    const unsigned int* val;
};

struct ExactArgs {
    const unsigned int* survivors;
    const unsigned int* n_survivors;
    unsigned int* work_counter;
    unsigned char* slice_scratch;
    unsigned int slice_scratch_stride;
    int run_cap;
    unsigned long long* total_survivors;
    int packed_probes;
    int reverse;
    unsigned int exp_flags;
};

struct LaunchPlan { int screen_blocks, decide_blocks, exact_blocks; };
LaunchPlan default_launch_plan(int sm_count);

void launch_filter(const DevCfg& cfg, const DevBatch& b, unsigned int n_units, unsigned int max_read_len,
                   unsigned int* deferred, unsigned int* n_deferred, unsigned int* survivors, unsigned int* n_survivors,
                   const LaunchPlan& plan, cudaStream_t stream, cudaEvent_t after_screen,
                   unsigned int* surv_b_top, unsigned int* n_surv_b, unsigned int* work_counter);
size_t exact_smem_bytes(int run_cap, bool wide);
cudaError_t prepare_exact(int run_cap_max);
void launch_exact(const DevCfg& cfg, const DevBatch& b, const ExactArgs& a, const LaunchPlan& plan, cudaStream_t stream);
int exact_warps_total(int sm_count);
bool long_thread_path_applies(const DevCfg& cfg);
size_t long_thread_scratch_bytes(unsigned int s_cap, unsigned int max_slices);
void launch_long_thread(const DevCfg& cfg, const DevBatch& b, const unsigned int* survivors, const unsigned int* n_survivors,
                        int packed_probes, unsigned int s_cap, unsigned int max_slices, unsigned char* scratch, unsigned int* hard,
                        unsigned int* n_hard, unsigned long long* total_survivors, int sm_count, cudaStream_t stream);
bool thread_path_applies(const DevCfg& cfg, unsigned int max_read_len);
void launch_exact_thread(const DevCfg& cfg, const DevBatch& b, const unsigned int* survivors, const unsigned int* n_survivors,
                         int packed_probes, unsigned int* hard, unsigned int* n_hard, unsigned long long* total_survivors, int sm_count,
                         int blocks_per_sm, unsigned int* work_counter, cudaStream_t stream);
void launch_compact(const Slot* slots, unsigned int n_slots, trew_entry* out, unsigned int* d_n, cudaStream_t stream, unsigned int cap);
cudaError_t sort_entries_radix(const trew_entry* d_entries, trew_entry* d_out, unsigned int n, bool wide, void* d_temp,
                               size_t* temp_bytes, cudaStream_t stream);
cudaError_t combine_sorted_rows(const trew_entry* d_sorted, unsigned int n, trew_entry* d_out, unsigned int* d_n_out, void* d_temp,
                                size_t* temp_bytes, cudaStream_t stream);
cudaError_t filter_report_rows(const trew_entry* d_rows, unsigned int n, unsigned int min_total, trew_entry* d_out, unsigned int* d_n_out,
                               void* d_temp, size_t* temp_bytes, cudaStream_t stream);
void launch_clear_invalid(unsigned int* val, const unsigned int* rec, unsigned int n, cudaStream_t stream);
void launch_merge_entries(const DevCfg& cfg, const trew_entry* entries, unsigned int n, cudaStream_t stream);

void launch_synth(unsigned long long seed, unsigned int n_reads, unsigned int read_len, unsigned int tel_thr,
                  unsigned int half_thr, unsigned int n_thr, unsigned int sub_thr, unsigned int flavor, unsigned int* bit_off,
                  unsigned int* hi, unsigned int* lo, unsigned int* val, size_t plane_words, cudaStream_t stream);

}
```

Baseline: 984.4.

## Pipeline screen of next resident batch with survivor stages of previous batch

Measured after the change: 1047, median of 6. 6.4% higher.

```diff
diff --git a/trew_b200/csrc/device_ctx.cu b/trew_b200/csrc/device_ctx.cu
--- a/trew_b200/csrc/device_ctx.cu
+++ b/trew_b200/csrc/device_ctx.cu
@@ -47,18 +47,19 @@
     unsigned int* d_counters = nullptr;
     unsigned char* d_scratch = nullptr;
     size_t scratch_bytes = 0;
-    cudaEvent_t ev[4] = {nullptr, nullptr, nullptr, nullptr};
+    bool screened = false;
+    cudaEvent_t ev[5] = {nullptr, nullptr, nullptr, nullptr, nullptr};
     bool ev_pending = false;
 };
 
 struct trew_ctx {
     trew_config cfg{};
     int sm_count = 0;
+    ScanShape shape{};
     LaunchPlan plan{};
     cudaStream_t aux_stream = nullptr;
     cudaEvent_t ev_join = nullptr;
-    int resident_streams = 1;
-    uint64_t resident_seq = 0;
+    trew_resident* pending = nullptr;
     DevCfg dcfg{};
     size_t n_slots = 0;
     unsigned int* d_error = nullptr;
@@ -150,14 +151,23 @@
 
 constexpr int kScanCounters = 8;
 
-static int env_blocks_thread() {
-    static const int v = [] { const char* e = getenv("TREW_GRID_THREAD"); int x = e && *e ? atoi(e) : 0; return x > 0 ? x : 0; }();
-    return v;
-}
-
-int launch_scan(trew_ctx* ctx, const DevBatch& b, uint32_t n_units, uint32_t max_read_len, unsigned int* d_survivors,
-                unsigned int* d_counters, unsigned char** d_scratch, size_t* scratch_bytes, cudaStream_t st,
-                cudaEvent_t* ev = nullptr) {
+constexpr int kPipeScreenRoom = 2;
+
+int launch_screen_stage(trew_ctx* ctx, const DevBatch& b, uint32_t n_units, uint32_t max_read_len, unsigned int* d_survivors,
+                        unsigned int* d_counters, const LaunchPlan& plan, cudaStream_t st, bool* screened, cudaEvent_t* ev = nullptr) {
+    ctx->export_valid = false;
+    CK(cudaMemsetAsync(d_counters, 0, kScanCounters * sizeof(unsigned int), st));
+    if (ev) CK(cudaEventRecord(ev[0], st));
+    *screened = launch_screen(ctx->dcfg, b, n_units, max_read_len, d_survivors + n_units, d_counters + 2, plan, st);
+    if (ev) CK(cudaEventRecord(ev[1], st));
+    CK(cudaGetLastError());
+    ctx->stats.kernel_launches += *screened ? 1 : 0;
+    return TREW_OK;
+}
+
+int launch_survivor_stage(trew_ctx* ctx, const DevBatch& b, uint32_t n_units, uint32_t max_read_len, unsigned int* d_survivors,
+                          unsigned int* d_counters, unsigned char** d_scratch, size_t* scratch_bytes, bool screened,
+                          const LaunchPlan& plan, cudaStream_t st, cudaEvent_t* ev = nullptr) {
     unsigned int stride, s_cap, max_slices;
     size_t long_off;
     size_t need = scratch_need(ctx, max_read_len, n_units, &stride, &long_off, &s_cap, &max_slices);
@@ -166,14 +176,11 @@
         CK(cudaMalloc((void**)d_scratch, need));
         *scratch_bytes = need;
     }
-    ctx->export_valid = false;
-    CK(cudaMemsetAsync(d_counters, 0, kScanCounters * sizeof(unsigned int), st));
-    if (ev) CK(cudaEventRecord(ev[0], st));
+    if (ev) CK(cudaEventRecord(ev[2], st));
     const bool thread_path = thread_path_applies(ctx->dcfg, max_read_len) && !(ctx->exact_flags & 4u) && n_units < (1u << 28);
-    launch_filter(ctx->dcfg, b, n_units, max_read_len, d_survivors + n_units, d_counters + 2, d_survivors, d_counters, ctx->plan, st,
-                  ev ? ev[1] : nullptr, thread_path ? d_survivors + n_units - 1 : nullptr, thread_path ? d_counters + 4 : nullptr,
-                  d_counters + 7);
-    if (ev) CK(cudaEventRecord(ev[2], st));
+    launch_decide(ctx->dcfg, b, n_units, max_read_len, screened ? d_survivors + n_units : nullptr, d_counters + 2, d_survivors, d_counters,
+                  plan, st, thread_path ? d_survivors + n_units - 1 : nullptr, thread_path ? d_counters + 4 : nullptr, d_counters + 7);
+    if (ev) CK(cudaEventRecord(ev[3], st));
     ExactArgs a{};
     a.survivors = d_survivors; a.n_survivors = d_counters; a.work_counter = d_counters + 1;
     a.slice_scratch = *d_scratch; a.slice_scratch_stride = stride; a.run_cap = run_cap_for(ctx->cfg, max_read_len);
@@ -183,24 +190,32 @@
     if (thread_path) {
         unsigned int* hard = d_survivors + n_units;
         launch_exact_thread(ctx->dcfg, b, d_survivors, d_counters, a.packed_probes, hard, d_counters + 3, ctx->d_total_surv,
-                            ctx->sm_count, env_blocks_thread(), d_counters + 6, st);
+                            plan, d_counters + 6, st);
         ExactArgs ab = a;
         ab.survivors = d_survivors + n_units - 1; ab.reverse = 1; ab.n_survivors = d_counters + 4;
-        launch_exact(ctx->dcfg, b, ab, ctx->plan, st);
+        launch_exact(ctx->dcfg, b, ab, plan, st);
         a.survivors = hard; a.n_survivors = d_counters + 3; a.work_counter = d_counters + 5; a.total_survivors = nullptr;
         ctx->stats.kernel_launches += 2;
     } else if (s_cap > 0 && n_units < (1u << 28)) {
         unsigned int* hard = d_survivors + n_units;
         launch_long_thread(ctx->dcfg, b, d_survivors, d_counters, a.packed_probes, s_cap, max_slices, *d_scratch + long_off, hard,
-                           d_counters + 3, ctx->d_total_surv, ctx->sm_count, st);
+                           d_counters + 3, ctx->d_total_surv, plan, st);
         a.survivors = hard; a.n_survivors = d_counters + 3; a.total_survivors = nullptr;
         ctx->stats.kernel_launches += 3;
     }
-    launch_exact(ctx->dcfg, b, a, ctx->plan, st);
-    if (ev) CK(cudaEventRecord(ev[3], st));
+    launch_exact(ctx->dcfg, b, a, plan, st);
+    if (ev) CK(cudaEventRecord(ev[4], st));
     CK(cudaGetLastError());
-    ctx->stats.kernel_launches += 3;
-    return TREW_OK;
+    ctx->stats.kernel_launches += 2;
+    return TREW_OK;
+}
+
+int launch_scan(trew_ctx* ctx, const DevBatch& b, uint32_t n_units, uint32_t max_read_len, unsigned int* d_survivors,
+                unsigned int* d_counters, unsigned char** d_scratch, size_t* scratch_bytes, cudaStream_t st) {
+    bool screened = false;
+    int rc = launch_screen_stage(ctx, b, n_units, max_read_len, d_survivors, d_counters, ctx->plan, st, &screened);
+    if (rc) return rc;
+    return launch_survivor_stage(ctx, b, n_units, max_read_len, d_survivors, d_counters, d_scratch, scratch_bytes, screened, ctx->plan, st);
 }
 
 int retire_slot(trew_ctx* ctx, SlotRes& s) {
@@ -412,33 +427,51 @@
 }
 
 int collect_prof(trew_ctx* ctx) {
+    size_t keep = 0;
     for (trew_resident* r : ctx->pending_prof) {
         if (!r->ev_pending) continue;
-        CK(cudaEventSynchronize(r->ev[3]));
+        if (r == ctx->pending) { ctx->pending_prof[keep++] = r; continue; }
+        CK(cudaEventSynchronize(r->ev[4]));
         float a = 0, b = 0, c = 0;
         CK(cudaEventElapsedTime(&a, r->ev[0], r->ev[1]));
-        CK(cudaEventElapsedTime(&b, r->ev[1], r->ev[2]));
-        CK(cudaEventElapsedTime(&c, r->ev[2], r->ev[3]));
+        CK(cudaEventElapsedTime(&b, r->ev[2], r->ev[3]));
+        CK(cudaEventElapsedTime(&c, r->ev[3], r->ev[4]));
         ctx->screen_ms += a; ctx->decide_ms += b; ctx->exact_ms += c; ctx->n_prof_scans++;
         ctx->stats.device_ms += a + b + c;
         r->ev_pending = false;
     }
-    ctx->pending_prof.clear();
+    ctx->pending_prof.resize(keep);
     return TREW_OK;
 }
 
 int join_aux(trew_ctx* ctx) {
-    if (ctx->resident_streams != 2) return TREW_OK;
     CK(cudaEventRecord(ctx->ev_join, ctx->aux_stream));
     CK(cudaStreamWaitEvent(ctx->main_stream, ctx->ev_join, 0));
     return TREW_OK;
 }
 
 int fork_aux(trew_ctx* ctx) {
-    if (ctx->resident_streams != 2) return TREW_OK;
     CK(cudaEventRecord(ctx->ev_join, ctx->main_stream));
     CK(cudaStreamWaitEvent(ctx->aux_stream, ctx->ev_join, 0));
     return TREW_OK;
+}
+
+int launch_stage_p(trew_ctx* ctx, trew_resident* r, const LaunchPlan& plan) {
+    r->ev_pending = false;
+    CK(cudaStreamWaitEvent(ctx->aux_stream, r->ev[1], 0));
+    int rc = launch_survivor_stage(ctx, r->batch, r->n_units, r->max_read_len, r->d_survivors, r->d_counters, &r->d_scratch,
+                                   &r->scratch_bytes, r->screened, plan, ctx->aux_stream, r->ev);
+    if (rc) return rc;
+    CK(cudaEventRecord(ctx->ev_b, ctx->aux_stream));
+    r->ev_pending = true;
+    return TREW_OK;
+}
+
+int flush_pending(trew_ctx* ctx) {
+    trew_resident* r = ctx->pending;
+    if (!r) return TREW_OK;
+    ctx->pending = nullptr;
+    return launch_stage_p(ctx, r, ctx->plan);
 }
 
 int check_device_error(trew_ctx* ctx) {
@@ -517,14 +550,15 @@
     cudaDeviceProp prop;
     CKC(cudaGetDeviceProperties(&prop, cfg->device));
     ctx->sm_count = prop.multiProcessorCount;
-    ctx->plan = default_launch_plan(ctx->sm_count);
+    CKC(query_scan_shape(cfg->device, &ctx->shape));
+    ctx->plan = default_launch_plan(&ctx->shape);
     {
         auto env_int = [](const char* name, int dflt) { const char* e = getenv(name); return e && *e ? atoi(e) : dflt; };
         int v;
         if ((v = env_int("TREW_GRID_SCREEN", 0)) > 0) ctx->plan.screen_blocks = ctx->sm_count * v;
         if ((v = env_int("TREW_GRID_DECIDE", 0)) > 0) ctx->plan.decide_blocks = ctx->sm_count * v;
         if ((v = env_int("TREW_GRID_EXACT", 0)) > 0) ctx->plan.exact_blocks = std::min(ctx->plan.exact_blocks, ctx->sm_count * v);
-        ctx->resident_streams = env_int("TREW_RESIDENT_STREAMS", 1) >= 2 ? 2 : 1;
+        if ((v = env_int("TREW_GRID_THREAD", 0)) > 0) ctx->plan.thread_bps = v;
         ctx->sparse_val = env_int("TREW_DENSE_VAL", 0) == 0;
         ctx->exact_flags = (unsigned int)env_int("TREW_EXACT_FLAGS", 0);
     }
@@ -553,7 +587,9 @@
     CKC(prepare_exact(kMaxWindow + 9));
     lap("kernel attributes (module load)");
     CKC(cudaStreamCreateWithFlags(&ctx->main_stream, cudaStreamNonBlocking));
-    CKC(cudaStreamCreateWithFlags(&ctx->aux_stream, cudaStreamNonBlocking));
+    int prio_low = 0, prio_high = 0;
+    CKC(cudaDeviceGetStreamPriorityRange(&prio_low, &prio_high));
+    CKC(cudaStreamCreateWithPriority(&ctx->aux_stream, cudaStreamNonBlocking, prio_high));
     CKC(cudaEventCreateWithFlags(&ctx->ev_join, cudaEventDisableTiming));
     CKC(cudaEventCreate(&ctx->ev_a));
     CKC(cudaEventCreate(&ctx->ev_b));
@@ -720,23 +756,34 @@
     CK(cudaSetDevice(ctx->cfg.device));
     trew_resident* r = const_cast<trew_resident*>(rb);
     ctx->keys_seen = std::max<unsigned int>(ctx->keys_seen, (unsigned int)(ctx->n_slots / 16 + 1));
-    if (r->ev_pending) { int rc0 = collect_prof(ctx); if (rc0) return rc0; }
-    if (!r->ev[0]) for (int i = 0; i < 4; i++) CK(cudaEventCreate(&r->ev[i]));
-    cudaStream_t st = (ctx->resident_streams == 2 && (ctx->resident_seq++ & 1)) ? ctx->aux_stream : ctx->main_stream;
-    CK(cudaEventRecord(ctx->ev_a, st));
-    int rc = launch_scan(ctx, r->batch, r->n_units, r->max_read_len, r->d_survivors, r->d_counters, &r->d_scratch,
-                         &r->scratch_bytes, st, r->ev);
+    int rc = TREW_OK;
+    if (ctx->pending == r && (rc = flush_pending(ctx)) != TREW_OK) return rc;
+    if (r->ev_pending && (rc = collect_prof(ctx)) != TREW_OK) return rc;
+    if (!r->ev[0]) for (int i = 0; i < 5; i++) CK(cudaEventCreate(&r->ev[i]));
+    CK(cudaStreamWaitEvent(ctx->main_stream, r->ev[4], 0));
+    CK(cudaEventRecord(ctx->ev_a, ctx->main_stream));
+    trew_resident* q = ctx->pending;
+    const LaunchPlan plan = q ? coresident_plan(ctx->plan, ctx->dcfg, r->max_read_len, kPipeScreenRoom) : ctx->plan;
+    ctx->pending = nullptr;
+    if (q && (rc = launch_stage_p(ctx, q, plan)) != TREW_OK) return rc;
+    rc = launch_screen_stage(ctx, r->batch, r->n_units, r->max_read_len, r->d_survivors, r->d_counters, plan, ctx->main_stream,
+                             &r->screened, r->ev);
+    if (rc) return rc;
     r->ev_pending = true; ctx->pending_prof.push_back(r);
-    if (rc) return rc;
-    CK(cudaEventRecord(ctx->ev_b, st));
+    ctx->pending = r;
     ctx->stats.reads += r->n_reads; ctx->stats.bases += r->bases; ctx->stats.units += r->n_units;
     return TREW_OK;
 }
 
 void trew_dev_free_resident(trew_ctx* ctx, trew_resident* r) {
     if (!r) return;
-    if (ctx) { cudaSetDevice(ctx->cfg.device); cudaStreamSynchronize(ctx->main_stream); cudaStreamSynchronize(ctx->aux_stream); collect_prof(ctx); }
-    for (int i = 0; i < 4; i++) if (r->ev[i]) cudaEventDestroy(r->ev[i]);
+    if (ctx) {
+        cudaSetDevice(ctx->cfg.device);
+        flush_pending(ctx);
+        cudaStreamSynchronize(ctx->main_stream); cudaStreamSynchronize(ctx->aux_stream);
+        collect_prof(ctx);
+    }
+    for (int i = 0; i < 5; i++) if (r->ev[i]) cudaEventDestroy(r->ev[i]);
     if (r->d_buf) cudaFree(r->d_buf);
     if (r->d_survivors) cudaFree(r->d_survivors);
     if (r->d_counters) cudaFree(r->d_counters);
@@ -747,6 +794,7 @@
 int trew_dev_sync(trew_ctx* ctx) {
     if (!ctx) return TREW_ERR_ARG;
     CK(cudaSetDevice(ctx->cfg.device));
+    { int rc = flush_pending(ctx); if (rc) return rc; }
     for (auto& s : ctx->slots) { int rc = retire_slot(ctx, s); if (rc) return rc; }
     { int rc = join_aux(ctx); if (rc) return rc; }
     CK(cudaStreamSynchronize(ctx->main_stream));
@@ -1017,6 +1065,8 @@
 
 int trew_dev_last_resident_ms(trew_ctx* ctx, float* ms) {
     if (!ctx || !ms) return TREW_ERR_ARG;
+    CK(cudaSetDevice(ctx->cfg.device));
+    { int rc = flush_pending(ctx); if (rc) return rc; }
     CK(cudaEventSynchronize(ctx->ev_b));
     CK(cudaEventElapsedTime(ms, ctx->ev_a, ctx->ev_b));
     return TREW_OK;
@@ -1032,6 +1082,7 @@
 int trew_dev_timer_stop(trew_ctx* ctx, float* ms) {
     if (!ctx || !ms) return TREW_ERR_ARG;
     CK(cudaSetDevice(ctx->cfg.device));
+    { int rc = flush_pending(ctx); if (rc) return rc; }
     { int rc = join_aux(ctx); if (rc) return rc; }
     CK(cudaEventRecord(ctx->ev_t1, ctx->main_stream));
     CK(cudaEventSynchronize(ctx->ev_t1));
@@ -1042,6 +1093,7 @@
 int trew_dev_kernel_times(trew_ctx* ctx, double* screen_ms, double* decide_ms, double* exact_ms, uint64_t* n_scans) {
     if (!ctx) return TREW_ERR_ARG;
     CK(cudaSetDevice(ctx->cfg.device));
+    { int rc0 = flush_pending(ctx); if (rc0) return rc0; }
     { int rc0 = join_aux(ctx); if (rc0) return rc0; }
     CK(cudaStreamSynchronize(ctx->main_stream));
     int rc = collect_prof(ctx);
diff --git a/trew_b200/csrc/scan_kernels.cu b/trew_b200/csrc/scan_kernels.cu
--- a/trew_b200/csrc/scan_kernels.cu
+++ b/trew_b200/csrc/scan_kernels.cu
@@ -1,7 +1,9 @@
 #include "scan_kernels.cuh"
 #include "exact_thread.cuh"
 
+#include <algorithm>
 #include <cstdio>
+#include <type_traits>
 
 namespace trew {
 
@@ -513,7 +515,7 @@
 #ifndef TREW_SCREEN_BPS
 #define TREW_SCREEN_BPS 8
 #endif
-template <bool LONG>
+template <bool LONG, bool CO>
 __global__ void __launch_bounds__(256, LONG ? 4 : TREW_SCREEN_BPS) trew_screen_kernel(DevCfg cfg, DevBatch b, u32 n_units,
                                                                                      u32* __restrict__ deferred, u32* __restrict__ n_deferred) {
     __shared__ uint4 tab[kFastTabSize];
@@ -676,7 +678,7 @@
     return k1 >= 32 && decide_span<1>(ph, pl, pa, wv, k0, k1, thr, done, t_hit, b, pos, wl, cache, cached, m4_below);
 }
 
-template <int MAXNW>
+template <int MAXNW, bool CO>
 __global__ void __launch_bounds__(kDecideThreads, (MAXNW <= 5 ? 4 : 2)) trew_filter_kernel(DevCfg cfg, DevBatch b, const u32* __restrict__ units,
                                                           const u32* __restrict__ n_units_ptr, u32 n_units_all,
                                                           u32* __restrict__ survivors, u32* __restrict__ n_survivors,
@@ -743,31 +745,64 @@
     }
 }
 
-void launch_filter(const DevCfg& cfg, const DevBatch& b, unsigned int n_units, unsigned int max_read_len,
-                   unsigned int* deferred, unsigned int* n_deferred, unsigned int* survivors, unsigned int* n_survivors,
-                   const LaunchPlan& plan, cudaStream_t stream, cudaEvent_t after_screen, unsigned int* surv_b_top,
-                   unsigned int* n_surv_b, unsigned int* work_counter) {
+static SmRes block_res(const ScanShape& s, KernelRes k, int threads, size_t dyn, int n) {
+    const int warps = (threads + 31) / 32;
+    const int smem = ((k.smem + (int)dyn + 127) & ~127) + s.smem_reserved;
+    return SmRes{n * warps * ((k.regs * 32 + 255) & ~255), n * smem, n * warps, n};
+}
+
+static int survivor_grid(const LaunchPlan& plan, KernelRes k, int threads, size_t dyn, int full) {
+    if (plan.beside.blocks == 0) return full;
+    const ScanShape& s = *plan.shape;
+    const SmRes one = block_res(s, k, threads, dyn, 1);
+    const int n = std::min(std::min((s.sm.regs - plan.beside.regs) / one.regs, (s.sm.smem - plan.beside.smem) / one.smem),
+                           std::min((s.sm.warps - plan.beside.warps) / one.warps, s.sm.blocks - plan.beside.blocks));
+    return s.sm_count * std::max(1, std::min(n, full / s.sm_count));
+}
+
+template <class F>
+static void with_co(const LaunchPlan& plan, F f) {
+    if (plan.beside.blocks) f(std::true_type{});
+    else f(std::false_type{});
+}
+
+static unsigned int longest_probe(const DevCfg& cfg, unsigned int max_read_len) {
+    if (cfg.mode == 2) return 2u * (unsigned)cfg.slice_len;
+    return (max_read_len < 4u * (unsigned)cfg.max_mer) ? max_read_len : (max_read_len + 1) / 2;
+}
+
+bool launch_screen(const DevCfg& cfg, const DevBatch& b, unsigned int n_units, unsigned int max_read_len, unsigned int* deferred,
+                   unsigned int* n_deferred, const LaunchPlan& plan, cudaStream_t stream) {
+    const bool screen = deferred != nullptr && !(cfg.mode == 2 && cfg.slice_len > kFastMaxWlLong) && n_units < (1u << kProbeShift);
+    if (!screen || n_units == 0) return false;
+    const unsigned int need = (n_units + 255) / 256;
+    int blocks = plan.screen_blocks;
+    if ((unsigned)blocks > need) blocks = (int)need;
+    const bool fast = longest_probe(cfg, max_read_len) <= (unsigned)kFastMaxWl;
+    with_co(plan, [&](auto co) {
+        if (fast) trew_screen_kernel<false, decltype(co)::value><<<blocks, 256, 0, stream>>>(cfg, b, n_units, deferred, n_deferred);
+        else trew_screen_kernel<true, decltype(co)::value><<<blocks, 256, 0, stream>>>(cfg, b, n_units, deferred, n_deferred);
+    });
+    return true;
+}
+
+void launch_decide(const DevCfg& cfg, const DevBatch& b, unsigned int n_units, unsigned int max_read_len,
+                   const unsigned int* deferred, const unsigned int* n_deferred, unsigned int* survivors, unsigned int* n_survivors,
+                   const LaunchPlan& plan, cudaStream_t stream, unsigned int* surv_b_top, unsigned int* n_surv_b,
+                   unsigned int* work_counter) {
     if (n_units == 0) return;
-    unsigned int longest;
-    if (cfg.mode == 2) longest = 2u * (unsigned)cfg.slice_len;
-    else longest = (max_read_len < 4u * (unsigned)cfg.max_mer) ? max_read_len : (max_read_len + 1) / 2;
-    unsigned int need = (n_units + 255) / 256;
-    const bool screen = deferred != nullptr && !(cfg.mode == 2 && cfg.slice_len > kFastMaxWlLong) && n_units < (1u << kProbeShift);
-    if (screen) {
-        int blocks = plan.screen_blocks;
-        if ((unsigned)blocks > need) blocks = (int)need;
-        if (longest <= (unsigned)kFastMaxWl) trew_screen_kernel<false><<<blocks, 256, 0, stream>>>(cfg, b, n_units, deferred, n_deferred);
-        else trew_screen_kernel<true><<<blocks, 256, 0, stream>>>(cfg, b, n_units, deferred, n_deferred);
-    }
-    if (after_screen) cudaEventRecord(after_screen, stream);
+    const unsigned int longest = longest_probe(cfg, max_read_len);
     static const int tmw = [] { const char* e = getenv("TREW_THREAD_MIN_WINDOWS"); return e && *e ? atoi(e) : kThreadMinWindows; }();
     static const int m4_on = [] { const char* e = getenv("TREW_MOD4_BELOW"); return e && *e ? atoi(e) : kMod4BelowWindows; }();
-    const unsigned int* list = screen ? deferred : nullptr;
-    int blocks = plan.decide_blocks;
+    const int v = longest + 1 <= 96 ? 0 : longest + 1 <= 160 ? 1 : 2;
+    int blocks = survivor_grid(plan, plan.shape->decide[v], 256, 0, plan.decide_blocks);
+    const unsigned int need = (n_units + 255) / 256;
     if ((unsigned)blocks > need) blocks = (int)need;
-    if (longest + 1 <= 96) trew_filter_kernel<3><<<blocks, 256, 0, stream>>>(cfg, b, list, n_deferred, n_units, survivors, n_survivors, surv_b_top, n_surv_b, tmw, m4_on, work_counter);
-    else if (longest + 1 <= 160) trew_filter_kernel<5><<<blocks, 256, 0, stream>>>(cfg, b, list, n_deferred, n_units, survivors, n_survivors, surv_b_top, n_surv_b, tmw, m4_on, work_counter);
-    else trew_filter_kernel<8><<<blocks, 256, 0, stream>>>(cfg, b, list, n_deferred, n_units, survivors, n_survivors, surv_b_top, n_surv_b, tmw, m4_on, work_counter);
+    with_co(plan, [&](auto co) {
+        if (v == 0) trew_filter_kernel<3, decltype(co)::value><<<blocks, 256, 0, stream>>>(cfg, b, deferred, n_deferred, n_units, survivors, n_survivors, surv_b_top, n_surv_b, tmw, m4_on, work_counter);
+        else if (v == 1) trew_filter_kernel<5, decltype(co)::value><<<blocks, 256, 0, stream>>>(cfg, b, deferred, n_deferred, n_units, survivors, n_survivors, surv_b_top, n_surv_b, tmw, m4_on, work_counter);
+        else trew_filter_kernel<8, decltype(co)::value><<<blocks, 256, 0, stream>>>(cfg, b, deferred, n_deferred, n_units, survivors, n_survivors, surv_b_top, n_surv_b, tmw, m4_on, work_counter);
+    });
 }
 
 
@@ -1633,7 +1668,7 @@
     }
 };
 
-template <int MODE, class K>
+template <int MODE, class K, bool CO>
 __global__ void __launch_bounds__(TREW_THREAD_BLOCK, (thread_kernel_bps<MODE, K>())) trew_exact_thread_kernel(DevCfg cfg, DevBatch b, const u32* __restrict__ survivors,
                                                                               const u32* __restrict__ n_survivors, int packed_probes,
                                                                               u32* __restrict__ hard, u32* __restrict__ n_hard,
@@ -1694,6 +1729,7 @@
     unsigned long long* total_survivors;
 };
 
+template <bool CO>
 __global__ void __launch_bounds__(TREW_THREAD_BLOCK, 4) trew_long_stats_kernel(DevCfg cfg, DevBatch b, LongArgs a) {
     u32* work = reinterpret_cast<u32*>(g_smem);
     const et::Mem m{work + threadIdx.x, TREW_THREAD_BLOCK};
@@ -1717,6 +1753,7 @@
     }
 }
 
+template <bool CO>
 __global__ void __launch_bounds__(256) trew_long_walk_kernel(DevCfg cfg, DevBatch b, LongArgs a) {
     const u32 n_all = *a.n_survivors;
     if (blockIdx.x == 0 && threadIdx.x == 0 && a.total_survivors) atomicAdd(a.total_survivors, (unsigned long long)n_all);
@@ -1750,6 +1787,7 @@
     }
 }
 
+template <bool CO>
 __global__ void __launch_bounds__(TREW_THREAD_BLOCK, 4) trew_long_emit_kernel(DevCfg cfg, DevBatch b, LongArgs a) {
     u32* work = reinterpret_cast<u32*>(g_smem);
     u64* s_key = reinterpret_cast<u64*>(work + et::Lay<et::u64>::WORDS * TREW_THREAD_BLOCK);
@@ -1800,7 +1838,7 @@
 
 void launch_long_thread(const DevCfg& cfg, const DevBatch& b, const unsigned int* survivors, const unsigned int* n_survivors,
                         int packed_probes, unsigned int s_cap, unsigned int max_slices, unsigned char* scratch, unsigned int* hard,
-                        unsigned int* n_hard, unsigned long long* total_survivors, int sm_count, cudaStream_t stream) {
+                        unsigned int* n_hard, unsigned long long* total_survivors, const LaunchPlan& plan, cudaStream_t stream) {
     LongArgs a{};
     a.survivors = survivors; a.n_survivors = n_survivors; a.packed_probes = packed_probes;
     a.s_cap = s_cap; a.max_slices = max_slices;
@@ -1808,9 +1846,15 @@
     a.stats = reinterpret_cast<unsigned short*>(scratch + (size_t)s_cap * (max_slices + 1) * sizeof(u32));
     a.hard = hard; a.n_hard = n_hard; a.total_survivors = total_survivors;
     const size_t smem_stats = (size_t)et::Lay<et::u64>::WORDS * TREW_THREAD_BLOCK * sizeof(u32);
-    trew_long_stats_kernel<<<sm_count * 4, TREW_THREAD_BLOCK, smem_stats, stream>>>(cfg, b, a);
-    trew_long_walk_kernel<<<sm_count * 2, 256, 0, stream>>>(cfg, b, a);
-    trew_long_emit_kernel<<<sm_count * 4, TREW_THREAD_BLOCK, kThreadKernelSmem, stream>>>(cfg, b, a);
+    const ScanShape& sh = *plan.shape;
+    const int g_stats = survivor_grid(plan, sh.long_stats, TREW_THREAD_BLOCK, smem_stats, sh.sm_count * 4);
+    const int g_walk = survivor_grid(plan, sh.long_walk, 256, 0, sh.sm_count * 2);
+    const int g_emit = survivor_grid(plan, sh.long_emit, TREW_THREAD_BLOCK, kThreadKernelSmem, sh.sm_count * 4);
+    with_co(plan, [&](auto co) {
+        trew_long_stats_kernel<decltype(co)::value><<<g_stats, TREW_THREAD_BLOCK, smem_stats, stream>>>(cfg, b, a);
+        trew_long_walk_kernel<decltype(co)::value><<<g_walk, 256, 0, stream>>>(cfg, b, a);
+        trew_long_emit_kernel<decltype(co)::value><<<g_emit, TREW_THREAD_BLOCK, kThreadKernelSmem, stream>>>(cfg, b, a);
+    });
 }
 
 bool thread_path_applies(const DevCfg& cfg, unsigned int max_read_len) {
@@ -1820,19 +1864,22 @@
 }
 
 void launch_exact_thread(const DevCfg& cfg, const DevBatch& b, const unsigned int* survivors, const unsigned int* n_survivors,
-                         int packed_probes, unsigned int* hard, unsigned int* n_hard, unsigned long long* total_survivors, int sm_count,
-                         int blocks_per_sm, unsigned int* work_counter, cudaStream_t stream) {
+                         int packed_probes, unsigned int* hard, unsigned int* n_hard, unsigned long long* total_survivors,
+                         const LaunchPlan& plan, unsigned int* work_counter, cudaStream_t stream) {
     const bool wide = cfg.max_mer > 32;
 #define TREW_LAUNCH_THREAD(MODE, K)                                                                                               \
-    trew_exact_thread_kernel<MODE, K><<<sm_count * (blocks_per_sm > 0 ? blocks_per_sm : thread_kernel_bps<MODE, K>()),            \
+    trew_exact_thread_kernel<MODE, K, decltype(co)::value><<<survivor_grid(plan, plan.shape->thread[MODE][wide], TREW_THREAD_BLOCK, thread_kernel_smem<K>(), \
+                                                      plan.shape->sm_count * (plan.thread_bps > 0 ? plan.thread_bps : thread_kernel_bps<MODE, K>())), \
                                         TREW_THREAD_BLOCK, thread_kernel_smem<K>(), stream>>>(                                    \
         cfg, b, survivors, n_survivors, packed_probes, hard, n_hard, total_survivors, work_counter)
-    if (cfg.mode == 0) { if (wide) TREW_LAUNCH_THREAD(0, et::u128); else TREW_LAUNCH_THREAD(0, et::u64); }
-    else               { if (wide) TREW_LAUNCH_THREAD(1, et::u128); else TREW_LAUNCH_THREAD(1, et::u64); }
+    with_co(plan, [&](auto co) {
+        if (cfg.mode == 0) { if (wide) TREW_LAUNCH_THREAD(0, et::u128); else TREW_LAUNCH_THREAD(0, et::u64); }
+        else               { if (wide) TREW_LAUNCH_THREAD(1, et::u128); else TREW_LAUNCH_THREAD(1, et::u64); }
+    });
 #undef TREW_LAUNCH_THREAD
 }
 
-template <int MODE>
+template <int MODE, bool CO>
 __global__ void __launch_bounds__(kExactWarps * 32, TREW_EXACT_BPS) trew_exact_kernel(DevCfg cfg, DevBatch b, ExactArgs a) {
     const int wid = threadIdx.x >> 5;
     const u32 lane = lane_id();
@@ -1861,28 +1908,97 @@
 constexpr int kExactBlocksPerSM = TREW_EXACT_BPS;
 int exact_warps_total(int sm_count) { return sm_count * kExactBlocksPerSM * kExactWarps; }
 
+template <bool CO>
+static cudaError_t prepare_kernels(int run_cap_max) {
+    const int bytes = (int)exact_smem_bytes(run_cap_max, true);
+    const int t64 = (int)thread_kernel_smem<et::u64>(), t128 = (int)thread_kernel_smem<et::u128>(), lt = (int)kThreadKernelSmem;
+    const auto dyn = cudaFuncAttributeMaxDynamicSharedMemorySize;
+    cudaError_t e = cudaFuncSetAttribute(trew_exact_kernel<0, CO>, dyn, bytes);
+    if (e == cudaSuccess) e = cudaFuncSetAttribute(trew_exact_kernel<1, CO>, dyn, bytes);
+    if (e == cudaSuccess) e = cudaFuncSetAttribute(trew_exact_kernel<2, CO>, dyn, bytes);
+    if (e == cudaSuccess) e = cudaFuncSetAttribute(trew_exact_thread_kernel<0, et::u64, CO>, dyn, t64);
+    if (e == cudaSuccess) e = cudaFuncSetAttribute(trew_exact_thread_kernel<1, et::u64, CO>, dyn, t64);
+    if (e == cudaSuccess) e = cudaFuncSetAttribute(trew_exact_thread_kernel<0, et::u128, CO>, dyn, t128);
+    if (e == cudaSuccess) e = cudaFuncSetAttribute(trew_exact_thread_kernel<1, et::u128, CO>, dyn, t128);
+    if (e == cudaSuccess) e = cudaFuncSetAttribute(trew_long_stats_kernel<CO>, dyn, lt);
+    if (e == cudaSuccess) e = cudaFuncSetAttribute(trew_long_emit_kernel<CO>, dyn, lt);
+    if (!CO || e != cudaSuccess) return e;
+    const int c = cudaSharedmemCarveoutMaxShared;
+    const auto cv = cudaFuncAttributePreferredSharedMemoryCarveout;
+    if (e == cudaSuccess) e = cudaFuncSetAttribute(trew_screen_kernel<false, CO>, cv, c);
+    if (e == cudaSuccess) e = cudaFuncSetAttribute(trew_screen_kernel<true, CO>, cv, c);
+    if (e == cudaSuccess) e = cudaFuncSetAttribute(trew_filter_kernel<3, CO>, cv, c);
+    if (e == cudaSuccess) e = cudaFuncSetAttribute(trew_filter_kernel<5, CO>, cv, c);
+    if (e == cudaSuccess) e = cudaFuncSetAttribute(trew_filter_kernel<8, CO>, cv, c);
+    if (e == cudaSuccess) e = cudaFuncSetAttribute(trew_exact_thread_kernel<0, et::u64, CO>, cv, c);
+    if (e == cudaSuccess) e = cudaFuncSetAttribute(trew_exact_thread_kernel<1, et::u64, CO>, cv, c);
+    if (e == cudaSuccess) e = cudaFuncSetAttribute(trew_exact_thread_kernel<0, et::u128, CO>, cv, c);
+    if (e == cudaSuccess) e = cudaFuncSetAttribute(trew_exact_thread_kernel<1, et::u128, CO>, cv, c);
+    if (e == cudaSuccess) e = cudaFuncSetAttribute(trew_exact_kernel<0, CO>, cv, c);
+    if (e == cudaSuccess) e = cudaFuncSetAttribute(trew_exact_kernel<1, CO>, cv, c);
+    if (e == cudaSuccess) e = cudaFuncSetAttribute(trew_exact_kernel<2, CO>, cv, c);
+    if (e == cudaSuccess) e = cudaFuncSetAttribute(trew_long_stats_kernel<CO>, cv, c);
+    if (e == cudaSuccess) e = cudaFuncSetAttribute(trew_long_walk_kernel<CO>, cv, c);
+    if (e == cudaSuccess) e = cudaFuncSetAttribute(trew_long_emit_kernel<CO>, cv, c);
+    return e;
+}
+
 cudaError_t prepare_exact(int run_cap_max) {
-    int bytes = (int)exact_smem_bytes(run_cap_max, true);
-    cudaError_t e = cudaFuncSetAttribute(trew_exact_kernel<0>, cudaFuncAttributeMaxDynamicSharedMemorySize, bytes);
-    if (e == cudaSuccess) e = cudaFuncSetAttribute(trew_exact_kernel<1>, cudaFuncAttributeMaxDynamicSharedMemorySize, bytes);
-    if (e == cudaSuccess) e = cudaFuncSetAttribute(trew_exact_kernel<2>, cudaFuncAttributeMaxDynamicSharedMemorySize, bytes);
-    if (e == cudaSuccess) e = cudaFuncSetAttribute(trew_exact_thread_kernel<0, et::u64>, cudaFuncAttributeMaxDynamicSharedMemorySize, (int)thread_kernel_smem<et::u64>());
-    if (e == cudaSuccess) e = cudaFuncSetAttribute(trew_exact_thread_kernel<1, et::u64>, cudaFuncAttributeMaxDynamicSharedMemorySize, (int)thread_kernel_smem<et::u64>());
-    if (e == cudaSuccess) e = cudaFuncSetAttribute(trew_exact_thread_kernel<0, et::u128>, cudaFuncAttributeMaxDynamicSharedMemorySize, (int)thread_kernel_smem<et::u128>());
-    if (e == cudaSuccess) e = cudaFuncSetAttribute(trew_exact_thread_kernel<1, et::u128>, cudaFuncAttributeMaxDynamicSharedMemorySize, (int)thread_kernel_smem<et::u128>());
-    if (e == cudaSuccess) e = cudaFuncSetAttribute(trew_long_stats_kernel, cudaFuncAttributeMaxDynamicSharedMemorySize, (int)kThreadKernelSmem);
-    if (e == cudaSuccess) e = cudaFuncSetAttribute(trew_long_emit_kernel, cudaFuncAttributeMaxDynamicSharedMemorySize, (int)kThreadKernelSmem);
+    cudaError_t e = prepare_kernels<false>(run_cap_max);
+    return e == cudaSuccess ? prepare_kernels<true>(run_cap_max) : e;
+}
+
+template <class F>
+static KernelRes kernel_res(F* f, cudaError_t* e) {
+    cudaFuncAttributes a{};
+    if (*e == cudaSuccess) *e = cudaFuncGetAttributes(&a, f);
+    return KernelRes{a.numRegs, (int)a.sharedSizeBytes};
+}
+
+cudaError_t query_scan_shape(int device, ScanShape* s) {
+    cudaDeviceProp p;
+    cudaError_t e = cudaGetDeviceProperties(&p, device);
+    if (e != cudaSuccess) return e;
+    s->sm_count = p.multiProcessorCount;
+    s->smem_reserved = (int)p.reservedSharedMemPerBlock;
+    s->sm = SmRes{p.regsPerMultiprocessor, (int)p.sharedMemPerMultiprocessor, p.maxThreadsPerMultiProcessor / 32, p.maxBlocksPerMultiProcessor};
+    s->screen[0] = kernel_res(trew_screen_kernel<false, true>, &e);
+    s->screen[1] = kernel_res(trew_screen_kernel<true, true>, &e);
+    s->decide[0] = kernel_res(trew_filter_kernel<3, true>, &e);
+    s->decide[1] = kernel_res(trew_filter_kernel<5, true>, &e);
+    s->decide[2] = kernel_res(trew_filter_kernel<8, true>, &e);
+    s->thread[0][0] = kernel_res(trew_exact_thread_kernel<0, et::u64, true>, &e);
+    s->thread[0][1] = kernel_res(trew_exact_thread_kernel<0, et::u128, true>, &e);
+    s->thread[1][0] = kernel_res(trew_exact_thread_kernel<1, et::u64, true>, &e);
+    s->thread[1][1] = kernel_res(trew_exact_thread_kernel<1, et::u128, true>, &e);
+    s->exact[0] = kernel_res(trew_exact_kernel<0, true>, &e);
+    s->exact[1] = kernel_res(trew_exact_kernel<1, true>, &e);
+    s->exact[2] = kernel_res(trew_exact_kernel<2, true>, &e);
+    s->long_stats = kernel_res(trew_long_stats_kernel<true>, &e);
+    s->long_walk = kernel_res(trew_long_walk_kernel<true>, &e);
+    s->long_emit = kernel_res(trew_long_emit_kernel<true>, &e);
     return e;
 }
 
-LaunchPlan default_launch_plan(int sm_count) { return LaunchPlan{sm_count * 128, sm_count * 4, sm_count * kExactBlocksPerSM}; }
+LaunchPlan coresident_plan(const LaunchPlan& full, const DevCfg& cfg, unsigned int screen_max_read_len, int screen_bps) {
+    LaunchPlan p = full;
+    const ScanShape& s = *full.shape;
+    p.beside = block_res(s, s.screen[longest_probe(cfg, screen_max_read_len) <= (unsigned)kFastMaxWl ? 0 : 1], 256, 0, screen_bps);
+    return p;
+}
+
+LaunchPlan default_launch_plan(const ScanShape* s) {
+    return LaunchPlan{s->sm_count * 128, s->sm_count * 4, s->sm_count * kExactBlocksPerSM, 0, s, SmRes{0, 0, 0, 0}};
+}
 
 void launch_exact(const DevCfg& cfg, const DevBatch& b, const ExactArgs& a, const LaunchPlan& plan, cudaStream_t stream) {
     size_t smem = exact_smem_bytes(a.run_cap, true);
-    dim3 grid(plan.exact_blocks), block(kExactWarps * 32);
-    if (cfg.mode == 0) trew_exact_kernel<0><<<grid, block, smem, stream>>>(cfg, b, a);
-    else if (cfg.mode == 1) trew_exact_kernel<1><<<grid, block, smem, stream>>>(cfg, b, a);
-    else trew_exact_kernel<2><<<grid, block, smem, stream>>>(cfg, b, a);
-}
-
-}
+    dim3 grid(survivor_grid(plan, plan.shape->exact[cfg.mode], kExactWarps * 32, smem, plan.exact_blocks)), block(kExactWarps * 32);
+    with_co(plan, [&](auto co) {
+        if (cfg.mode == 0) trew_exact_kernel<0, decltype(co)::value><<<grid, block, smem, stream>>>(cfg, b, a);
+        else if (cfg.mode == 1) trew_exact_kernel<1, decltype(co)::value><<<grid, block, smem, stream>>>(cfg, b, a);
+        else trew_exact_kernel<2, decltype(co)::value><<<grid, block, smem, stream>>>(cfg, b, a);
+    });
+}
+
+}
diff --git a/trew_b200/csrc/scan_kernels.cuh b/trew_b200/csrc/scan_kernels.cuh
--- a/trew_b200/csrc/scan_kernels.cuh
+++ b/trew_b200/csrc/scan_kernels.cuh
@@ -48,13 +48,30 @@
     unsigned int exp_flags;
 };
 
-struct LaunchPlan { int screen_blocks, decide_blocks, exact_blocks; };
-LaunchPlan default_launch_plan(int sm_count);
+struct SmRes { int regs, smem, warps, blocks; };
+struct KernelRes { int regs, smem; };
+struct ScanShape {
+    int sm_count, smem_reserved;
+    SmRes sm;
+    KernelRes screen[2], decide[3], thread[2][2], exact[3];
+    KernelRes long_stats, long_walk, long_emit;
+};
+cudaError_t query_scan_shape(int device, ScanShape* out);
 
-void launch_filter(const DevCfg& cfg, const DevBatch& b, unsigned int n_units, unsigned int max_read_len,
-                   unsigned int* deferred, unsigned int* n_deferred, unsigned int* survivors, unsigned int* n_survivors,
-                   const LaunchPlan& plan, cudaStream_t stream, cudaEvent_t after_screen,
-                   unsigned int* surv_b_top, unsigned int* n_surv_b, unsigned int* work_counter);
+struct LaunchPlan {
+    int screen_blocks, decide_blocks, exact_blocks, thread_bps;
+    const ScanShape* shape;
+    SmRes beside;
+};
+LaunchPlan default_launch_plan(const ScanShape* shape);
+LaunchPlan coresident_plan(const LaunchPlan& full, const DevCfg& cfg, unsigned int screen_max_read_len, int screen_bps);
+
+bool launch_screen(const DevCfg& cfg, const DevBatch& b, unsigned int n_units, unsigned int max_read_len, unsigned int* deferred,
+                   unsigned int* n_deferred, const LaunchPlan& plan, cudaStream_t stream);
+void launch_decide(const DevCfg& cfg, const DevBatch& b, unsigned int n_units, unsigned int max_read_len,
+                   const unsigned int* deferred, const unsigned int* n_deferred, unsigned int* survivors, unsigned int* n_survivors,
+                   const LaunchPlan& plan, cudaStream_t stream, unsigned int* surv_b_top, unsigned int* n_surv_b,
+                   unsigned int* work_counter);
 size_t exact_smem_bytes(int run_cap, bool wide);
 cudaError_t prepare_exact(int run_cap_max);
 void launch_exact(const DevCfg& cfg, const DevBatch& b, const ExactArgs& a, const LaunchPlan& plan, cudaStream_t stream);
@@ -63,11 +80,11 @@
 size_t long_thread_scratch_bytes(unsigned int s_cap, unsigned int max_slices);
 void launch_long_thread(const DevCfg& cfg, const DevBatch& b, const unsigned int* survivors, const unsigned int* n_survivors,
                         int packed_probes, unsigned int s_cap, unsigned int max_slices, unsigned char* scratch, unsigned int* hard,
-                        unsigned int* n_hard, unsigned long long* total_survivors, int sm_count, cudaStream_t stream);
+                        unsigned int* n_hard, unsigned long long* total_survivors, const LaunchPlan& plan, cudaStream_t stream);
 bool thread_path_applies(const DevCfg& cfg, unsigned int max_read_len);
 void launch_exact_thread(const DevCfg& cfg, const DevBatch& b, const unsigned int* survivors, const unsigned int* n_survivors,
-                         int packed_probes, unsigned int* hard, unsigned int* n_hard, unsigned long long* total_survivors, int sm_count,
-                         int blocks_per_sm, unsigned int* work_counter, cudaStream_t stream);
+                         int packed_probes, unsigned int* hard, unsigned int* n_hard, unsigned long long* total_survivors,
+                         const LaunchPlan& plan, unsigned int* work_counter, cudaStream_t stream);
 void launch_compact(const Slot* slots, unsigned int n_slots, trew_entry* out, unsigned int* d_n, cudaStream_t stream, unsigned int cap);
 cudaError_t sort_entries_radix(const trew_entry* d_entries, trew_entry* d_out, unsigned int n, bool wide, void* d_temp,
                                size_t* temp_bytes, cudaStream_t stream);
```
